# seanwood/gcc-nmf

Measured on AMD Instinct MI355X. Metric: stereo frames/sec (1024-FFT, K=1024, 100 NMF iters), higher is better.
Workload: dtype f32; 1 GPU; HBM-resident (float32 samples in HBM -> separated float32 waveforms in HBM; the host-to-host rates are the host_to_host_* fields of a --full run): 64 x 10 s stereo @16 kHz synthetic mixtures per GPU (SURVEY 8d recipe), 1024-pt FFT hop 256 (F=513, T=622/file), K=1024, 100 KL-NMF iters, 128 TDOAs, 3 targets, independent dictionary per file; dictionary_size=1024, parallelism=file-sharded x1, no data-path collective

## Files before the change

gcc_nmf_amd/_hip.py:

```python
import ctypes
import math
import numbers
import os
import warnings

import torch

_HERE = os.path.dirname(os.path.abspath(__file__))
LIB_PATH = os.environ.get('GCCNMF_HIP_LIB') or os.path.join(_HERE, 'libgccnmf_hip.so')

c_int, c_long, c_float, c_void_p = ctypes.c_int, ctypes.c_long, ctypes.c_float, ctypes.c_void_p
P_INT = ctypes.POINTER(ctypes.c_int)


class SharedShard(ctypes.Structure):
    _fields_ = [('V', c_void_p), ('H', c_void_p), ('workspace', c_void_p), ('N', c_int), ('batch', c_int), ('ld', c_int)]


class DirectGemm(ctypes.Structure):
    _fields_ = [('A', c_void_p), ('B', c_void_p), ('sA', c_long), ('sB', c_long), ('lda', c_int), ('ldb', c_int),
                ('M', c_int), ('N', c_int), ('Kd', c_int), ('batch', c_int),
                ('bscale', c_void_p), ('s_bscale', c_long), ('tailA', c_void_p), ('s_tailA', c_long), ('tail_row', c_int),
                ('rowsumB', c_void_p), ('s_rowsumB', c_long), ('C', c_void_p), ('sC', c_long), ('ldc', c_int),
                ('Ct', c_void_p), ('sCt', c_long), ('ldct', c_int), ('E0', c_void_p), ('sE0', c_long), ('lde0', c_int),
# ... 290 lines not shown

GCCNMF_SCORES_TRACKS = 0x100


def target_scores_masks(CC, trig, idx, W, F, T, K, D, S, batch, ws, scores, argmax, tracks=False, stream=None):
    _stage('gccnmf_target_scores_masks', CC, trig, idx, W, F, T, K, D, S | GCCNMF_SCORES_TRACKS if tracks else S, batch, ws, scores,
           argmax, stream=stream)


GCCNMF_PEAKS_COUNT_BIT = 1 << 30
GCCNMF_SCORES_COUNTED = 0x800
MAX_AUTO_SOURCES = 8
ENGINE_MAX_AUTO_TARGETS = 8


def check_auto_sources(numSources, maxSources=MAX_AUTO_SOURCES):
    if isinstance(numSources, str):
        if numSources != 'auto':
            raise ValueError("numSources must be a number of sources or 'auto', got %r" % (numSources,))
        m = maxSources
        if isinstance(m, bool) or not isinstance(m, numbers.Integral) or not 1 <= m <= 255:
            raise ValueError('maxSources must be a whole number from 1 to 255, got %r' % (m,))
        return True
    return False


def check_auto_targets(numTargets, maxTargets, tdoaTracking=False):
    if check_auto_sources(numTargets, 1):
        if tdoaTracking:
            raise ValueError("numTargets='auto' cannot be combined with tdoaTracking (every frame's peak set takes one count per launch)")
        m = 4 if maxTargets is None else maxTargets
        if isinstance(m, bool) or not isinstance(m, numbers.Integral) or not 1 <= m <= ENGINE_MAX_AUTO_TARGETS:
            raise ValueError('maxTargets must be a whole number from 1 to %d, got %r' % (ENGINE_MAX_AUTO_TARGETS, m))
        return True, int(m)
    if maxTargets is not None:
        raise ValueError("maxTargets needs numTargets='auto'")
    return False, numTargets


def peaks_count_word(maxSources):
    check_auto_sources('auto', maxSources)
    return int(maxSources) | GCCNMF_PEAKS_COUNT_BIT


def count_tdoa_peaks(mean_ang, D, Dp, maxSources, batch, idx, status, stream=None):
    _stage('gccnmf_pick_tdoa_peaks', mean_ang, D, Dp, peaks_count_word(maxSources), batch, idx, status, stream=stream,
           what='gccnmf_pick_tdoa_peaks (count)')


def target_scores_masks_counted(CC, trig, idx, W, F, T, K, D, S, batch, ws, scores, argmax, counted=False, stream=None):
    if not 1 <= int(S) <= 255:
        raise ValueError('the score stage takes 1 to 255 targets, got %r' % (S,))
    _stage('gccnmf_target_scores_masks', CC, trig, idx, W, F, T, K, D, int(S) | GCCNMF_SCORES_COUNTED if counted else int(S), batch, ws,
           scores, argmax, stream=stream, what='gccnmf_target_scores_masks (counted)' if counted else None)


GCCNMF_SCORES_ATOM_TDOA = 0x200
GCCNMF_SCORES_ENHANCEMENT_MASKS = 0x400
ATOM_TDOA_MAX_D = 1024
TARGET_MODE_BOXCAR, TARGET_MODE_MULTIPLE, TARGET_MODE_WINDOW_FUNCTION = 0, 1, 2


def atom_tdoa_indexes(CC, trig, W, F, T, K, D, batch, atom_tdoa, atom_score=None, stream=None):
    _stage('gccnmf_target_scores_masks', CC, trig, None, W, F, T, K, D, GCCNMF_SCORES_ATOM_TDOA, batch, None, atom_score, atom_tdoa,
           stream=stream, what='gccnmf_target_scores_masks (atom TDOA)')


def check_enhancement_target(targetMode, targetTDOAEpsilon, targetTDOABeta, targetTDOANoiseFloor):
    modes = {'boxcar': 0, 'window': 1, TARGET_MODE_BOXCAR: 0, TARGET_MODE_WINDOW_FUNCTION: 1}
    if isinstance(targetMode, bool) or targetMode not in modes:
        raise ValueError("targetMode must be TARGET_MODE_BOXCAR / 'boxcar' or TARGET_MODE_WINDOW_FUNCTION / 'window', got %r" % (targetMode,))
    out = []
    for name, v, low_ok in (('targetTDOAEpsilon', targetTDOAEpsilon, False), ('targetTDOABeta', targetTDOABeta, False),
                            ('targetTDOANoiseFloor', targetTDOANoiseFloor, True)):
        if isinstance(v, bool) or not isinstance(v, numbers.Real) or not math.isfinite(v) or v < 0 or (v == 0 and not low_ok):
            raise ValueError('%s must be a finite number %s 0, got %r' % (name, '>=' if low_ok else '>', v))
        v32 = ctypes.c_float(float(v)).value
        if not math.isfinite(v32) or (v32 == 0 and not low_ok):
            raise ValueError('%s=%r is not a float32 number %s 0' % (name, v, '>=' if low_ok else '>'))
        out.append(v32)
    return (modes[targetMode],) + tuple(out)


def enhancement_masks(atom_tdoa, target, T, K, batch, image, masks, window=0, eps=5.0, beta=2.0, noise_floor=0.0, per_frame=False, stream=None):
    if window not in (0, 1):
        raise ValueError('window must be 0 (boxcar) or 1 (window function), got %r' % (window,))
    params = (c_float * 3)(eps, beta, noise_floor)
    word = GCCNMF_SCORES_ENHANCEMENT_MASKS | int(window) | (GCCNMF_SCORES_TRACKS if per_frame else 0)
    _stage('gccnmf_target_scores_masks', atom_tdoa, ctypes.addressof(params), target, None, 0, T, K, 0, word, batch, None, masks, image,
           stream=stream, what='gccnmf_target_scores_masks (enhancement masks)')


def argmax_targets(scores, K, T, S, batch, argmax, stream=None):
    _stage('gccnmf_argmax_targets', scores, K, T, S, batch, argmax, stream=stream)


RECONSTRUCTIONS = ('direct', 'ratio', 'spatial')
GCCNMF_RECONSTRUCT_RATIO = 0x100
RATIO_MAX_TARGETS = 8
GCCNMF_RECONSTRUCT_SPATIAL_BIT = 1 << 16
GCCNMF_SPATIAL_LOADING = 1e-3
GCCNMF_RECONSTRUCT_SPATIAL_ITERATIONS_SHIFT = 20
MAX_SPATIAL_ITERATIONS = 255


def check_reconstruction(reconstruction, numTargets):
    if reconstruction not in RECONSTRUCTIONS:
        raise ValueError("reconstruction must be 'direct', 'ratio' or 'spatial', got %r" % (reconstruction,))
    if reconstruction != 'direct' and not 1 <= int(numTargets) <= RATIO_MAX_TARGETS:
        raise ValueError("reconstruction=%r takes 1 to %d targets, got %d" % (reconstruction, RATIO_MAX_TARGETS, int(numTargets)))
    return reconstruction


def check_spatial_iterations(spatialIterations, reconstruction):
    n = spatialIterations
    if isinstance(n, bool) or not isinstance(n, numbers.Integral) or not 0 <= int(n) <= MAX_SPATIAL_ITERATIONS:
        raise ValueError('spatialIterations must be an int from 0 to %d, got %r' % (MAX_SPATIAL_ITERATIONS, n))
    if int(n) and reconstruction != 'spatial':
        raise ValueError("spatialIterations=%d needs reconstruction='spatial', got %r" % (int(n), reconstruction))
    return int(n)


def reconstruct_word(S, mode, iterations=0):
    iterations = check_spatial_iterations(iterations, mode)
    word = int(S)
    if mode != 'direct':
        word |= GCCNMF_RECONSTRUCT_RATIO
    return word | (iterations << GCCNMF_RECONSTRUCT_SPATIAL_ITERATIONS_SHIFT)


def reconstruct_spatial_batch(batch):
    if not 1 <= int(batch) <= 65535:
        raise ValueError('the spatial reconstruction takes 1 to 65535 files per call, got %r' % (batch,))
    return int(batch) | GCCNMF_RECONSTRUCT_SPATIAL_BIT


def reconstruct_spatial_workspace_floats(batch, S, Fp):
    return 4 * int(batch) * int(S) * int(Fp)


def reconstruct_spatial_em_workspace_floats(batch, S, Fp, Tp):
    return reconstruct_spatial_workspace_floats(batch, S, Fp) + int(batch) * int(S) * int(Fp) * int(Tp)


def reconstruct_workspace_floats(mode, T, K, S, batch, Fp, iterations=0):
    iterations = check_spatial_iterations(iterations, mode)
    if mode == 'direct':
        return lib().gccnmf_reconstruct_workspace_floats(T, K, S, batch)
    if mode == 'spatial' and iterations:
        return reconstruct_spatial_em_workspace_floats(batch, S, Fp, -(-int(T) // 64) * 64)
    return reconstruct_spatial_workspace_floats(batch, S, Fp) if mode == 'spatial' else 0


def reconstruct(W, H, argmax, masks, X, V, F, T, K, S, batch, spec, mode='direct', workspace=None, iterations=0, stream=None):
    if mode not in RECONSTRUCTIONS:
        raise ValueError('unknown reconstruction mode %r' % (mode,))
    S = reconstruct_word(S, mode, iterations)
    if mode == 'spatial':
        if workspace is None:
            raise ValueError("reconstruction='spatial' needs its covariance workspace (reconstruct_workspace_floats)")
        batch = reconstruct_spatial_batch(batch)
    _stage('gccnmf_reconstruct', W, H, argmax, masks, X, V, F, T, K, S, batch, None if mode == 'ratio' else workspace, spec, stream=stream)


RT_FRAMES, RT_SKIP_LOCALIZE, RT_ONLY_LOCALIZE = 1, 2, 4
RT_BANK_LAYOUT, MAX_BANK_STREAMS = 1 << 3, 4096
RT_MULTI_LAYOUT, MAX_SOURCES = 1 << 20, 8
RT_ROW8_LAYOUT = 1 << 24
RT_LOCALIZE = {'with': 0, 'skip': RT_SKIP_LOCALIZE, 'only': RT_ONLY_LOCALIZE}
RT_SEPARATION_SPATIAL = 2
DEFAULT_SPATIAL_FILTER_FRAMES = 128.0


def rt_spatial_state_offset(D, numTDOAHistory, S=1):
    return -(-(int(S) * int(D) * int(numTDOAHistory)) // 4) * 4


def rt_spatial_state_floats(F, NC, S=1):
    return 4 * int(S) * int(NC) * int(F)


def check_spatial_filter(spatialFilterEnabled, spatialFilterFrames):
    t = spatialFilterFrames
    if isinstance(t, bool) or not isinstance(t, numbers.Real) or not math.isfinite(t) or not t >= 1:
        raise ValueError('spatialFilterFrames must be a finite number of frames >= 1, got %r' % (t,))
    t32 = ctypes.c_float(float(t)).value
    if not math.isfinite(t32):
        raise ValueError('spatialFilterFrames=%r is not a float32' % (t,))
    return bool(spatialFilterEnabled), float(t32)


def rt_mode_word(frames=False, localize='with', streams=None, targets=None, nl_row=False, target_mode=TARGET_MODE_MULTIPLE):
    if not isinstance(localize, str) or localize not in RT_LOCALIZE:
        raise ValueError("localize must be 'with', 'skip' or 'only', got %r" % (localize,))
    word = (RT_FRAMES if frames else 0) | RT_LOCALIZE[localize] | (RT_ROW8_LAYOUT if nl_row else 0)
    if nl_row and (streams is not None or targets is not None):
        raise ValueError('nl_row is the single-stream, single-target row: the bank and multi-target rows always have word 6')
    if streams is not None:
        if frames:
            raise ValueError('a bank of streams has no frames mode')
        if not 1 <= int(streams) <= MAX_BANK_STREAMS:
            raise ValueError('a bank holds 1 to %d streams, got %r' % (MAX_BANK_STREAMS, streams))
        word |= RT_BANK_LAYOUT | (int(streams) - 1) << 8
    if targets is not None:
        if int(target_mode) != TARGET_MODE_MULTIPLE:
            raise ValueError('the multi-target layout needs TARGET_MODE_MULTIPLE, got target_mode %r' % (target_mode,))
        if not 1 <= int(targets) <= MAX_SOURCES:
            raise ValueError('the multi-target layout takes 1 to %d targets, got %r' % (MAX_SOURCES, targets))
        word |= RT_MULTI_LAYOUT | (int(targets) - 1) << 21
    return word


def rt_process_block(block_in, block_out, in_ring, out_ring, X, Y, C, HMask, argmaxTDOA, tfMask, hist, hist_pos, target, gccphat, W, cosT,
                     sinT, window, synthesis_window, twiddle, colsumW, Hcoef, Rv, windowSize, hopSize, blockSize, K, Kp, D, Dp, numTDOAHistory,
                     target_mode, separation_enabled, localization_enabled, localization_window, numHUpdates=0, out_delay_blocks=2,
                     frames=False, localize='with', streams=None, targets=None, nl_row=False, spatial=False, stream=None):
    word = rt_mode_word(frames, localize, streams, targets, nl_row, target_mode)
    if spatial and not (nl_row or streams is not None or targets is not None):
        raise ValueError('spatial needs a target row with a word 7: nl_row, a bank of streams or the multi-target layout')
    separation = (1 | (RT_SEPARATION_SPATIAL if spatial else 0)) if separation_enabled else 0
    _stage('gccnmf_rt_process_block_ll', block_in, block_out, in_ring, out_ring, X, Y, C, HMask, argmaxTDOA, tfMask, hist, hist_pos, target,
           gccphat, W, cosT, sinT, window, synthesis_window, twiddle, colsumW, Hcoef, Rv, windowSize, hopSize, blockSize, K, Kp, D, Dp,
           numTDOAHistory, int(target_mode), separation, int(bool(localization_enabled)), localization_window, word,
           int(numHUpdates), int(out_delay_blocks), stream=stream)
```

gcc_nmf_amd/csrc/common.h:

```cpp
#pragma once
#include <hip/hip_runtime.h>
#include <stdint.h>

#define GCCNMF_OK 0
#define GCCNMF_ERR_ARG 1
#define GCCNMF_ERR_LAUNCH 2
#define GCCNMF_ERR_UNSUPPORTED 3

static inline int gccnmf_ceil_div(int a, int b) { return (a + b - 1) / b; }
static inline int gccnmf_round_up(int a, int b) { return gccnmf_ceil_div(a, b) * b; }

#define GCCNMF_CHECK_LAUNCH()                                   \
    do {                                                        \
        hipError_t e__ = hipGetLastError();                     \
        if (e__ != hipSuccess) return GCCNMF_ERR_LAUNCH;        \
    } while (0)

struct GccNmfPitches {
    int Fp, Kp, Np, Tp;
};

static inline GccNmfPitches gccnmf_make_pitches(int F, int T, int K) {
    GccNmfPitches p;
    p.Fp = gccnmf_round_up(F, 16);
    p.Kp = gccnmf_round_up(K, 64);
    p.Np = gccnmf_round_up(2 * T, 64);
    p.Tp = gccnmf_round_up(T, 64);
    return p;
}

#define GCCNMF_TUNE_KEYS 26
struct GccNmfTune {
    int v[GCCNMF_TUNE_KEYS];
};
extern thread_local GccNmfTune gccnmf_tune;
struct GccNmfCall {
    GccNmfCall();
    ~GccNmfCall();
};
#define GCCNMF_ENTER() GccNmfCall gccnmf_call_scope_
#define gccnmf_tune_ablate (gccnmf_tune.v[1])
#define gccnmf_tune_tile_policy (gccnmf_tune.v[2])
#define gccnmf_tune_dma (gccnmf_tune.v[3])
#define gccnmf_tune_ring (gccnmf_tune.v[4])
#define gccnmf_tune_wh_splits (gccnmf_tune.v[5])
#define gccnmf_tune_rht_splits (gccnmf_tune.v[6])
#define gccnmf_tune_exact_div (gccnmf_tune.v[7])
#define gccnmf_tune_shared_groups (gccnmf_tune.v[8])
#define gccnmf_tune_tail_split (gccnmf_tune.v[9])
#define gccnmf_tune_direct (gccnmf_tune.v[10])
#define gccnmf_tune_direct_tile (gccnmf_tune.v[11])
#define gccnmf_tune_direct_batch (gccnmf_tune.v[12])
#define gccnmf_tune_direct_depth (gccnmf_tune.v[13])
#define gccnmf_tune_short_updh (gccnmf_tune.v[14])
#define gccnmf_tune_fft_r16 (gccnmf_tune.v[15])
#define gccnmf_tune_fused_k12 (gccnmf_tune.v[16])
#define gccnmf_tune_fused_k34 (gccnmf_tune.v[17])
#define gccnmf_tune_persistent (gccnmf_tune.v[18])
#define gccnmf_tune_prefetch (gccnmf_tune.v[19])
#define gccnmf_tune_wide_update_w (gccnmf_tune.v[20])
#define gccnmf_tune_chain (gccnmf_tune.v[21])
#define gccnmf_tune_chain_solo (gccnmf_tune.v[22])
#define gccnmf_tune_chain_rag (gccnmf_tune.v[23])
#define gccnmf_tune_chain_chunk (gccnmf_tune.v[24])
#define gccnmf_tune_chain_fault (gccnmf_tune.v[25])
```

gcc_nmf_amd/csrc/gcc.hip:

```cpp
#include "gemm_ring.h"
#include "ratio.h"
#include "spatial.h"
#include "angular_nl.h"
#include "atom_tdoa.h"
#include "source_count.h"
#include "../../include/gccnmf_hip.h"


static bool gcc_small_launch(int batch, int M, int N, int Kd) {
    if (!gccnmf_tune_ring || !gccnmf_ring_supports(Kd) || gccnmf_tune_tile_policy == 1) return false;
    if (gccnmf_tune_tile_policy == 2) return true;
    return (long)batch * gccnmf_ceil_div(M, 512) * gccnmf_ceil_div(N, 64) < 256;
}

__global__ __launch_bounds__(256) void ang_mean_kernel(const float* __restrict__ ang, int T, int D, int Dp, int Tp,
                                                       double* __restrict__ mean_ang) {
    __shared__ double red[256];
    const int b = blockIdx.x / D, d = blockIdx.x - b * D;
    const float* row = ang + ((long)b * Dp + d) * Tp;
    double s = 0.0;
    for (int t = threadIdx.x; t < T; t += 256) s += (double)row[t];
    red[threadIdx.x] = s;
    __syncthreads();
    for (int w = 128; w > 0; w >>= 1) {
        if (threadIdx.x < w) red[threadIdx.x] += red[threadIdx.x + w];
        __syncthreads();
    }
    if (threadIdx.x == 0) mean_ang[(long)b * Dp + d] = red[0] / (double)T;
}

__device__ __forceinline__ bool pick_peaks_row(const double* v, unsigned char* is_peak, int* s_found, int D, int S, int* out,
                                               long out_stride) {
    __syncthreads();
    for (int i = threadIdx.x; i < D; i += 64) is_peak[i] = (i > 0 && i < D - 1 && v[i] > v[i - 1] && v[i] > v[i + 1]) ? 1 : 0;
    __syncthreads();
    if (threadIdx.x == 0) *s_found = 0;
    __syncthreads();
    for (int s = 0; s < S; ++s) {
        double bv = 0.0;
        int bi = -1;
        for (int i = 1 + threadIdx.x; i < D - 1; i += 64)
            if (is_peak[i] == 1 && (bi < 0 || v[i] >= bv)) {
                bv = v[i];
                bi = i;
            }
#pragma unroll
        for (int o = 32; o > 0; o >>= 1) {
            const double ov = __shfl_xor(bv, o);
            const int oi = __shfl_xor(bi, o);
            if (oi >= 0 && (bi < 0 || ov > bv || (ov == bv && oi > bi))) {
                bv = ov;
                bi = oi;
            }
        }
        if (bi < 0) break;
        if (threadIdx.x == 0) {
            is_peak[bi] = 2;
            ++*s_found;
        }
        __syncthreads();
    }
    __syncthreads();
    if (threadIdx.x != 0) return false;
    int n = 0;
    for (int i = 1; i < D - 1 && n < S; ++i)
        if (is_peak[i] == 2) out[(n++) * out_stride] = i;
    for (; n < S; ++n) out[n * out_stride] = -1;
    return *s_found == S;
}

__global__ __launch_bounds__(64) void pick_peaks_kernel(const double* __restrict__ mean_ang, int D, int Dp, int S,
                                                        int* __restrict__ tdoa_idx, int* __restrict__ status) {
    __shared__ double v[4096];
    __shared__ unsigned char is_peak[4096];
    __shared__ int s_found;
    const int b = blockIdx.x;
    const double* m = mean_ang + (long)b * Dp;
    for (int i = threadIdx.x; i < D; i += 64) v[i] = m[i];
    const bool all = pick_peaks_row(v, is_peak, &s_found, D, S, tdoa_idx + (long)b * S, 1);
    if (threadIdx.x == 0) status[b] = all ? 0 : 1;
}

__global__ __launch_bounds__(64) void track_peaks_kernel(const float* __restrict__ ang, int T, int Tp, int D, int Dp, int S, int L,
                                                         int* __restrict__ tracks, int* __restrict__ status) {
    extern __shared__ double track_lds[];
    double* v = track_lds;
    int* s_found = (int*)(track_lds + D);
    unsigned char* is_peak = (unsigned char*)(track_lds + D + 2);
    const int t = blockIdx.x, b = blockIdx.y;
    const int first = t - L / 2;
    const int lo = first < 0 ? 0 : first, hi = first + L < T ? first + L : T;
    const double len = (double)(hi - lo);
    for (int d = threadIdx.x; d < D; d += 64) {
        const float* row = ang + ((long)b * Dp + d) * Tp;
        double s = 0.0;
        for (int g = lo & ~3; g < hi; g += 4) {
            const float4 a = *(const float4*)(row + g);
            if (g >= lo) s += (double)a.x;
            if (g + 1 >= lo && g + 1 < hi) s += (double)a.y;
            if (g + 2 >= lo && g + 2 < hi) s += (double)a.z;
            if (g + 3 >= lo && g + 3 < hi) s += (double)a.w;
        }
        v[d] = s / len;
    }
    const bool all = pick_peaks_row(v, is_peak, s_found, D, S, tracks + (long)b * S * Tp + t, Tp);
    if (threadIdx.x == 0) status[(long)b * Tp + t] = all ? 0 : 1;
}

__global__ __launch_bounds__(256) void track_carry_kernel(int T, int Tp, int S, int* __restrict__ tracks, int* __restrict__ status) {
    __shared__ int scan[256];
    __shared__ int s_carry, s_first;
    const int tid = threadIdx.x;
    int* st = status + (long)blockIdx.x * Tp;
    int* tr = tracks + (long)blockIdx.x * S * Tp;
    if (tid == 0) {
        s_carry = -1;
        s_first = T;
    }
    __syncthreads();
    for (int c = 0; c < T; c += 256) {
        const int t = c + tid;
        const bool complete = t < T && st[t] == 0;
        if (complete) atomicMin(&s_first, t);
        scan[tid] = complete ? t : -1;
        __syncthreads();
        for (int o = 1; o < 256; o <<= 1) {
            const int left = tid >= o ? scan[tid - o] : -1;
            __syncthreads();
            if (left > scan[tid]) scan[tid] = left;
            __syncthreads();
        }
        const int src = scan[tid] > s_carry ? scan[tid] : s_carry;
        if (t < T) st[t] = src;
        __syncthreads();
        if (tid == 255) s_carry = src;
        __syncthreads();
    }
    const int first = s_first;
    for (int t = tid; t < T; t += 256) {
        int src = st[t];
        if (src == t) {
            st[t] = 0;
            continue;
        }
        if (src < 0) src = first;
        for (int i = 0; i < S; ++i) tr[(long)i * Tp + t] = first < T ? tr[(long)i * Tp + src] : -1;
        st[t] = first < T ? 1 : 3;
    }
}

__device__ __forceinline__ float4 gcc_steer4(float4 cr, float4 ci, float4 c, float4 sn) {
#pragma clang fp contract(off)
    float4 out;
    out.x = fmaf(cr.x, c.x, ci.x * sn.x);
    out.y = cr.y * c.y + ci.y * sn.y;
    out.z = fmaf(cr.z, c.z, ci.z * sn.z);
    out.w = fmaf(cr.w, c.w, ci.w * sn.w);
    return out;
}

template <bool TRACKS, bool COUNTED>
__global__ __launch_bounds__(256) void gcc_steer_kernel(const float* __restrict__ CC, const float* __restrict__ trig,
                                                        const int* __restrict__ tdoa_idx, int F, int Fp, int T, int Tp, int D,
                                                        int Dp, int S, float* __restrict__ P) {
    const int col = 4 * (blockIdx.x * 256 + threadIdx.x);
// ... 169 lines not shown
    return GCCNMF_OK;
}

int gccnmf_pick_tdoa_peaks(const double* mean_ang, int D, int Dp, int S, int batch, int* tdoa_idx, int* status,
                           void* stream) {
    GCCNMF_ENTER();
    if (S > 0 && (S & ~0xff) == GCCNMF_PEAKS_COUNT_BIT) {
        S &= 0xff;
        if (!mean_ang || !tdoa_idx || !status || D < 3 || D > SOURCE_COUNT_MAX_D || Dp < D || S < 1 || batch < 1) return GCCNMF_ERR_ARG;
        return gccnmf_launch_count_peaks(mean_ang, D, Dp, S, batch, tdoa_idx, status, (hipStream_t)stream);
    }
    if (S & ~0xff) {
        const int L = (S >> 9) & 0x3fffff, T = Dp;
        if (S < 0 || !(S & GCCNMF_PEAKS_TRACKS_BIT) || L < 1) return GCCNMF_ERR_ARG;
        S &= 0xff;
        if (!mean_ang || !tdoa_idx || !status || D < 3 || D > 4096 || T < 1 || T >= (1 << 21) || S < 1 || batch < 1 || batch > 65535)
            return GCCNMF_ERR_ARG;
        const int Tp = gccnmf_round_up(T, 64);
        hipLaunchKernelGGL(track_peaks_kernel, dim3(T, batch), dim3(64), 8 * D + 16 + gccnmf_round_up(D, 16), (hipStream_t)stream, (const float*)mean_ang, T, Tp, D,
                           gccnmf_round_up(D, 64), S, L, tdoa_idx, status);
        GCCNMF_CHECK_LAUNCH();
        hipLaunchKernelGGL(track_carry_kernel, dim3(batch), dim3(256), 0, (hipStream_t)stream, T, Tp, S, tdoa_idx, status);
        GCCNMF_CHECK_LAUNCH();
        return GCCNMF_OK;
    }
    if (!mean_ang || !tdoa_idx || !status || D < 3 || D > 4096 || Dp < D || S < 1 || batch < 1) return GCCNMF_ERR_ARG;
    hipLaunchKernelGGL(pick_peaks_kernel, dim3(batch), dim3(64), 0, (hipStream_t)stream, mean_ang, D, Dp, S, tdoa_idx, status);
    GCCNMF_CHECK_LAUNCH();
    return GCCNMF_OK;
}

long gccnmf_scores_workspace_floats(int F, int T, int S, int batch) {
    GCCNMF_ENTER();
    if (F < 2 || T < 1 || S < 1 || batch < 1) return -1;
    GccNmfPitches p = gccnmf_make_pitches(F, T, 1);
    return (long)batch * p.Fp * S * p.Tp;
}

int gccnmf_target_scores_masks(const float* CC, const float* trig, const int* tdoa_idx, const float* W, int F, int T,
                               int K, int D, int S, int batch, float* workspace, float* scores, unsigned char* argmax,
                               void* stream) {
    GCCNMF_ENTER();
    const int mode = S & ~0xff;
    if (S > 0 && mode == GCCNMF_SCORES_ATOM_TDOA) {
        if (S & 0xff) return GCCNMF_ERR_ARG;
        if (!CC || !trig || !W || !argmax || F < 2 || T < 1 || K < 1 || D < 1 || batch < 1) return GCCNMF_ERR_ARG;
        if (D > ATOM_TDOA_MAX_D || batch > 65535 || T > (1 << 19)) return GCCNMF_ERR_UNSUPPORTED;
        return gccnmf_launch_atom_tdoa(CC, trig, W, F, T, K, D, batch, (unsigned short*)argmax, scores, (hipStream_t)stream);
    }
    if (S > 0 && (mode & ~GCCNMF_SCORES_TRACKS) == GCCNMF_SCORES_ENHANCEMENT_MASKS) {
        const int window = S & 0xff;
        if (window > 1 || !CC || !trig || !tdoa_idx || (!scores && !argmax) || T < 1 || K < 1 || batch < 1) return GCCNMF_ERR_ARG;
        const float eps = trig[0], beta = trig[1], nf = trig[2];
        if (!(eps > 0.f && eps < INFINITY && beta > 0.f && beta < INFINITY && nf >= 0.f && nf < INFINITY)) return GCCNMF_ERR_ARG;
        if (batch > 65535 || K > 65535 - 63) return GCCNMF_ERR_UNSUPPORTED;
        return gccnmf_launch_enhancement_masks((const unsigned short*)CC, tdoa_idx, (mode & GCCNMF_SCORES_TRACKS) ? 1 : 0, window, eps,
                                               beta, nf, T, K, batch, argmax, scores, (hipStream_t)stream);
    }
    if (S < 0 || ((mode & ~GCCNMF_SCORES_TRACKS) && mode != GCCNMF_SCORES_COUNTED)) return GCCNMF_ERR_ARG;
    S &= 0xff;
    const bool tracks = mode == GCCNMF_SCORES_TRACKS, counted = mode == GCCNMF_SCORES_COUNTED;
    if (!CC || !trig || !tdoa_idx || !W || !workspace || !scores || F < 2 || T < 1 || K < 1 || D < 1 || S < 1 || batch < 1)
        return GCCNMF_ERR_ARG;
    hipStream_t s = (hipStream_t)stream;
    GccNmfPitches p = gccnmf_make_pitches(F, T, K);
    const int Dp = gccnmf_round_up(D, 64);
    const int ncol = S * p.Tp;
    float* P = workspace;
    if (counted)
        hipLaunchKernelGGL((gcc_steer_kernel<false, true>), dim3(gccnmf_ceil_div(ncol, 1024), p.Fp, batch), dim3(256), 0, s, CC, trig,
                           tdoa_idx, F, p.Fp, T, p.Tp, D, Dp, S, P);
    else if (tracks)
        hipLaunchKernelGGL((gcc_steer_kernel<true, false>), dim3(gccnmf_ceil_div(ncol, 1024), p.Fp, batch), dim3(256), 0, s, CC, trig, tdoa_idx,
                           F, p.Fp, T, p.Tp, D, Dp, S, P);
    else
        hipLaunchKernelGGL((gcc_steer_kernel<false, false>), dim3(gccnmf_ceil_div(ncol, 1024), p.Fp, batch), dim3(256), 0, s, CC, trig, tdoa_idx,
                           F, p.Fp, T, p.Tp, D, Dp, S, P);
    GCCNMF_CHECK_LAUNCH();
    GemmArgs a = {};
    a.A = W; a.sA = (long)p.Fp * p.Kp; a.lda = p.Kp; a.a_clamp = p.Kp - 4;
    a.B = P; a.sB = (long)p.Fp * ncol; a.ldb = ncol; a.b_clamp = ncol - 4;
    a.M = K; a.N = ncol; a.Kd = F;
    if ((F % 16) == 1) {
        a.Kd = F - 1;
        a.ktailA = W + (long)(F - 1) * p.Kp; a.s_ktailA = a.sA;
        a.ktailB = P + (long)(F - 1) * ncol; a.s_ktailB = a.sB;
    }
    a.batch = batch; a.xcd_affine = 1;
    a.C = scores; a.sC = (long)p.Kp * ncol; a.ldc = ncol;
    int rc;
    if (gcc_small_launch(batch, a.M, a.N, a.Kd)) rc = gccnmf_launch_gemm_ring<false, false, EPI_STORE, false>(a, s);
    else if (K > 128 && gccnmf_tune_dma && gccnmf_tune_ablate != 128) rc = gccnmf_launch_gemm_dma<false, false, EPI_STORE, false>(a, s);
    else rc = (K > 128) ? gccnmf_launch_gemm<4, 1, false, false, EPI_STORE, false>(a, s)
                        : gccnmf_launch_gemm<1, 4, false, false, EPI_STORE, false>(a, s);
    if (rc) return rc;
    if (argmax) {
        hipLaunchKernelGGL(gcc_argmax_kernel, dim3(gccnmf_ceil_div(p.Tp, 1024), p.Kp, batch), dim3(256), 0, s, scores, K, p.Kp, T,
                           p.Tp, S, argmax);
        GCCNMF_CHECK_LAUNCH();
    }
    return GCCNMF_OK;
}

int gccnmf_argmax_targets(const float* scores, int K, int T, int S, int batch, unsigned char* argmax, void* stream) {
    GCCNMF_ENTER();
    if (!scores || !argmax || K < 1 || T < 1 || S < 1 || S > 255 || batch < 1) return GCCNMF_ERR_ARG;
    GccNmfPitches p = gccnmf_make_pitches(2, T, K);
    hipLaunchKernelGGL(gcc_argmax_kernel, dim3(gccnmf_ceil_div(p.Tp, 1024), p.Kp, batch), dim3(256), 0, (hipStream_t)stream, scores,
                       K, p.Kp, T, p.Tp, S, argmax);
    GCCNMF_CHECK_LAUNCH();
    return GCCNMF_OK;
}

int gccnmf_coherence(const float* X, int F, int T, int batch, float* CC, void* stream) {
    GCCNMF_ENTER();
    if (!X || !CC || F < 2 || T < 1 || batch < 1) return GCCNMF_ERR_ARG;
    GccNmfPitches p = gccnmf_make_pitches(F, T, 1);
    hipLaunchKernelGGL(gcc_coherence_kernel, dim3(gccnmf_ceil_div(T, 256), F, batch), dim3(256), 0, (hipStream_t)stream,
                       (const float2*)X, p.Fp, T, p.Tp, CC);
    GCCNMF_CHECK_LAUNCH();
    return GCCNMF_OK;
}

int gccnmf_magnitude(const float* X, int F, int T, int batch, float* V, void* stream) {
    GCCNMF_ENTER();
    if (!X || !V || F < 2 || T < 1 || batch < 1) return GCCNMF_ERR_ARG;
    GccNmfPitches p = gccnmf_make_pitches(F, T, 1);
    hipLaunchKernelGGL(gcc_magnitude_kernel, dim3(gccnmf_ceil_div(T, 256), F, batch * 2), dim3(256), 0, (hipStream_t)stream,
                       (const float2*)X, p.Fp, T, p.Tp, p.Np, V);
    GCCNMF_CHECK_LAUNCH();
    return GCCNMF_OK;
}

long gccnmf_reconstruct_workspace_floats(int T, int K, int S, int batch) {
    GCCNMF_ENTER();
    if (T < 1 || K < 1 || S < 1 || batch < 1) return -1;
    GccNmfPitches p = gccnmf_make_pitches(2, T, K);
    return (long)batch * p.Kp * 2 * S * p.Tp;
}

int gccnmf_reconstruct(const float* W, const float* H, const unsigned char* argmax, const float* masks, const float* X,
                       const float* V, int F, int T, int K, int S, int batch, float* workspace, float* spec, void* stream) {
    GCCNMF_ENTER();
    const int mode = S & ~0xff;
    S &= 0xff;
    if (mode & ~(GCCNMF_RECONSTRUCT_RATIO | GCCNMF_RECONSTRUCT_SPATIAL_ITERATIONS(0xff))) return GCCNMF_ERR_ARG;
    const bool ratio = (mode & GCCNMF_RECONSTRUCT_RATIO) != 0;
    const int iterations = (mode >> 20) & 0xff;
    if (batch < 1 || (batch & ~(0xffff | GCCNMF_RECONSTRUCT_SPATIAL_BIT))) return GCCNMF_ERR_ARG;
    const bool spatial = (batch & GCCNMF_RECONSTRUCT_SPATIAL_BIT) != 0;
    batch &= 0xffff;
    if (spatial && !ratio) return GCCNMF_ERR_ARG;
    if (iterations && !spatial) return GCCNMF_ERR_ARG;
    if (!W || !H || (!argmax && !masks) || !X || (!ratio && (!V || !workspace)) || !spec || F < 2 || T < 1 || K < 1 || S < 1 || batch < 1)
        return GCCNMF_ERR_ARG;
    if (spatial && (!workspace || ((uintptr_t)workspace & 15))) return GCCNMF_ERR_ARG;
    if (ratio && S > GCCNMF_RATIO_MAX_TARGETS) return GCCNMF_ERR_UNSUPPORTED;
    hipStream_t s = (hipStream_t)stream;
    if (ratio) {
        const int rc = gccnmf_launch_ratio(W, H, argmax, masks, X, F, T, K, S, batch, spec, s);
        if (rc != GCCNMF_OK || !spatial) return rc;
        if (!iterations) return gccnmf_launch_spatial(X, F, T, S, batch, workspace, spec, s);
        GccNmfPitches p = gccnmf_make_pitches(F, T, 1);
        float* powers = workspace + GCCNMF_RECONSTRUCT_SPATIAL_WORKSPACE_FLOATS(batch, S, p.Fp);
        return gccnmf_launch_spatial_em(X, F, T, S, batch, iterations, workspace, powers, spec, s);
    }
    GccNmfPitches p = gccnmf_make_pitches(F, T, K);
    const int ncol = 2 * S * p.Tp;
    float* Hm = workspace;
    hipLaunchKernelGGL(gcc_masked_h_kernel, dim3(gccnmf_ceil_div(ncol, 1024), p.Kp, batch), dim3(256), 0, s, H, argmax, masks, K, p.Kp,
                       T, p.Tp, p.Np, S, Hm);
    GCCNMF_CHECK_LAUNCH();
    const bool tail = (F % 128) == 1;
    GemmArgs a = {};
    a.A = W; a.sA = (long)p.Fp * p.Kp; a.lda = p.Kp; a.a_clamp = p.Fp - 1;
    a.B = Hm; a.sB = (long)p.Kp * ncol; a.ldb = ncol; a.b_clamp = ncol - 4;
    a.M = tail ? F - 1 : F; a.N = ncol; a.Kd = K;
    a.tail_row = F - 1;
    a.batch = batch; a.xcd_affine = 1;
    a.C = spec; a.sC = 2L * S * p.Fp * p.Tp;
    a.E0 = V; a.sE0 = (long)p.Fp * p.Np;
    a.X = (const float2*)X; a.sX = 2L * p.Fp * p.Tp;
    a.T = T; a.Tp = p.Tp; a.Fp = p.Fp; a.ldv = p.Np;
    if (gcc_small_launch(batch, a.M, a.N, a.Kd))
        return tail ? gccnmf_launch_gemm_ring<true, false, EPI_PHASE, true>(a, s) : gccnmf_launch_gemm_ring<true, false, EPI_PHASE, false>(a, s);
    const bool tall = a.M > 128;
    if (tall && gccnmf_tune_dma && gccnmf_tune_ablate != 128)
        return tail ? gccnmf_launch_gemm_dma<true, false, EPI_PHASE, true>(a, s) : gccnmf_launch_gemm_dma<true, false, EPI_PHASE, false>(a, s);
    if (tall) return tail ? gccnmf_launch_gemm<4, 1, true, false, EPI_PHASE, true>(a, s)
                          : gccnmf_launch_gemm<4, 1, true, false, EPI_PHASE, false>(a, s);
    return tail ? gccnmf_launch_gemm<1, 4, true, false, EPI_PHASE, true>(a, s)
                : gccnmf_launch_gemm<1, 4, true, false, EPI_PHASE, false>(a, s);
}

}
```

gcc_nmf_amd/csrc/gemm_dma.h:

```cpp
#pragma once
#include <mutex>
#include <type_traits>
#include "gemm_mfma.h"
#include "chain_sync.h"

#ifndef GEMM_DMA_ABL
#define GEMM_DMA_ABL 0
#endif

typedef __attribute__((address_space(3))) void* gemm_lds_ptr;
typedef __attribute__((address_space(1))) const void* gemm_glb_ptr;

__device__ __forceinline__ void gemm_dma16(const float* wave_uniform_base, unsigned lane_byte_offset, unsigned lds_wave_byte_addr) {
    asm volatile("s_mov_b32 m0, %2\n\tglobal_load_lds_dwordx4 %0, %1"
                 :
                 : "v"(lane_byte_offset), "s"(wave_uniform_base), "s"(lds_wave_byte_addr)
                 : "memory");
}

__device__ __forceinline__ void gemm_dma16_masked(const float* wave_uniform_base, unsigned lane_byte_offset, unsigned lds_wave_byte_addr,
                                                  unsigned long long wave_uniform_mask) {
    unsigned long long saved;
    asm volatile("s_mov_b64 %0, exec\n\ts_mov_b64 exec, %4\n\ts_mov_b32 m0, %3\n\tglobal_load_lds_dwordx4 %1, %2\n\ts_mov_b64 exec, %0"
                 : "=&s"(saved)
                 : "v"(lane_byte_offset), "s"(wave_uniform_base), "s"(lds_wave_byte_addr), "s"(wave_uniform_mask)
                 : "memory");
}

__device__ __forceinline__ int gemm_swz(int row) { return (row >> 2) & 3; }

__device__ __forceinline__ int gemm_opaque_tid() {
    int t;
    asm volatile("v_mov_b32 %0, %1" : "=v"(t) : "v"(threadIdx.x));
    return t;
}

typedef float gemm_f32x4 __attribute__((ext_vector_type(4)));
template <int OFF>
__device__ __forceinline__ gemm_f32x4 gemm_lds_read_b128(unsigned byte_addr) {
    gemm_f32x4 v;
    asm volatile("ds_read_b128 %0, %1 offset:%2" : "=v"(v) : "v"(byte_addr), "n"(OFF));
    return v;
}
typedef float gemm_f32x2 __attribute__((ext_vector_type(2)));
template <int OFF0, int OFF1>
__device__ __forceinline__ gemm_f32x2 gemm_lds_read2_b32(unsigned byte_addr) {
    gemm_f32x2 v;
    asm volatile("ds_read2_b32 %0, %1 offset0:%2 offset1:%3" : "=v"(v) : "v"(byte_addr), "n"(OFF0), "n"(OFF1));
    return v;
}

__device__ __forceinline__ void gemm_wait_lds() { asm volatile("s_waitcnt lgkmcnt(0)" ::: "memory"); }
template <typename T>
__device__ __forceinline__ void gemm_tie(T& v) { asm volatile("" : "+v"(v)); }

__device__ __forceinline__ void gemm_barrier_arrive(unsigned counter_byte_addr) {
    unsigned long long saved;
    asm volatile("s_mov_b64 %0, exec\n\ts_mov_b64 exec, 1\n\tds_add_u32 %1, %2\n\ts_mov_b64 exec, %0"
                 : "=&s"(saved)
                 : "v"(counter_byte_addr), "v"(1u)
                 : "memory");
}
__device__ __forceinline__ unsigned gemm_barrier_peek(unsigned counter_byte_addr) {
    unsigned seen;
    asm volatile("ds_read_b32 %0, %1" : "=v"(seen) : "v"(counter_byte_addr) : "memory");
    return seen;
}
__device__ __forceinline__ void gemm_barrier_wait(unsigned counter_byte_addr, unsigned target, unsigned seen) {
    unsigned seen_s;
    asm volatile("s_waitcnt lgkmcnt(0)\n1:\n\tv_readfirstlane_b32 %1, %0\n\ts_cmp_ge_u32 %1, %3\n\ts_cbranch_scc1 2f\n\t"
                 "s_sleep 1\n\tds_read_b32 %0, %2\n\ts_waitcnt lgkmcnt(0)\n\ts_branch 1b\n2:"
                 : "+v"(seen), "=&s"(seen_s)
                 : "v"(counter_byte_addr), "s"(target)
                 : "memory", "scc");
}

template <bool KC, int NT, int ROWS>
struct GemmFrag;
template <int NT, int ROWS>
struct GemmFrag<true, NT, ROWS> {
    gemm_f32x4 v[NT];
    __device__ __forceinline__ void read(unsigned base) {
        v[0] = gemm_lds_read_b128<0 * 2048>(base);
        v[1] = gemm_lds_read_b128<1 * 2048>(base);
        if constexpr (NT == 4) {
            v[2] = gemm_lds_read_b128<2 * 2048>(base);
            v[3] = gemm_lds_read_b128<3 * 2048>(base);
        }
    }
    __device__ __forceinline__ void tie() {
#pragma unroll
        for (int m = 0; m < NT; ++m) gemm_tie(v[m]);
    }
    __device__ __forceinline__ void clear() {
#pragma unroll
        for (int m = 0; m < NT; ++m) v[m] = gemm_f32x4{0.f, 0.f, 0.f, 0.f};
    }
    __device__ __forceinline__ float get(int m, int e) const { return v[m][e]; }
    __device__ __forceinline__ void scale(const gemm_f32x4& s) {
#pragma unroll
        for (int m = 0; m < NT; ++m) v[m] *= s;
    }
};
template <int NT, int ROWS>
struct GemmFrag<false, NT, ROWS> {
    gemm_f32x2 v[4][NT / 2];
    __device__ __forceinline__ void read(unsigned base) {
#pragma unroll
        for (int e = 0; e < 4; ++e) {
            v[e][0] = gemm_lds_read2_b32<0, 32>(base + 4 * e * ROWS);
            if constexpr (NT == 4) v[e][1] = gemm_lds_read2_b32<64, 96>(base + 4 * e * ROWS);
        }
    }
    __device__ __forceinline__ void tie() {
#pragma unroll
        for (int e = 0; e < 4; ++e)
#pragma unroll
            for (int h = 0; h < NT / 2; ++h) gemm_tie(v[e][h]);
    }
    __device__ __forceinline__ void clear() {
#pragma unroll
        for (int e = 0; e < 4; ++e)
#pragma unroll
            for (int h = 0; h < NT / 2; ++h) v[e][h] = gemm_f32x2{0.f, 0.f};
    }
    __device__ __forceinline__ float get(int m, int e) const { return v[e][m >> 1][m & 1]; }
    __device__ __forceinline__ void scale(const gemm_f32x4& s) {
#pragma unroll
        for (int e = 0; e < 4; ++e)
#pragma unroll
            for (int h = 0; h < NT / 2; ++h) v[e][h] *= s[e];
    }
};

__device__ __forceinline__ float gemm_div_fast(float v, float d) {
    const float r = __builtin_amdgcn_rcpf(d);
    const float q = v * r;
    return fmaf(fmaf(-d, q, v), r, q);
}

typedef int gemm_i32x4 __attribute__((ext_vector_type(4)));
__device__ float gemm_buffer_load(gemm_i32x4 rsrc, int voffset, int soffset, int aux) __asm("llvm.amdgcn.raw.buffer.load.f32");
__device__ gemm_f32x4 gemm_buffer_load4(gemm_i32x4 rsrc, int voffset, int soffset, int aux) __asm("llvm.amdgcn.raw.buffer.load.v4f32");
__device__ void gemm_buffer_store(float data, gemm_i32x4 rsrc, int voffset, int soffset, int aux) __asm("llvm.amdgcn.raw.buffer.store.f32");
__device__ __forceinline__ gemm_i32x4 gemm_buffer_rsrc(const void* wave_uniform_base, long bytes = 0x7fffffffL) {
    const unsigned long long a = (unsigned long long)wave_uniform_base;
    gemm_i32x4 r;
    r.x = __builtin_amdgcn_readfirstlane((int)(unsigned)a);
    r.y = __builtin_amdgcn_readfirstlane((int)(unsigned)(a >> 32) & 0xffff);
    r.z = __builtin_amdgcn_readfirstlane((int)(bytes < 0x7fffffffL ? bytes : 0x7fffffffL));
    r.w = 0x00020000;
    return r;
}

template <int EPI, int BM = 512>
struct GemmEpiloguePair {
    static_assert(EPI == EPI_STORE || EPI == EPI_DIV || EPI == EPI_UPDH, "");
    float xa[16], xb[16];

    __device__ __forceinline__ void load(const GemmArgs& p, int file, int row_u, int hh, int col_a, long cb) {
        if (EPI == EPI_DIV || EPI == EPI_UPDH) {
            const int lo = 4 * (4 * hh * p.ldc + col_a);
            const int ro = 4 * row_u * p.ldc, rstep = 4 * p.ldc;
            const gemm_i32x4 X = gemm_buffer_rsrc(EPI == EPI_DIV ? p.E0 + file * p.sE0 : p.C + file * p.sC, cb);
#pragma unroll
            for (int r = 0; r < 16; ++r) {
                const int so = ro + ((r & 3) + 8 * (r >> 2)) * rstep;
                xa[r] = gemm_buffer_load(X, lo, so, 0);
                xb[r] = gemm_buffer_load(X, lo + 128, so, 0);
            }
        }
    }

    __device__ __forceinline__ void finish(const GemmArgs& p, int file, int row_u, int tile_row, int hh, int col_a, float ba, float bb,
                                           const float* s_rowvec, const f32x16& acc_a, const f32x16& acc_b, bool oka, bool okb, long cb) const {
        const int lo = 4 * (4 * hh * p.ldc + col_a);
        const int ro = 4 * row_u * p.ldc, rstep = 4 * p.ldc;
        const gemm_i32x4 C = gemm_buffer_rsrc(p.C + file * p.sC, cb);
        auto column = [&](const f32x16& acc, const float (&x)[16], const float b, const int lane_off) {
            float u[16];
#pragma unroll
            for (int r = 0; r < 16; ++r) u[r] = acc[r];
            if (EPI == EPI_STORE || EPI == EPI_UPDH) {
#pragma unroll
                for (int g = 0; g < 4; ++g) {
                    const gemm_f32x4 tav = *(const gemm_f32x4*)(s_rowvec + tile_row + 8 * g + 4 * hh);
                    gemm_f32x4 gv = {1.f, 1.f, 1.f, 1.f};
                    if (EPI == EPI_UPDH) gv = *(const gemm_f32x4*)(s_rowvec + BM + tile_row + 8 * g + 4 * hh);
#pragma unroll
                    for (int i = 0; i < 4; ++i) {
                        const int r = 4 * g + i;
                        u[r] = fmaf(tav[i], b, u[r]);
                        if (EPI == EPI_UPDH) u[r] = (x[r] * u[r]) * gv[i];
                    }
                }
            }
            if (EPI == EPI_DIV) {
                if (p.exact_div) {
#pragma unroll
                    for (int r = 0; r < 16; ++r) u[r] = x[r] / u[r];
                } else {
// ... 61 lines not shown
        if (TAIL) {
            const float u = (s_tail[tid] + s_tail[64 + tid]) + (s_tail[128 + tid] + s_tail[192 + tid]);
            wt_tail = Wp[(long)p.tail_row * p.ldc + col0 + tid] * (u / s_rs[tid]);
        }
        s_red[256 + tid] = wt_tail * wt_tail;
    }
    __syncthreads();
    if (tid < 64) s_norm[tid] = sqrtf(((s_red[tid] + s_red[64 + tid]) + (s_red[128 + tid] + s_red[192 + tid])) + s_red[256 + tid]);
    __syncthreads();
    const float ina = 1.0f / s_norm[ca], inb = 1.0f / s_norm[cb];
    float csa = 0.f, csb = 0.f;
    if (wave_active) {
#pragma unroll
        for (int m = 0; m < 4; ++m) {
            const int ro = (wm * 128 + m * 32) * rstep;
#pragma unroll
            for (int r = 0; r < 16; ++r) {
                const int so = ro + ((r & 3) + 8 * (r >> 2)) * rstep;
                const float na = acc[m][0][r] * ina, nb = acc[m][1][r] * inb;
                gemm_buffer_store(na, W, lo, so, 0);
                gemm_buffer_store(nb, W, lo + 128, so, 0);
                csa += na;
                csb += nb;
            }
        }
    }
    csa += __shfl_xor(csa, 32);
    csb += __shfl_xor(csb, 32);
    if (hh == 0) {
        s_red[wm * 64 + ca] = csa;
        s_red[wm * 64 + cb] = csb;
    }
    if (tid < 64) {
        float wn_tail = 0.f;
        if (TAIL) {
            wn_tail = wt_tail / s_norm[tid];
            Wp[(long)p.tail_row * p.ldc + col0 + tid] = wn_tail;
        }
        s_red[256 + tid] = wn_tail;
    }
    __syncthreads();
    if (tid < 64) {
        p.out_colsum[file * p.s_out + col0 + tid] = ((s_red[tid] + s_red[64 + tid]) + (s_red[128 + tid] + s_red[192 + tid])) + s_red[256 + tid];
        p.out_norm[file * p.s_out + col0 + tid] = s_norm[tid];
    }
}

__host__ __device__ __forceinline__ int gemm_dma_list_file(const GemmArgs& p, int q) {
    if (p.lists != 8) return q;
    const int n_full = p.batch >> 3, rem = p.batch & 7, big = rem * (n_full + 1);
    const int cls = q < big ? q / (n_full + 1) : rem + (q - big) / n_full;
    return cls + 8 * (q < big ? q - cls * (n_full + 1) : (q - big) - (cls - rem) * n_full);
}
__host__ __device__ __forceinline__ bool gemm_dma_item(const GemmArgs& p, int list, int t, int& file, int& tm, int& col0, int& nw) {
    if (p.ragged_n) {
        const int* L = p.ragged_lists + list * (GEMM_RAGGED_LMAX + 1);
        const int cnt = L[0];
        int acc = 0;
        for (int k = 0; k < cnt; ++k) {
            const int f = L[1 + k];
            const int n = p.ragged_kd ? p.N : p.ragged_n[f];
            const int tn = (n + 63) >> 6, per = p.tiles_m * tn;
            if (t < acc + per) {
                const int w = t - acc;
                const int wide_n = tn - (gemm_dma_file_rag(p.narrow_ok, n) ? 1 : 0), wt = p.tiles_m * wide_n;
                if (w < wt) {
                    tm = w / wide_n;
                    col0 = (w - tm * wide_n) * 64;
                    nw = 2;
                } else {
                    tm = w - wt;
                    col0 = (tn - 1) * 64;
                    nw = 1;
                }
                file = f + p.file0;
                return true;
            }
            acc += per;
        }
        return false;
    }
    const int wt = p.tiles_m * p.wide_n;
    if (p.whole_files == 2) {
        const int per = p.tiles_m * p.tiles_n;
        const long idx = (long)list * p.cw + t;
        if (t >= p.cw || idx >= (long)p.batch * per) return false;
        const int q = (int)(idx / per), w = (int)(idx - (long)q * per);
        if (w < wt) {
            tm = w / p.wide_n;
            col0 = (w - tm * p.wide_n) * 64;
            nw = 2;
        } else {
            tm = w - wt;
            col0 = (p.tiles_n - 1) * 64;
            nw = 1;
        }
        file = gemm_dma_list_file(p, q) + p.file0;
        return true;
    }
    if (p.whole_files) {
        const int per = p.tiles_m * p.tiles_n;
        const int ql = t / per, w = t - ql * per;
        const int fi = list + 8 * ql;
        if (fi >= p.batch) return false;
        if (w < wt) {
            tm = w / p.wide_n;
            col0 = (w - tm * p.wide_n) * 64;
            nw = 2;
        } else {
            tm = w - wt;
            col0 = (p.tiles_n - 1) * 64;
            nw = 1;
        }
        file = fi + p.file0;
        return true;
    }
    const int base_w = list * p.cw;
    const int len = min(max(p.batch * wt - base_w, 0), p.cw), s = min(p.split, len);
    int q;
    if (t < len + s) {
        int idx, half = 0;
        if (t < len - s) {
            idx = base_w + t;
            nw = 2;
        } else {
            const int j = t - (len - s);
            idx = base_w + (len - s) + (j >> 1);
            half = j & 1;
            nw = 1;
        }
        q = idx / wt;
        const int w = idx - q * wt;
        tm = w / p.wide_n;
        col0 = (w - tm * p.wide_n) * 64 + 32 * half;
    } else {
        const int r = t - (len + s), base_r = list * p.cr;
        const int lenr = min(max(p.batch * p.rag * p.tiles_m - base_r, 0), p.cr);
        if (r >= lenr) return false;
        const int idx = base_r + r;
        q = idx / p.tiles_m;
        tm = idx - q * p.tiles_m;
        col0 = (p.tiles_n - 1) * 64;
        nw = 1;
    }
    file = gemm_dma_list_file(p, q) + p.file0;
    return true;
}

template <int TM>
struct GemmDmaLds {
    static constexpr int SBUF = 128 * TM * 16 + 64 * 16 + 16 + 16;
};

template <bool A_KC, bool B_KC, int EPI, bool TAIL, int TM, bool NARROW>
__device__ __forceinline__ void gemm_dma_workgroup(const GemmArgs& p, float* const smem, float* const s_rowvec, unsigned* const s_arrivals_p,
                                                   int* const s_ticket, const int list, int t, const GemmSync& sync, const int sync_it = 0,
                                                   const bool trace_on = true) {
    static_assert(TM == 4 || TM == 2, "");
    static_assert(TM == 4 || EPI != EPI_UPDW, "the fused W update owns all rows of its atoms: full-height tiles only");
    static_assert(!NARROW || (EPI != EPI_UPDW && TM == 4), "narrow items: full-height tiles with an element-wise epilogue");
    constexpr int BK = 16, BM = 128 * TM, BN = 64, RW = 32 * TM;
    constexpr int NA = 2 * TM;
    constexpr int SA = BM * BK, SB = BN * BK;
    constexpr int SBUF = SA + SB + BK + BK;
    static_assert(SBUF == GemmDmaLds<TM>::SBUF, "");
    constexpr bool SCALE = !B_KC && (EPI == EPI_DIV || EPI == EPI_STORE);
    unsigned& s_arrivals = *s_arrivals_p;

    int tid = threadIdx.x, lane = tid & 63;
    const int wave = __builtin_amdgcn_readfirstlane(tid >> 6);
    const int wm = wave, wn = 0;
    int l31 = lane & 31, hh = lane >> 5;
#ifdef GCCNMF_EXPERIMENTS
    const bool persistent = p.tickets != nullptr;
#else
    constexpr bool persistent = false;
#endif

    int nkt = (p.Kd + BK - 1) / BK;
    int n_item = p.N;
    int n_sync = p.N;
    int file = 0, tm = 0, col0 = 0, nw = 2, row0 = 0;
    const float* __restrict__ A = nullptr;
    const float* __restrict__ B = nullptr;
    const float* __restrict__ bscale = nullptr;
    const float* __restrict__ tail_src = nullptr;
    const float* __restrict__ scale_src = nullptr;
    unsigned long long tail_mask = 0, scale_mask = 0;
    bool wave_active = false, do_tail = false, do_rowsum = false;
    unsigned offA[NA], offB = 0;
    auto take_item = [&](const int ticket) -> bool {
        int f_, tm_, c_, nw_;
        if (!gemm_dma_item(p, list, ticket, f_, tm_, c_, nw_)) return false;
        file = __builtin_amdgcn_readfirstlane(f_);
        tm = __builtin_amdgcn_readfirstlane(tm_);
        col0 = __builtin_amdgcn_readfirstlane(c_);
        nw = NARROW ? __builtin_amdgcn_readfirstlane(nw_) : 2;
        if (p.ragged_n) {
            const int nf = __builtin_amdgcn_readfirstlane(p.ragged_n[file]);
            n_sync = nf;
            if (p.ragged_kd) nkt = (nf + BK - 1) / BK;
            else n_item = nf;
        }
        row0 = tm * BM;
        A = p.A + file * p.sA;
        B = p.B + file * p.sB;
        bscale = (SCALE && p.bscale) ? p.bscale + file * p.s_bscale : nullptr;
        wave_active = (row0 + wm * RW) < p.M;
        do_tail = TAIL && (tm == 0);
        do_rowsum = B_KC && (p.rowsumB != nullptr || EPI == EPI_UPDW) && (tm == 0);
        tail_src = A + (long)p.tail_row * p.lda;
        tail_mask = (wave == 0 && do_tail) ? 0x0full : 0ull;
        scale_mask = (wave == 0 && bscale != nullptr) ? 0xf0ull : 0ull;
        scale_src = bscale != nullptr ? bscale : A;
        return true;
    };
    auto set_offsets = [&](const int lane) {
#pragma unroll
        for (int i = 0; i < NA; ++i) {
            const int piece = wave * NA + i;
            if (A_KC) {
                const int row = piece * 16 + (lane >> 2), c = (lane & 3) ^ gemm_swz(piece * 16 + (lane >> 2));
                offA[i] = 4u * (unsigned)(min(row0 + row, p.a_clamp) * p.lda + 4 * c);
            } else {
                constexpr int PPR = BM / 256;
                const int kk = piece / PPR, col = (piece % PPR) * 256 + lane * 4;
                offA[i] = 4u * (unsigned)(kk * p.lda + min(row0 + col, p.a_clamp));
            }
        }
        if (B_KC) {
            const int row = wave * 16 + (lane >> 2), c = (lane & 3) ^ gemm_swz(row);
            offB = 4u * (unsigned)(min(col0 + row, p.b_clamp) * p.ldb + 4 * c);
        } else {
            const int kk = wave * 4 + (lane >> 4), col = (lane & 15) * 4;
            offB = 4u * (unsigned)(kk * p.ldb + min(col0 + col, p.b_clamp));
        }
    };

    f32x16 acc[TM][2];
    float tail_acc = 0.f, rowsum_acc = 0.f;

    const unsigned lds0 = __builtin_amdgcn_readfirstlane((unsigned)(size_t)(gemm_lds_ptr)smem);
    unsigned side_off = 0;

    auto dma_piece = [&](const int piece, const int kt, const int buf) {
#ifdef GEMM_DMA_SKIP_FROM
        if (piece >= GEMM_DMA_SKIP_FROM) return;
#endif
        if (piece < NA) {
            gemm_dma16(A + (A_KC ? (long)kt * BK : (long)kt * BK * p.lda), offA[piece], lds0 + 4 * (buf * SBUF + (wave * NA + piece) * 256));
        } else if (piece == NA) {
            gemm_dma16(B + (B_KC ? (long)kt * BK : (long)kt * BK * p.ldb), offB, lds0 + 4 * (buf * SBUF + SA + wave * 256));
        } else {
            if (TAIL || SCALE) {
                const unsigned dst = lds0 + 4 * (buf * SBUF + SA + SB);
                if (TAIL) gemm_dma16_masked(tail_src + kt * BK, side_off, dst, tail_mask);
                if (SCALE) gemm_dma16_masked(scale_src + kt * BK, side_off, dst, scale_mask);
            }
        }
    };
    constexpr int NPIECES = NA + 2;
#ifdef GEMM_DMA_SPREAD
    constexpr int SPREAD = GEMM_DMA_SPREAD;
#else
    constexpr int SPREAD = (A_KC && !B_KC) ? 1 : 2;
#endif

    const gemm_f32x4 zero4 = {0.f, 0.f, 0.f, 0.f};
    GemmFrag<A_KC, TM, BM> a0, a1;
    GemmFrag<B_KC, 2, BN> b0, b1;
    gemm_f32x4 sc0 = zero4, sc1 = zero4, t4 = zero4, tb4 = zero4, ts4 = zero4, rs4 = zero4;
    gemm_f32x2 tbxy = {0.f, 0.f}, tbzw = {0.f, 0.f};

    const unsigned arrivals_addr = (unsigned)(size_t)(gemm_lds_ptr)s_arrivals_p;
    unsigned oA0 = 0, oA1 = 0, oB0 = 0, oB1 = 0, oTB = 0, oRS = 0;
    const int tg = wave;
    auto set_lane_constants = [&](const int tid_) {
        tid = tid_;
        lane = tid_ & 63;
        l31 = lane & 31;
        hh = lane >> 5;
        const int arow = wm * RW + l31, bcol = wn * 64 + l31, tj = lane;
        side_off = 16u * (unsigned)(lane & 3);
        oA0 = A_KC ? 4 * (arow * 16 + 4 * ((0 + hh) ^ gemm_swz(arow))) : 4 * (4 * (0 + hh) * BM + arow);
        oA1 = A_KC ? 4 * (arow * 16 + 4 * ((2 + hh) ^ gemm_swz(arow))) : 4 * (4 * (2 + hh) * BM + arow);
        oB0 = 4 * SA + (B_KC ? 4 * (bcol * 16 + 4 * ((0 + hh) ^ gemm_swz(bcol))) : 4 * (4 * (0 + hh) * BN + bcol));
        oB1 = 4 * SA + (B_KC ? 4 * (bcol * 16 + 4 * ((2 + hh) ^ gemm_swz(bcol))) : 4 * (4 * (2 + hh) * BN + bcol));
        oTB = 4 * SA + (B_KC ? 4 * (tj * 16 + 4 * (tg ^ gemm_swz(tj))) : 4 * (4 * tg * BN + tj));
        oRS = 4 * SA + 4 * ((tid_ >> 2) * 16 + 4 * (tid_ & 3));
    };

    auto read_group0 = [&](const unsigned lds) {
        if (wave_active) {
            a0.read(lds + oA0);
            b0.read(lds + oB0);
        }
        if (SCALE) sc0 = gemm_lds_read_b128<4 * (SA + SB + BK)>(lds + 16 * hh);
    };
    auto read_group1 = [&](const unsigned lds) {
        if (wave_active) {
            a1.read(lds + oA1);
            b1.read(lds + oB1);
        }
        if (SCALE) sc1 = gemm_lds_read_b128<4 * (SA + SB + BK) + 32>(lds + 16 * hh);
        if (TAIL) {
            t4 = gemm_lds_read_b128<4 * (SA + SB)>(lds + 16 * tg);
            if (B_KC) {
                tb4 = gemm_lds_read_b128<0>(lds + oTB);
            } else {
                tbxy = gemm_lds_read2_b32<0 * BN, 1 * BN>(lds + oTB);
                tbzw = gemm_lds_read2_b32<2 * BN, 3 * BN>(lds + oTB);
                if (SCALE) ts4 = gemm_lds_read_b128<4 * (SA + SB + BK)>(lds + 16 * tg);
            }
        }
        if (B_KC) rs4 = gemm_lds_read_b128<0>(lds + oRS);
    };
    auto wait_group0 = [&]() {
        gemm_wait_lds();
        a0.tie();
        b0.tie();
        if (SCALE) {
            gemm_tie(sc0);
            b0.scale(sc0);
        }
    };
    auto wait_group1 = [&]() {
        gemm_wait_lds();
        a1.tie();
        b1.tie();
        if (SCALE) {
            gemm_tie(sc1);
            b1.scale(sc1);
        }
        if (TAIL) {
            gemm_tie(t4);
            if (B_KC) {
                gemm_tie(tb4);
            } else {
                gemm_tie(tbxy);
                gemm_tie(tbzw);
                tb4 = gemm_f32x4{tbxy.x, tbxy.y, tbzw.x, tbzw.y};
                if (SCALE) {
                    gemm_tie(ts4);
                    tb4 *= ts4;
                }
            }
        }
        if (B_KC) gemm_tie(rs4);
    };
    auto mma = [&](auto nw_c, const GemmFrag<A_KC, TM, BM>& a, const GemmFrag<B_KC, 2, BN>& b, const int e, const int m) {
        constexpr int NW = decltype(nw_c)::value;
        acc[m][0] = __builtin_amdgcn_mfma_f32_32x32x2f32(a.get(m, e), b.get(0, e), acc[m][0], 0, 0, 0);
        if constexpr (NW == 2) acc[m][1] = __builtin_amdgcn_mfma_f32_32x32x2f32(a.get(m, e), b.get(1, e), acc[m][1], 0, 0, 0);
    };

#ifdef GEMM_DMA_PROBE
    unsigned long long probe[7] = {0, 0, 0, 0, 0, 0, 0};
#define GEMM_PROBE(i_) const unsigned long long pt##i_ = __builtin_amdgcn_s_memtime()
#define GEMM_PROBE_DECL(i_) unsigned long long pt##i_ = 0
#define GEMM_PROBE_SET(i_) pt##i_ = __builtin_amdgcn_s_memtime()
#else
#define GEMM_PROBE(i_)
#define GEMM_PROBE_DECL(i_)
#define GEMM_PROBE_SET(i_)
#endif
    auto step = [&](auto cur_c, auto nw_c, const int kt) {
        constexpr int CUR = decltype(cur_c)::value;
        const unsigned ldsC = lds0 + 4 * CUR * SBUF, ldsN = lds0 + 4 * (CUR ^ 1) * SBUF;
        const int ktn = min(kt + 1, nkt - 1);
        GEMM_PROBE(0);
#if !(GEMM_DMA_ABL & 1)
        read_group1(ldsC);
#endif
        __builtin_amdgcn_sched_barrier(0);
        if (wave_active) {
            if (SPREAD == 0) {
#pragma unroll
                for (int i = 0; i < NPIECES; ++i) dma_piece(i, ktn, CUR ^ 1);
                __builtin_amdgcn_sched_barrier(0);
            }
#pragma unroll
            for (int e = 0; e < 4; ++e)
#pragma unroll
                for (int m = 0; m < TM; ++m) {
                    mma(nw_c, a0, b0, e, m);
                    const int slot = e * TM + m;
                    if (SPREAD == 1 && slot < NPIECES) {
                        dma_piece(slot, ktn, CUR ^ 1);
                        __builtin_amdgcn_sched_barrier(0);
                    }
                    if (SPREAD == 2 && slot % 3 != 2 && (slot / 3) * 2 + slot % 3 < NPIECES) {
                        dma_piece((slot / 3) * 2 + slot % 3, ktn, CUR ^ 1);
                        __builtin_amdgcn_sched_barrier(0);
                    }
                }
        } else {
#pragma unroll
            for (int i = 0; i < NPIECES; ++i) dma_piece(i, ktn, CUR ^ 1);
        }
        __builtin_amdgcn_sched_barrier(0);
        GEMM_PROBE(1);
        wait_group1();
        GEMM_PROBE(2);
        GEMM_PROBE_DECL(3);
        GEMM_PROBE_DECL(4);
        GEMM_PROBE_DECL(5);
        unsigned seen = 0;
#ifndef GEMM_DMA_ARRIVE_E
#define GEMM_DMA_ARRIVE_E 1
#define GEMM_DMA_WAIT_E 3
#endif
#pragma unroll
        for (int e = 0; e < 4; ++e) {
            if (e == GEMM_DMA_ARRIVE_E) {
                __builtin_amdgcn_sched_barrier(0);
                GEMM_PROBE_SET(3);
                asm volatile("s_waitcnt vmcnt(0)" ::: "memory");
#if !(GEMM_DMA_ABL & 2)
                gemm_barrier_arrive(arrivals_addr);
#endif
                __builtin_amdgcn_sched_barrier(0);
            }
            if (e == GEMM_DMA_WAIT_E - 1) {
                __builtin_amdgcn_sched_barrier(0);
#if !(GEMM_DMA_ABL & 2)
                seen = gemm_barrier_peek(arrivals_addr);
#endif
                __builtin_amdgcn_sched_barrier(0);
            }
            if (e == GEMM_DMA_WAIT_E) {
                __builtin_amdgcn_sched_barrier(0);
                GEMM_PROBE_SET(4);
#if !(GEMM_DMA_ABL & 2)
                gemm_barrier_wait(arrivals_addr, 4u * (unsigned)(kt + 1), seen);
#endif
                GEMM_PROBE_SET(5);
#if !(GEMM_DMA_ABL & 1)
                read_group0(ldsN);
#endif
                __builtin_amdgcn_sched_barrier(0);
            }
            if (wave_active) {
#pragma unroll
                for (int m = 0; m < TM; ++m) mma(nw_c, a1, b1, e, m);
            }
        }
        if (TAIL) {
            tail_acc = fmaf(t4.x, tb4.x, tail_acc);
            tail_acc = fmaf(t4.y, tb4.y, tail_acc);
            tail_acc = fmaf(t4.z, tb4.z, tail_acc);
            tail_acc = fmaf(t4.w, tb4.w, tail_acc);
        }
        if (B_KC) rowsum_acc += (rs4.x + rs4.y) + (rs4.z + rs4.w);
        __builtin_amdgcn_sched_barrier(0);
        GEMM_PROBE(6);
        wait_group0();
#ifdef GEMM_DMA_PROBE
        __builtin_amdgcn_sched_barrier(0);
        const unsigned long long pt7 = __builtin_amdgcn_s_memtime();
        probe[0] += pt1 - pt0;
        probe[1] += pt2 - pt1;
        probe[2] += pt3 - pt2;
        probe[3] += pt4 - pt3;
        probe[4] += pt5 - pt4;
        probe[5] += pt6 - pt5;
        probe[6] += pt7 - pt6;
        __builtin_amdgcn_sched_barrier(0);
#endif
    };
    auto main_loop = [&](auto nw_c) {
        for (int kt = 0; kt < nkt; kt += 2) {
            step(std::integral_constant<int, 0>{}, nw_c, kt);
            if (kt + 1 < nkt) step(std::integral_constant<int, 1>{}, nw_c, kt + 1);
        }
    };

    if (SCALE) {
        if (!p.bscale && tid < 2 * BK) smem[(tid >> 4) * SBUF + SA + SB + BK + (tid & 15)] = 1.f;
    }
    bool have = take_item(t);
    if (have) set_offsets(lane);
    bool prefetched = false;
    int it = 0;
    long long* trace_row = nullptr;
    while (have) {
        const int vb = p.lists == 8 ? 8 * t + list : t;
        trace_row = (trace_on && p.trace && vb < p.trace_rows) ? p.trace + 8 * (long)vb : nullptr;
        if (trace_row && tid == 0) {
            trace_row[0] = trace_row[1] = __builtin_amdgcn_s_memrealtime();
            trace_row[4] = (long long)((__builtin_amdgcn_s_getreg((3 << 11) | 20) & 15u) << 16 | (__builtin_amdgcn_s_getreg((31 << 11) | 4) & 0xffffu));
            trace_row[7] = (long long)blockIdx.x << 16 | (long long)it;
        }
#ifdef GCCNMF_EXPERIMENTS
        set_lane_constants(gemm_opaque_tid());
        if (it > 0) set_offsets(lane);
        a0.clear(); a1.clear(); b0.clear(); b1.clear();
        sc0 = sc1 = t4 = tb4 = ts4 = rs4 = zero4;
        tbxy = tbzw = gemm_f32x2{0.f, 0.f};
#else
        set_lane_constants(tid);
#endif
        gemm_sync_wait(sync, file, col0, tid, sync_it, list, n_sync);
        if (trace_row && tid == 0) trace_row[1] = __builtin_amdgcn_s_memrealtime();
        if (!prefetched) {
#pragma unroll
            for (int i = 0; i < NPIECES; ++i) dma_piece(i, 0, 0);
        }
#pragma unroll
        for (int m = 0; m < TM; ++m)
#pragma unroll
            for (int n = 0; n < 2; ++n)
#pragma unroll
                for (int r = 0; r < 16; ++r) acc[m][n][r] = 0.f;
        tail_acc = 0.f;
        rowsum_acc = 0.f;
        if constexpr (EPI == EPI_STORE || EPI == EPI_UPDH) {
#pragma unroll
            for (int i = 0; i < BM / 256; ++i) {
                const int lr = tid + 256 * i, row = min(row0 + lr, p.M - 1);
                s_rowvec[lr] = p.ktailA ? p.ktailA[file * p.s_ktailA + row] : 0.f;
                if (EPI == EPI_UPDH) {
                    const float rd = 1.0f / (p.E2[file * p.sE2 + row] + p.alpha + p.eps);
                    s_rowvec[BM + lr] = p.E1 ? p.E1[file * p.sE1 + row] * rd : rd;
                }
            }
        }
        if (tid == 0) {
            s_arrivals = 0;
            if (persistent) s_ticket[it & 1] = p.wpl + (int)__hip_atomic_fetch_add(p.tickets + list, 1u, __ATOMIC_RELAXED, __HIP_MEMORY_SCOPE_AGENT);
        }
        asm volatile("s_waitcnt vmcnt(0)" ::: "memory");
        __syncthreads();
        read_group0(lds0);
        wait_group0();

        if constexpr (NARROW) {
            if (nw == 1) main_loop(std::integral_constant<int, 1>{});
            else main_loop(std::integral_constant<int, 2>{});
        } else {
            main_loop(std::integral_constant<int, 2>{});
        }
        __syncthreads();
        if (trace_row && tid == 0) trace_row[2] = __builtin_amdgcn_s_memrealtime();

        const int e_file = file, e_row0 = row0, e_col0 = col0, e_nw = nw, e_n = n_item;
        const bool e_active = wave_active, e_tail = do_tail, e_rowsum = do_rowsum;
        have = false;
        prefetched = false;
        if (persistent) {
            t = __builtin_amdgcn_readfirstlane(s_ticket[it & 1]);
            have = take_item(t);
            if (have && p.prefetch) {
                set_offsets(gemm_opaque_tid() & 63);
#pragma unroll
                for (int i = 0; i < NPIECES; ++i) dma_piece(i, 0, 0);
                prefetched = true;
            }
        }
        float* const scratch = smem + SBUF;

        if constexpr (EPI == EPI_UPDW) {
            if constexpr (TM == 4) gemm_epilogue_update_w_full<TAIL>(p, e_file, e_col0, tid, wm, l31, hh, e_active, acc, tail_acc, rowsum_acc, scratch);
        } else {
            if (e_active) {
                const int row_w = e_row0 + wm * RW;
                bool lean = false;
                if constexpr (EPI == EPI_STORE || EPI == EPI_DIV || EPI == EPI_UPDH) {
                    lean = row_w + RW <= p.M;
                    if (lean) {
                        GemmEpiloguePair<EPI, BM> e0, e1;
                        const int ca = e_col0 + l31, tr = wm * RW;
                        const bool oka = ca < e_n, okb = (!NARROW || e_nw == 2) && ca + 32 < e_n;
                        const long cb = 4L * p.ldc * (p.M + (TAIL ? 1 : 0));
                        float ba = 0.f, bb = 0.f;
                        e0.load(p, e_file, row_w, hh, ca, cb);
                        e1.load(p, e_file, row_w + 32, hh, ca, cb);
                        if (EPI != EPI_DIV && p.ktailA) {
                            ba = p.ktailB[e_file * p.s_ktailB + min(ca, e_n - 1)];
                            bb = p.ktailB[e_file * p.s_ktailB + min(ca + 32, e_n - 1)];
                        }
                        e0.finish(p, e_file, row_w, tr, hh, ca, ba, bb, s_rowvec, acc[0][0], acc[0][1], oka, okb, cb);
                        if (trace_row && tid == 0) trace_row[5] = __builtin_amdgcn_s_memrealtime();
                        if constexpr (TM == 4) e0.load(p, e_file, row_w + 64, hh, ca, cb);
                        e1.finish(p, e_file, row_w + 32, tr + 32, hh, ca, ba, bb, s_rowvec, acc[1][0], acc[1][1], oka, okb, cb);
                        if constexpr (TM == 4) {
                            e1.load(p, e_file, row_w + 96, hh, ca, cb);
                            e0.finish(p, e_file, row_w + 64, tr + 64, hh, ca, ba, bb, s_rowvec, acc[2][0], acc[2][1], oka, okb, cb);
                            e1.finish(p, e_file, row_w + 96, tr + 96, hh, ca, ba, bb, s_rowvec, acc[3][0], acc[3][1], oka, okb, cb);
                        }
                        if (trace_row && tid == 0) trace_row[6] = __builtin_amdgcn_s_memrealtime();
                    }
                }
                if (!lean) {
                    GemmArgs pq = p;
                    pq.N = e_n;
#pragma unroll
                    for (int m = 0; m < TM; ++m)
                        gemm_epilogue_pair<EPI>(pq, e_file, row_w + m * 32 + 4 * hh, e_col0 + wn * 64 + l31, acc[m][0], acc[m][1], !NARROW || e_nw == 2);
                }
            }
            if (TAIL) {
                if (e_tail) {
                    scratch[tid] = tail_acc;
                    __syncthreads();
                    if (tid < (NARROW && e_nw == 1 ? 32 : BN)) {
                        const float s = (scratch[tid] + scratch[BN + tid]) + (scratch[2 * BN + tid] + scratch[3 * BN + tid]);
                        const int col = e_col0 + tid;
                        if (EPI == EPI_PHASE ? gemm_col_valid<EPI>(p, col) : col < e_n) gemm_epilogue<EPI>(p, e_file, p.tail_row, col, s);
                    }
                }
            }
            if (B_KC) {
                if (e_rowsum) {
                    float s = rowsum_acc;
                    s += __shfl_xor(s, 1);
                    s += __shfl_xor(s, 2);
                    const int j = tid >> 2;
                    if ((tid & 3) == 0 && (e_col0 + j) < e_n && (!NARROW || e_nw == 2 || j < 32)) p.rowsumB[e_file * p.s_rowsumB + e_col0 + j] = s;
                }
            }
        }
        if (trace_row) {
            asm volatile("s_waitcnt vmcnt(0)" ::: "memory");
            __syncthreads();
            if (tid == 0) trace_row[3] = __builtin_amdgcn_s_memrealtime();
        }
        gemm_sync_signal(sync, e_file, e_col0, e_nw, tid);
        ++it;
        if (have) __syncthreads();
    }
#ifdef GEMM_DMA_PROBE
    if (p.trace && lane == 0 && (long)p.trace_grid + 4L * blockIdx.x + 4 <= p.trace_rows) {
#pragma unroll
        for (int i = 0; i < 7; ++i) p.trace[8 * ((long)p.trace_grid + blockIdx.x * 4 + wave) + i] = (long long)probe[i];
        p.trace[8 * ((long)p.trace_grid + blockIdx.x * 4 + wave) + 7] = it;
    }
#endif
    if (persistent && tid == 0) {
        const unsigned gone = __hip_atomic_fetch_add(p.tickets + 8, 1u, __ATOMIC_ACQ_REL, __HIP_MEMORY_SCOPE_AGENT);
        if (gone == gridDim.x - 1) {
#pragma unroll
            for (int i = 0; i < 9; ++i) __hip_atomic_store(p.tickets + i, 0u, __ATOMIC_RELAXED, __HIP_MEMORY_SCOPE_AGENT);
        }
    }
}

template <bool A_KC, bool B_KC, int EPI, bool TAIL, int TM, bool NARROW>
__global__ __launch_bounds__(256, 2) void gccnmf_gemm_dma_kernel(GemmArgs p) {
    __shared__ __attribute__((aligned(16))) float smem[2 * GemmDmaLds<TM>::SBUF];
    __shared__ __attribute__((aligned(16))) float s_rowvec[(EPI == EPI_STORE || EPI == EPI_UPDH) ? 2 * 128 * TM : 4];
    __shared__ unsigned s_arrivals;
    __shared__ int s_ticket[2];
    const int list = p.lists == 8 ? (int)(blockIdx.x & 7) : 0;
    const int t = p.lists == 8 ? (int)(blockIdx.x >> 3) : (int)blockIdx.x;
    GemmSync none = {};
    gemm_dma_workgroup<A_KC, B_KC, EPI, TAIL, TM, NARROW>(p, smem, s_rowvec, &s_arrivals, s_ticket, list, t, none);
}

struct GemmChain {
    int first[5];
    int it0, iterations;
    int trace_it;
    GemmSync sync[4];
};
template <bool TAIL, int STAGES, int TM1>
__global__ __launch_bounds__(256, 2) void gccnmf_gemm_chain_kernel(GemmArgs p0, GemmArgs p1, GemmArgs p2, GemmArgs p3, GemmChain ch) {
    static_assert(STAGES == 2 || STAGES == 4, "");
    __shared__ __attribute__((aligned(16))) float smem[2 * GemmDmaLds<4>::SBUF];
    __shared__ __attribute__((aligned(16))) float s_rowvec[2 * 512];
    __shared__ unsigned s_arrivals;
    __shared__ int s_ticket[2];
    const int list = (int)(blockIdx.x & 7);
    int pos = (int)(blockIdx.x >> 3), it = ch.it0;
    if (ch.iterations > 1) {
        const int q = pos / ch.first[4];
        it += q;
        pos -= q * ch.first[4];
    }
    const bool tr = it == ch.trace_it;
    if (pos < ch.first[1]) {
        gemm_dma_workgroup<true, false, EPI_DIV, TAIL, 4, true>(p0, smem, s_rowvec, &s_arrivals, s_ticket, list, pos, ch.sync[0], it, tr);
    } else if (pos < ch.first[2]) {
        gemm_dma_workgroup<false, false, EPI_UPDH, false, TM1, TM1 == 4>(p1, smem, s_rowvec, &s_arrivals, s_ticket, list, pos - ch.first[1], ch.sync[1], it, tr);
    } else if constexpr (STAGES == 4) {
        if (pos < ch.first[3]) {
            gemm_dma_workgroup<true, false, EPI_DIV, TAIL, 4, true>(p2, smem, s_rowvec, &s_arrivals, s_ticket, list, pos - ch.first[2], ch.sync[2], it, tr);
        } else {
            gemm_dma_workgroup<true, true, EPI_UPDW, TAIL, 4, false>(p3, smem, s_rowvec, &s_arrivals, s_ticket, list, pos - ch.first[3], ch.sync[3], it, tr);
        }
    }
}

#ifdef GCCNMF_EXPERIMENTS
unsigned* gccnmf_ticket_block(hipStream_t stream);
#endif

static int gemm_dma_plan(GemmArgs& a, bool narrow_capable, int TM, int whole_files = 0) {
    a.tiles_m = gccnmf_ceil_div(a.M, 128 * TM);
    a.tiles_n = gccnmf_ceil_div(a.N, 64);
    a.lists = (a.xcd_affine && a.batch >= 8) ? 8 : 1;
    const int policy = gccnmf_tune_tail_split;
    const bool narrow_ok = narrow_capable && TM == 4 && policy != 0;
    a.narrow_ok = narrow_ok ? 1 : 0;
    const long tiles = (long)a.batch * a.tiles_m * a.tiles_n;
    if (tiles > (1L << 28)) return -1;
    a.rag = (narrow_ok && a.tiles_n >= 2 && a.N - (a.tiles_n - 1) * 64 <= 32) ? 1 : 0;
    if (a.rag && policy == 1 && !a.concurrent) {
        const long slots = a.lists == 8 ? 64 : 512;
        const long plain = (tiles + a.lists - 1) / a.lists;
        const long with_rag = ((long)a.batch * a.tiles_m * (a.tiles_n - 1) + a.lists - 1) / a.lists + ((long)a.batch * a.tiles_m + a.lists - 1) / a.lists;
        if ((with_rag + slots - 1) / slots > (plain + slots - 1) / slots) a.rag = 0;
    }
    a.wide_n = a.tiles_n - a.rag;
    a.whole_files = 0;
    if (whole_files) {
        if (a.lists != 8 || policy > 1) return -1;
        a.rag = (narrow_ok && a.tiles_n >= 2 && a.N - (a.tiles_n - 1) * 64 <= 32) ? 1 : 0;
        a.wide_n = a.tiles_n - a.rag;
        a.whole_files = whole_files;
        a.cw = whole_files == 2 ? (int)((tiles + 7) / 8) : ((a.batch + 7) / 8) * a.tiles_m * a.tiles_n;
        a.cr = a.split = 0;
        return a.lists * a.cw;
    }
    const long wide = (long)a.batch * a.tiles_m * a.wide_n, ragged = (long)a.batch * a.rag * a.tiles_m;
    a.cw = (int)((wide + a.lists - 1) / a.lists);
    a.cr = (int)((ragged + a.lists - 1) / a.lists);
    a.split = (narrow_ok && policy == 2) ? a.cw : 0;
    return a.lists * (a.cw + a.split + a.cr);
}

template <bool A_KC, bool B_KC, int EPI, bool TAIL, int TM>
static int gccnmf_launch_gemm_dma_tm(GemmArgs a, hipStream_t stream) {
#ifdef GEMM_DMA_NO_NARROW
    constexpr bool NARROW = false;
#else
    constexpr bool NARROW = TM == 4 && (EPI == EPI_DIV || EPI == EPI_UPDH || EPI == EPI_STORE);
#endif
    const int classic_grid = gemm_dma_plan(a, NARROW, TM);
    if (classic_grid < 1) return GCCNMF_ERR_ARG;
    a.trace = gccnmf_trace_buf;
    a.trace_rows = gccnmf_trace_buf ? gccnmf_trace_blocks : 0;
    a.trace_grid = classic_grid;
    a.tickets = nullptr;
    a.prefetch = 0;
    a.wpl = 0;
    int grid = classic_grid;
#ifdef GCCNMF_EXPERIMENTS
    a.prefetch = gccnmf_tune_prefetch;
    if (gccnmf_tune_persistent && TM == 4 && classic_grid > 512) {
        a.tickets = gccnmf_ticket_block(stream);
        if (a.tickets) {
            grid = 512;
            a.wpl = 512 / a.lists;
        }
    }
#endif
    hipLaunchKernelGGL((gccnmf_gemm_dma_kernel<A_KC, B_KC, EPI, TAIL, TM, NARROW>), dim3(grid), dim3(256), 0, stream, a);
    GCCNMF_CHECK_LAUNCH();
    return GCCNMF_OK;
}

template <bool A_KC, bool B_KC, int EPI, bool TAIL>
static int gccnmf_launch_gemm_dma(GemmArgs a, hipStream_t stream) {
    if (!a.A || !a.B || !a.C || a.M < 1 || a.N < 1 || a.Kd < 1 || a.batch < 1) return GCCNMF_ERR_ARG;
    if ((a.lda & 3) || (a.ldb & 3)) return GCCNMF_ERR_ARG;
    a.ablate = gccnmf_tune_ablate;
    a.exact_div = gccnmf_tune_exact_div;
    if constexpr (EPI != EPI_UPDW) {
        if ((a.M <= 256 && gccnmf_tune_tail_split != 0) || gccnmf_tune_tail_split == 3) return gccnmf_launch_gemm_dma_tm<A_KC, B_KC, EPI, TAIL, 2>(a, stream);
        const long tpf = (long)gccnmf_ceil_div(a.M, 512) * gccnmf_ceil_div(a.N, 64);
        const long total = tpf * a.batch, rounds = total / 512;
        if (gccnmf_tune_tail_split == 1 && !gccnmf_trace_buf && !a.concurrent && a.M > 256) {
            auto full_cost = [](long tiles) { const long r = tiles % 512; return (tiles / 512) * 250 + (r == 0 ? 0 : r <= 256 ? 135 : 250); };
            auto half_cost = [](long halves) {
                const long r = halves % 768;
                return (halves / 768) * 190 + (r == 0 ? 0 : r <= 256 ? 85 : r <= 512 ? 135 : 190);
            };
            const long plain = full_cost(total), all_half = half_cost(2 * total);
            long split = 1L << 40;
            const int head = (int)(rounds * 512 / tpf);
            const int rest = a.batch - head;
            if (rounds >= 1 && head >= 8 && rest >= 1 && 2 * rest * tpf <= 768) split = full_cost(head * tpf) + half_cost(2 * rest * tpf) + 10;
            if (all_half < plain && all_half <= split) return gccnmf_launch_gemm_dma_tm<A_KC, B_KC, EPI, TAIL, 2>(a, stream);
            if (split < plain) {
                GemmArgs h = a, t = a;
                h.batch = head;
                t.batch = rest;
                t.file0 = a.file0 + head;
                int rc = gccnmf_launch_gemm_dma_tm<A_KC, B_KC, EPI, TAIL, 4>(h, stream);
                if (rc) return rc;
                return gccnmf_launch_gemm_dma_tm<A_KC, B_KC, EPI, TAIL, 2>(t, stream);
            }
        }
    }
    return gccnmf_launch_gemm_dma_tm<A_KC, B_KC, EPI, TAIL, 4>(a, stream);
}
```

gcc_nmf_amd/csrc/nmf.hip:

```cpp
#include <mutex>
#include "gemm_ring.h"
#include "direct.h"
#include "update_w.h"
#include "divergence.h"
#ifdef GCCNMF_EXPERIMENTS
int gccnmf_launch_gemm_stream(GemmArgs a, hipStream_t stream);
#endif
int gccnmf_klnmf_fixed_launch(const float* V, const float* W, float* H, float* workspace, int F, int N, int K, int batch, int iterations,
                              float alpha, float eps, bool ones, hipStream_t s);
bool gccnmf_klnmf_fixed_supported(int F, int K);
long gccnmf_klnmf_fixed_workspace_floats(int F, int K);
bool gccnmf_klnmf_semi_supported(int F, int K, int nfree);
int gccnmf_klnmf_semi_rht_launch(const float* R, const float* H, float* U, float* rowsumH, int F, int N, int K, int nfree, int batch, hipStream_t s);
int gccnmf_klnmf_semi_update_w_launch(float* W, const float* U, const float* rowsumH, float* colsumW, float* hscale, int F, int K, int nfree,
                                      int batch, hipStream_t s);
#include "../../include/gccnmf_hip.h"

#include <atomic>
#include <algorithm>
#include <vector>
#define GCCNMF_SHARED_STREAMS 4
#define GCCNMF_CHAIN_MAX_ITERATIONS gccnmf_tune_chain_chunk
#define GCCNMF_RAGGED_MAX_BATCH 248
#define GCCNMF_SPLITS 4
#define GCCNMF_DIRECT_MAX_BATCH 8
struct GccNmfKnob {
    int def, lo, hi, experiment;
};
static const GccNmfKnob gccnmf_knobs[GCCNMF_TUNE_KEYS] = {
    {0, 0, 0, 1},
    {0, 0, 1 << 30, 1},
    {0, 0, 2, 0},
    {1, 0, 1, 0},
    {1, 0, 1, 1},
    {3, 1, 4, 1},
    {4, 1, 4, 1},
    {1, 0, 1, 0},
    {3, 1, GCCNMF_SHARED_STREAMS, 0},
    {1, 0, 3, 0},
    {1, 0, 1, 0},
    {0, 0, 8, 1},
    {4, 1, GCCNMF_DIRECT_MAX_BATCH, 0},
    {0, 0, 4, 1},
    {1, 0, 1, 1},
    {1, 0, 1, 1},
    {1, 0, 2, 0},
    {1, 0, 2, 0},
    {0, 0, 1, 1},
    {1, 0, 1, 1},
    {1, 0, 1, 1},
    {1, 0, 8, 0},
    {0, 0, 1, 1},
    {1, 0, 3, 0},
    {2048, 1, 65536, 0},
    {0, 0, 1, 1},
};
static std::atomic<int> gccnmf_knob_value[GCCNMF_TUNE_KEYS];
static std::atomic<int> gccnmf_knobs_ready{0};
static void gccnmf_knobs_init() {
    static std::mutex mu;
    if (gccnmf_knobs_ready.load(std::memory_order_acquire)) return;
    std::lock_guard<std::mutex> lock(mu);
    if (gccnmf_knobs_ready.load(std::memory_order_relaxed)) return;
    for (int k = 0; k < GCCNMF_TUNE_KEYS; ++k) gccnmf_knob_value[k].store(gccnmf_knobs[k].def, std::memory_order_relaxed);
    gccnmf_knobs_ready.store(1, std::memory_order_release);
}
static GccNmfTune gccnmf_tune_load() {
    gccnmf_knobs_init();
    GccNmfTune t;
    for (int k = 0; k < GCCNMF_TUNE_KEYS; ++k) t.v[k] = gccnmf_knob_value[k].load(std::memory_order_relaxed);
    return t;
}
thread_local GccNmfTune gccnmf_tune = gccnmf_tune_load();
static thread_local int gccnmf_call_depth = 0;
GccNmfCall::GccNmfCall() {
    if (gccnmf_call_depth++ == 0) gccnmf_tune = gccnmf_tune_load();
}
GccNmfCall::~GccNmfCall() { --gccnmf_call_depth; }
long long* gccnmf_trace_buf = nullptr;
int gccnmf_trace_blocks = 0;

extern "C" {
int gccnmf_version(void) { return 106; }

int gccnmf_set_tuning(int key, int value) {
    GCCNMF_ENTER();
    gccnmf_knobs_init();
    if (key < 1 || key >= GCCNMF_TUNE_KEYS) return GCCNMF_ERR_ARG;
    const GccNmfKnob& k = gccnmf_knobs[key];
#ifndef GCCNMF_EXPERIMENTS
    if (k.experiment) return GCCNMF_ERR_ARG;
#endif
    if (value < k.lo || value > k.hi || (key == 13 && value == 1) || (key == 21 && value != 0 && value != 1 && value != 2 && value != 4 && value != 8)) return GCCNMF_ERR_ARG;
    gccnmf_knob_value[key].store(value, std::memory_order_relaxed);
    return GCCNMF_OK;
}

}

#ifdef GCCNMF_EXPERIMENTS
unsigned* gccnmf_ticket_block(hipStream_t stream) {
    constexpr int MAX_DEV = 16, PER_DEV = 128;
    struct Entry { hipStream_t s; };
    static std::mutex mu;
    static unsigned* pool[MAX_DEV] = {};
    static Entry entries[MAX_DEV][PER_DEV];
    static int used[MAX_DEV] = {};
    int dev = 0;
    if (hipGetDevice(&dev) != hipSuccess || dev < 0 || dev >= MAX_DEV) return nullptr;
    std::lock_guard<std::mutex> lock(mu);
    for (int i = 0; i < used[dev]; ++i)
        if (entries[dev][i].s == stream) return pool[dev] + 16 * i;
    if (used[dev] == PER_DEV) return nullptr;
    if (!pool[dev]) {
        static const unsigned zeros[16 * PER_DEV] = {};
        unsigned* p = nullptr;
        if (hipMalloc((void**)&p, sizeof(zeros)) != hipSuccess) {
            (void)hipGetLastError();
            return nullptr;
        }
        if (hipMemcpy(p, zeros, sizeof(zeros), hipMemcpyHostToDevice) != hipSuccess) {
            (void)hipGetLastError();
            (void)hipFree(p);
            return nullptr;
        }
        pool[dev] = p;
    }
    entries[dev][used[dev]].s = stream;
    return pool[dev] + 16 * used[dev]++;
}

#endif

extern "C" {
#ifdef GCCNMF_EXPERIMENTS
int gccnmf_debug_set_trace(long long* buf, int blocks) {
    GCCNMF_ENTER();
    gccnmf_trace_buf = buf;
    gccnmf_trace_blocks = buf ? blocks : 0;
    return GCCNMF_OK;
}

#endif

int gccnmf_pitches(int F, int T, int K, int* Fp, int* Kp, int* Np, int* Tp) {
    GCCNMF_ENTER();
    if (F < 2 || T < 1 || K < 1 || !Fp || !Kp || !Np || !Tp) return GCCNMF_ERR_ARG;
    GccNmfPitches p = gccnmf_make_pitches(F, T, K);
    *Fp = p.Fp;
    *Kp = p.Kp;
    *Np = p.Np;
    *Tp = p.Tp;
    return GCCNMF_OK;
}
}

#ifdef GCCNMF_EXPERIMENTS
__global__ __launch_bounds__(256, 2) void mfma_peak_kernel(float* out, int iters) {
    f32x16 acc[8];
#pragma unroll
    for (int i = 0; i < 8; ++i)
#pragma unroll
        for (int r = 0; r < 16; ++r) acc[i][r] = 0.f;
    float a = 1.0f + threadIdx.x * 1e-3f, b = 0.5f;
    for (int it = 0; it < iters; ++it) {
#pragma unroll
        for (int i = 0; i < 8; ++i) acc[i] = __builtin_amdgcn_mfma_f32_32x32x2f32(a, b, acc[i], 0, 0, 0);
    }
    float s = 0.f;
#pragma unroll
    for (int i = 0; i < 8; ++i)
#pragma unroll
        for (int r = 0; r < 16; ++r) s += acc[i][r];
    if (s == 123.456f) out[0] = s;
}
#endif

__global__ __launch_bounds__(256) void nmf_prepare_kernel(const float* __restrict__ W, float* __restrict__ colsumW,
                                                          float* __restrict__ hscale, int F, int Fp, int Kp) {
    __shared__ float red[4][16];
    const int chunks = Kp / 16;
    const int b = blockIdx.x / chunks, ch = blockIdx.x - b * chunks;
    const int c = threadIdx.x & 15, q = threadIdx.x >> 4, wave = threadIdx.x >> 6;
    const int k = ch * 16 + c;
    const float* Wb = W + (long)b * Fp * Kp;
    float s = 0.f;
#pragma unroll 4
    for (int f = q; f < F; f += 16) s += Wb[(long)f * Kp + k];
    s += __shfl_xor(s, 16);
    s += __shfl_xor(s, 32);
    if ((threadIdx.x & 63) < 16) red[wave][c] = s;
    __syncthreads();
    if (threadIdx.x < 16) {
        colsumW[(long)b * Kp + k] = (red[0][c] + red[1][c]) + (red[2][c] + red[3][c]);
        hscale[(long)b * Kp + k] = 1.f;
    }
}

template <int AT>
__global__ __launch_bounds__(256) void nmf_update_w_kernel(float* __restrict__ W, const float* __restrict__ U,
                                                           const float* __restrict__ rowsumH, float* __restrict__ colsumW,
                                                           float* __restrict__ hscale, int F, int Fp, int K, int Kp,
                                                           long sW, long sU, long sVec, long sRowsum, int nsplit, long sSplitU,
                                                           long sSplitR) {
    constexpr int PH = 256 / AT;
    __shared__ float red[256];
    __shared__ float s_norm[AT];
    const int chunks = Kp / AT;
// ... 638 lines not shown
    else hipLaunchKernelGGL((gccnmf_gemm_chain_kernel<true, 4, 2>), dim3(grid), dim3(256), pad, s, a[0], a[1], a[2], a[3], ch);
    GCCNMF_CHECK_LAUNCH();
    return GCCNMF_OK;
}

static int short_chain_group(const NmfGeom& g, int batch, const KlnmfMode& m) {
    const int want = gccnmf_tune_chain;
    if (!want || want == 2 || want == 4 || !gccnmf_tune_fused_k12 || !gccnmf_tune_fused_k34 || gccnmf_tune_tile_policy != 0) return 0;
    if (direct_path(g, batch, m.groups) || !m.xcd_affine || m.unfused_w_update || batch < 8 || !g.tail || g.Fm < 64 || g.Fm > 512 || (g.Fm % 64) != 0 || g.K > 128) return 0;
    if ((g.Fm / 64) * 16 < 32 * gccnmf_ceil_div(g.K, 32) || g.F > 64 * 9 || !gccnmf_tune_ring || (long)batch * (g.Kp / 64) >= 256) return 0;
    if (want == 1 && !(chain_rule(batch, m) && fused_wh_updh(g, batch, m) && fused_whdiv_rht_files(g, batch, m) == batch)) return 0;
    if (gccnmf_tune_ablate == 64) return 0;
    return ((long)batch * (g.Kp / 32) >= 256 && gccnmf_tune_wide_update_w) ? 32 : 16;
}

static int launch_short_chain(const NmfGeom& g, const float* V, float* W, float* H, const KlnmfWorkspace& ws, float alpha, float eps, int batch,
                              int group, int it0, int iterations, hipStream_t s) {
    ShortChainArgs c = {};
    c.a12 = wh_updh_args(g, V, W, H, ws.hscale, ws.colsumW, alpha, eps, batch);
    c.a34 = whdiv_rht_args(g, V, W, H, ws.U, ws.rowsumH, batch);
    c.aw = update_w_args(g, W, g.sW, ws.U, g.sU, ws.rowsumH, ws.colsumW, ws.hscale, g.Kp);
    c.it0 = it0; c.iterations = iterations; c.atoms_per_group = group; c.solo = gccnmf_tune_chain_solo;
    c.counters = ws.c12;
    c.error = ws.status;
    c.xcc_seen = ws.xcc_seen;
    c.timeout = gccnmf_tune_chain_fault ? 0 : GEMM_SYNC_TIMEOUT;
    return gccnmf_short_chain_launch(c, s);
}

__global__ void nmf_chain_poison_kernel(const unsigned* __restrict__ err, float* __restrict__ W, float* __restrict__ H, long nW, long nH) {
    bool bad = err[0] != 0u;
    for (int l = 0; l < 8; ++l) bad = bad || __popc(err[GCCNMF_STATUS_XCC_SEEN + l]) > 1;
    if (!bad) return;
    const float nan = __int_as_float(0x7fc00000);
    for (long i = blockIdx.x * 256L + threadIdx.x; i < nW; i += 256L * gridDim.x) W[i] = nan;
    for (long i = blockIdx.x * 256L + threadIdx.x; i < nH; i += 256L * gridDim.x) H[i] = nan;
}

extern "C" {

long gccnmf_klnmf_workspace_floats(int F, int N, int K, int batch) {
    GCCNMF_ENTER();
    if (F < 2 || N < 1 || K < 1 || batch < 1) return -1;
    return carve(nullptr, make_geom(F, N, K), batch, false).floats;
}

static int klnmf_stage(int stage, const float* V, float* W, float* H, const KlnmfWorkspace& ws, const NmfGeom& g, int batch, float alpha, float eps,
                       const KlnmfMode& m, hipStream_t s) {
    float *R = ws.R, *U = ws.U, *colsumW = ws.colsumW, *rowsumH = ws.rowsumH, *hscale = ws.hscale;
    if (stage == 7) {
        return gccnmf_kl_divergence_launch(V, W, m.fixed_w ? 0 : g.sW, H, g.F, g.N, g.K, g.Fp, g.Kp, g.Np, batch, (double*)R, g.sV / 2, (double*)U, s);
    }
    const int nfree = m.free_atoms;
    const bool semi = nfree > 0;
    const bool fused12 = fused_wh_updh(g, batch, m);
    const int head34 = semi ? 0 : fused_whdiv_rht_files(g, batch, m), rest34 = batch - head34;
    const bool fused34 = head34 > 0;
    const int groups = m.groups;
    if (!semi && stage != 6 && direct_path(g, batch, groups)) {
        const DirectBufs d = direct_bufs(g, ws.direct_base, batch);
        switch (stage) {
            case 0: {
                if (hipMemsetAsync(R, 0, sizeof(float) * batch * g.sV, s) != hipSuccess) return GCCNMF_ERR_LAUNCH;
                if (hipMemsetAsync(d.Wt, 0, sizeof(float) * direct_floats(g, batch), s) != hipSuccess) return GCCNMF_ERR_LAUNCH;
                hipLaunchKernelGGL(nmf_prepare_kernel, dim3(batch * (g.Kp / 16)), dim3(256), 0, s, W, colsumW, hscale, g.F, g.Fp, g.Kp);
                GCCNMF_CHECK_LAUNCH();
                return gccnmf_transpose_launch(W, g.sW, g.Kp, d.Wt, d.sWt, d.ldwt, g.F, g.Kp, batch, s);
            }
            case 1: return direct_wh_div(g, d, V, W, H, hscale, R, false, batch, s);
            case 2: return direct_update_h(g, d, W, R, H, hscale, colsumW, alpha, eps, batch, s);
            case 3: return direct_wh_div(g, d, V, W, H, nullptr, R, true, batch, s);
            case 4: return direct_rht(g, d, R, U, rowsumH, batch, s);
            case 5: return launch_update_w(update_w_args(g, W, g.sW, U, g.sU, rowsumH, colsumW, hscale, g.Kp), batch, groups, s, 1, 0, 0, d.Wt, d.sWt, d.ldwt);
            default: return GCCNMF_ERR_ARG;
        }
    }
#ifdef GCCNMF_EXPERIMENTS
    const bool split_wh = !semi && single_file_split(g, batch, g.Kp, gccnmf_tune_wh_splits);
    const bool split_rht = !semi && single_file_split(g, batch, g.Np, gccnmf_tune_rht_splits);
#else
    constexpr bool split_rht = false;
#endif
    const int xa = m.xcd_affine, conc = m.groups > 1 ? m.groups : 0;
    const int vec_grid = batch * (g.Kp / 16);
    switch (stage) {
        case 0:
            if (hipMemsetAsync(R, 0, sizeof(float) * batch * g.sV, s) != hipSuccess) return GCCNMF_ERR_LAUNCH;
            hipLaunchKernelGGL(nmf_prepare_kernel, dim3(vec_grid), dim3(256), 0, s, W, colsumW, hscale, g.F, g.Fp, g.Kp);
            break;
        case 1:
            if (fused12) return gccnmf_wh_updh_launch(wh_updh_args(g, V, W, H, hscale, colsumW, alpha, eps, batch), s);
#ifdef GCCNMF_EXPERIMENTS
            if (split_wh) return launch_wh_div_split(g, V, W, H, hscale, ws.parts, R, s);
#endif
            return launch_wh_div(g, wh_div_args(g, V, W, g.sW, H, hscale, g.Kp, R, batch, xa, conc), s);
        case 2:
            if (fused12) return GCCNMF_OK;
            return launch_update_h(update_h_args(g, W, g.sW, R, H, hscale, g.Kp, colsumW, g.Kp, alpha, eps, batch, xa, conc), s);
        case 3:
            if (fused34) {
                const int rc = gccnmf_whdiv_rht_launch(whdiv_rht_args(g, V, W, H, U, rowsumH, head34), s);
                if (rc || !rest34) return rc;
                return launch_wh_div(g, wh_div_args(g, V + head34 * g.sV, W + head34 * g.sW, g.sW, H + head34 * g.sH, nullptr, 0, R + head34 * g.sV, rest34, xa, conc), s);
            }
#ifdef GCCNMF_EXPERIMENTS
            if (split_wh) return launch_wh_div_split(g, V, W, H, nullptr, ws.parts, R, s);
#endif
            return launch_wh_div(g, wh_div_args(g, V, W, g.sW, H, nullptr, 0, R, batch, xa, conc), s);
        case 4:
            if (semi) return gccnmf_klnmf_semi_rht_launch(R, H, U, rowsumH, g.F, g.N, g.K, nfree, batch, s);
            if (fused34)
                return rest34 ? launch_rht(g, rht_args(g, R + head34 * g.sV, H + head34 * g.sH, U + head34 * g.sU, rowsumH + (long)head34 * g.Kp, rest34, xa, conc), s)
                              : GCCNMF_OK;
#ifdef GCCNMF_EXPERIMENTS
            if (split_rht) return launch_rht_split(g, R, H, ws.parts, ws.rowsum_parts, s);
#endif
            if (can_fuse_w_update(g, batch, groups) && !m.unfused_w_update)
                return launch_rht_update_w(g, rht_update_w_args(g, R, H, W, colsumW, hscale, batch, xa, conc), s);
            return launch_rht(g, rht_args(g, R, H, U, rowsumH, batch, xa, conc), s);
        case 5:
            if (semi) return gccnmf_klnmf_semi_update_w_launch(W, U, rowsumH, colsumW, hscale, g.F, g.K, nfree, batch, s);
            if (split_rht)
                return launch_update_w(update_w_args(g, W, g.sW, ws.parts, g.sU, ws.rowsum_parts, colsumW, hscale, g.Kp), batch, 1, s, gccnmf_tune_rht_splits,
                                       g.sU, (long)g.Kp, nullptr, 0, 0);
            if (can_fuse_w_update(g, batch, groups) && !m.unfused_w_update && !fused34) return GCCNMF_OK;
            return launch_update_w(update_w_args(g, W, g.sW, U, g.sU, rowsumH, colsumW, hscale, g.Kp), batch, groups, s, 1, 0, 0, nullptr, 0, 0);
        case 6:
            hipLaunchKernelGGL(nmf_scale_h_kernel, dim3(batch * g.K), dim3(256), 0, s, H, hscale, (long)g.Kp, g.K, g.sH, g.ld, g.Np);
            break;
        default: return GCCNMF_ERR_ARG;
    }
    GCCNMF_CHECK_LAUNCH();
    return GCCNMF_OK;
}

static int clear_chain_status(const KlnmfWorkspace& ws, hipStream_t s) {
    return hipMemsetAsync(ws.status, 0, GCCNMF_STATUS_WORDS * sizeof(unsigned), s) == hipSuccess ? GCCNMF_OK : GCCNMF_ERR_LAUNCH;
}
static int zero_chain_counters(const KlnmfWorkspace& ws, hipStream_t s) {
    return hipMemsetAsync(ws.c12, 0, sizeof(unsigned) * ws.counter_words, s) == hipSuccess ? GCCNMF_OK : GCCNMF_ERR_LAUNCH;
}
static int finish_call(bool chained, const float* V, float* W, float* H, const KlnmfWorkspace& ws, const NmfGeom& g, int batch, float alpha, float eps,
                       const KlnmfMode& m, hipStream_t s) {
    if (chained) {
        hipLaunchKernelGGL(nmf_chain_poison_kernel, dim3(64), dim3(256), 0, s, ws.status, W, H, (long)batch * g.sW, (long)batch * g.sH);
        GCCNMF_CHECK_LAUNCH();
    }
    return klnmf_stage(6, V, W, H, ws, g, batch, alpha, eps, m, s);
}

int gccnmf_klnmf_plan(int F, int N, int K, int batch, int flags) {
    GCCNMF_ENTER();
    if (F < 2 || N < 1 || K < 1 || batch < 1) return -1;
    KlnmfMode m;
    if (decode_mode(flags, F, K, m)) return -1;
    if (m.fixed_w) return gccnmf_klnmf_fixed_supported(F, K) ? 16 : -1;
    if (m.free_atoms) return 32;
    const NmfGeom g = make_geom(F, N, K);
    return (direct_path(g, batch, m.groups) ? 1 : 0) | (fused_wh_updh(g, batch, m) ? 2 : 0) | (fused_whdiv_rht_files(g, batch, m) > 0 ? 4 : 0) |
           ((chain_stages(g, batch, m) || short_chain_group(g, batch, m)) ? 8 : 0);
}

int gccnmf_klnmf_stage(const float* V, float* W, float* H, float* workspace, int F, int N, int K, int batch,
                       float sparsity_alpha, float epsilon, int flags, int stage, void* stream) {
    GCCNMF_ENTER();
    if (!V || !W || !H || !workspace || F < 2 || N < 1 || K < 1 || batch < 1) return GCCNMF_ERR_ARG;
    if (!workspace_aligned(workspace)) return GCCNMF_ERR_ARG;
    KlnmfMode m;
    if (const int rc = decode_mode(flags, F, K, m)) return rc;
    if (m.fixed_w && (stage != 7 || m.h_ones)) return GCCNMF_ERR_ARG;
    const NmfGeom g = make_geom(F, N, K);
    return klnmf_stage(stage, V, W, H, carve(workspace, g, batch, false), g, batch, sparsity_alpha, epsilon, m, (hipStream_t)stream);
}

int gccnmf_klnmf(const float* V, float* W, float* H, float* workspace, int F, int N, int K, int batch, int iterations,
                 float sparsity_alpha, float epsilon, int flags, void* stream) {
    GCCNMF_ENTER();
    if (!V || !W || !H || !workspace || F < 2 || N < 1 || K < 1 || batch < 1 || iterations < 0) return GCCNMF_ERR_ARG;
    if (!workspace_aligned(workspace)) return GCCNMF_ERR_ARG;
    hipStream_t s = (hipStream_t)stream;
    KlnmfMode m;
    int rc;
    if ((rc = decode_mode(flags, F, K, m))) return rc;
    const NmfGeom g = make_geom(F, N, K);
    const KlnmfWorkspace ws = carve(workspace, g, batch, false);
    const float alpha = sparsity_alpha, eps = epsilon;
    if (m.free_atoms) {
        if ((rc = clear_chain_status(ws, s))) return rc;
        if ((rc = klnmf_stage(0, V, W, H, ws, g, batch, alpha, eps, m, s))) return rc;
        for (int it = 0; it < iterations; ++it)
            for (int stage = 1; stage <= 5; ++stage)
                if ((rc = klnmf_stage(stage, V, W, H, ws, g, batch, alpha, eps, m, s))) return rc;
        return finish_call(false, V, W, H, ws, g, batch, alpha, eps, m, s);
    }
    if (m.fixed_w) {
        if (!gccnmf_klnmf_fixed_supported(F, K) || gccnmf_klnmf_fixed_workspace_floats(F, K) > ws.scratch_floats) return GCCNMF_ERR_UNSUPPORTED;
        if ((rc = clear_chain_status(ws, s))) return rc;
        return gccnmf_klnmf_fixed_launch(V, W, H, workspace, F, N, K, batch, iterations, alpha, eps, m.h_ones, s);
    }
    if ((rc = klnmf_stage(0, V, W, H, ws, g, batch, alpha, eps, m, s))) return rc;
    const int chained = chain_stages(g, batch, m);
    const int short_group = chained ? 0 : short_chain_group(g, batch, m);
    const bool chains = (chained || short_group) && iterations > 0;
    if (!chained && !short_group && (rc = clear_chain_status(ws, s))) return rc;
    if (chains && (rc = zero_chain_counters(ws, s))) return rc;
    if (short_group) {
        for (int it0 = 0; it0 < iterations; it0 += GCCNMF_CHAIN_MAX_ITERATIONS)
            if ((rc = launch_short_chain(g, V, W, H, ws, alpha, eps, batch, short_group, it0, std::min(GCCNMF_CHAIN_MAX_ITERATIONS, iterations - it0), s))) return rc;
    } else if (chained == 8) {
        for (int it0 = 0; it0 < iterations; it0 += GCCNMF_CHAIN_MAX_ITERATIONS)
            if ((rc = launch_klnmf_chain(4, g, V, W, H, ws, alpha, eps, batch, m, it0, std::min(GCCNMF_CHAIN_MAX_ITERATIONS, iterations - it0), s, nullptr))) return rc;
    } else {
        for (int it = 0; it < iterations; ++it) {
            if (chained && (rc = launch_klnmf_chain(chained, g, V, W, H, ws, alpha, eps, batch, m, it, 1, s, nullptr))) return rc;
            for (int stage = chained + 1; stage <= 5; ++stage)
                if ((rc = klnmf_stage(stage, V, W, H, ws, g, batch, alpha, eps, m, s))) return rc;
        }
    }
    return finish_call(chains, V, W, H, ws, g, batch, alpha, eps, m, s);
}

int gccnmf_klnmf_chain_status(const float* workspace, int F, int N, int K, int batch, int* status) {
    GCCNMF_ENTER();
    if (!workspace || !status || F < 2 || N < 1 || K < 1 || batch < 1) return GCCNMF_ERR_ARG;
    const KlnmfWorkspace ws = carve(const_cast<float*>(workspace), make_geom(F, N, K), batch, false);
    unsigned host[GCCNMF_STATUS_WORDS];
    if (hipMemcpy(host, ws.status, sizeof(host), hipMemcpyDeviceToHost) != hipSuccess) return GCCNMF_ERR_LAUNCH;
    int st = host[0] ? 1 : 0;
    for (int l = 0; l < 8; ++l)
        if (__builtin_popcount(host[GCCNMF_STATUS_XCC_SEEN + l]) > 1) st |= 2;
    *status = st;
    return GCCNMF_OK;
}

struct RaggedTables {
    int v[GCCNMF_RAGGED_MAX_BATCH + 8 * (GEMM_RAGGED_LMAX + 1)];
};
__global__ void nmf_store_ragged_tables_kernel(RaggedTables t, int* dst, int n) {
    for (int i = threadIdx.x; i < n; i += blockDim.x) dst[i] = t.v[i];
}

long gccnmf_klnmf_ragged_workspace_floats(int F, int Nmax, int K, int batch) {
    GCCNMF_ENTER();
    if (F < 2 || Nmax < 1 || K < 1 || batch < 1 || batch > GCCNMF_RAGGED_MAX_BATCH) return -1;
    return carve(nullptr, make_geom(F, Nmax, K), batch, true).floats;
}

int gccnmf_klnmf_ragged(const float* V, float* W, float* H, float* workspace, int F, const int* N, int Nmax, int K, int batch, int iterations,
                        float sparsity_alpha, float epsilon, int flags, void* stream) {
    GCCNMF_ENTER();
    if (!V || !W || !H || !workspace || !N || F < 2 || Nmax < 1 || K < 1 || batch < 1 || iterations < 0) return GCCNMF_ERR_ARG;
    KlnmfMode m;
    if (decode_mode(flags, F, K, m) || m.fixed_w || m.free_atoms) return GCCNMF_ERR_ARG;
    m.groups = 1;
    if (!workspace_aligned(workspace)) return GCCNMF_ERR_ARG;
    if (batch > GCCNMF_RAGGED_MAX_BATCH) return GCCNMF_ERR_UNSUPPORTED;
    long tiles = 0;
    for (int f = 0; f < batch; ++f) {
        if (N[f] < 1 || N[f] > Nmax) return GCCNMF_ERR_ARG;
        tiles += gccnmf_ceil_div(N[f], 64);
    }
    hipStream_t s = (hipStream_t)stream;
    const NmfGeom g = make_geom(F, Nmax, K);
    if (!gccnmf_tune_chain || !chain_capable(g, batch, m, true) || (gccnmf_tune_tile_policy != 1 && tiles < 256)) return GCCNMF_ERR_UNSUPPORTED;
    RaggedPlan rg = {};
    rg.n = N;
    std::vector<int> order(batch);
    for (int f = 0; f < batch; ++f) order[f] = f;
    std::stable_sort(order.begin(), order.end(), [&](int x, int y) { return N[x] > N[y]; });
    long load[8] = {};
    for (int f : order) {
        int best = 0;
        for (int l = 1; l < 8; ++l)
            if (load[l] < load[best]) best = l;
        int& cnt = rg.lists[best][0];
        if (cnt >= GEMM_RAGGED_LMAX) return GCCNMF_ERR_UNSUPPORTED;
        rg.lists[best][1 + cnt++] = f;
        load[best] += gccnmf_ceil_div(N[f], 64);
    }
    for (int l = 0; l < 8; ++l) std::sort(rg.lists[l] + 1, rg.lists[l] + 1 + rg.lists[l][0]);
    const KlnmfWorkspace ws = carve(workspace, g, batch, true);
    RaggedTables t = {};
    for (int f = 0; f < batch; ++f) t.v[f] = N[f];
    for (int l = 0; l < 8; ++l)
        for (int k = 0; k <= GEMM_RAGGED_LMAX; ++k) t.v[batch + l * (GEMM_RAGGED_LMAX + 1) + k] = rg.lists[l][k];
    hipLaunchKernelGGL(nmf_store_ragged_tables_kernel, dim3(1), dim3(256), 0, s, t, ws.ragged_tables, batch + 8 * (GEMM_RAGGED_LMAX + 1));
    GCCNMF_CHECK_LAUNCH();
    rg.d_n = ws.ragged_tables;
    rg.d_lists = ws.ragged_tables + batch;
    int rc;
    if ((rc = klnmf_stage(0, V, W, H, ws, g, batch, sparsity_alpha, epsilon, m, s))) return rc;
    if (iterations > 0) {
        if ((rc = zero_chain_counters(ws, s))) return rc;
        for (int it0 = 0; it0 < iterations; it0 += GCCNMF_CHAIN_MAX_ITERATIONS)
            if ((rc = launch_klnmf_chain(4, g, V, W, H, ws, sparsity_alpha, epsilon, batch, m, it0, std::min(GCCNMF_CHAIN_MAX_ITERATIONS, iterations - it0), s, &rg)))
                return rc;
    }
    return finish_call(iterations > 0, V, W, H, ws, g, batch, sparsity_alpha, epsilon, m, s);
}

struct SharedShard {
    const float* V;
    float *H, *R, *Upart, *rowsum_part;
    float *parts, *rowsum_parts;
    bool latency;
    bool direct;
// ... 377 lines not shown
```

gcc_nmf_amd/engine.py:

```python
import ctypes
import functools
import warnings

import numpy as np
import torch

from . import _hip
from ._hip import (_ptr, _stream, klnmf_divergence, check_gcc_phat_nl, check_tdoa_tracking, check_reconstruction,
                   GCCNMF_FLAG_FIXED_W, GCCNMF_FLAG_H_ONES, GCCNMF_RECONSTRUCT_RATIO, RECONSTRUCTIONS, RATIO_MAX_TARGETS)

SPEED_OF_SOUND_IN_METRES_PER_SECOND = 340.29


def _on_device(method):
    @functools.wraps(method)
    def wrapper(self, *args, **kwargs):
        with torch.cuda.device(self.device):
            return method(self, *args, **kwargs)
    return wrapper


def num_frames(n_samples, n_fft, hop):
    return 1 + int((n_samples - n_fft) / hop)

# ... 103 lines not shown
                                           [Hd], numIterations, tolerance, checkEvery)
        H = Hd[:, :K, :N].cpu().numpy()
    checks = check_iterations(trace, checkEvery, numIterations)
    if single:
        return H[0], dict(iterations=int(iterations[0]), divergences=[(it, float(d[0])) for it, d in zip(checks, trace)])
    return H, dict(iterations=iterations, divergences=[(it, d.copy()) for it, d in zip(checks, trace)])


def fft_twiddles(n_fft):
    k = np.arange(n_fft // 2, dtype=np.float64)
    tw = np.exp(-2j * np.pi * k / n_fft).astype(np.complex64)
    return np.ascontiguousarray(tw).view(np.float32)


def steering_tables(frequenciesInHz, tdoasInSeconds, Fp, Dp):
    E = np.exp(np.outer(np.asarray(frequenciesInHz, np.float64), -(2j * np.pi) * np.asarray(tdoasInSeconds, np.float64)))
    F, D = E.shape
    trig = np.zeros((2, Fp, Dp), np.float32)
    trig[0, :F, :D] = E.real
    trig[1, :F, :D] = -E.imag
    return trig


class Geometry(object):

    def __init__(self, F, T, K, D=1, S=1):
        vals = [ctypes.c_int() for _ in range(4)]
        _hip.check(_hip.lib().gccnmf_pitches(F, T, K, *[ctypes.byref(v) for v in vals]), 'gccnmf_pitches')
        self.F, self.T, self.K, self.D, self.S = F, T, K, D, S
        self.N = 2 * T
        self.Fp, self.Kp, self.Np, self.Tp = [v.value for v in vals]
        self.Dp = -(-D // 64) * 64


def padded(host, shape, device, dtype=torch.float32):
    t = torch.zeros(shape, dtype=dtype, device=device)
    src = torch.from_numpy(np.ascontiguousarray(host))
    idx = tuple(slice(0, n) for n in host.shape)
    t[idx] = src.to(device)
    return t


class GCCNMFEngine(object):

    def __new__(cls, n_samples=None, *args, **kwargs):
        if cls is GCCNMFEngine and kwargs.get('lengths') is not None:
            kwargs = dict(kwargs)
            if kwargs.pop('numFreeAtoms', 0):
                raise ValueError('numFreeAtoms is not available with lengths= (the ragged engine has no semi-supervised form)')
            return RaggedGCCNMFEngine(kwargs.pop('lengths'), *args, **kwargs)
        return super(GCCNMFEngine, cls).__new__(cls)

    def __init__(self, n_samples, sampleRate=16000, windowSize=1024, hopSize=256, numTDOAs=128,
                 microphoneSeparationInMetres=1.0, numTargets=3, dictionarySize=None, numIterations=100,
                 sparsityAlpha=0, epsilon=1e-16, seedValue=0, batch=1, windowFunction=np.hanning,
                 device='cuda:0', klnmf_flags=0, nmf_groups=None, dictionaryW=None, initialH='random', reconstruction='direct',
                 gccPHATNLEnabled=False, gccPHATNLAlpha=2.0, tdoaTracking=False, localizationWindowSize=None, tolerance=None, checkEvery=10,
                 numFreeAtoms=0, maxTargets=None, spatialIterations=0):
        self.autoTargets, numTargets = _hip.check_auto_targets(numTargets, maxTargets, tdoaTracking)
        if initialH not in ('random', 'ones'):
            raise ValueError("initialH must be 'random' or 'ones'")
        self.initialH = initialH
        if numFreeAtoms and dictionaryW is None:
            raise ValueError('numFreeAtoms needs dictionaryW (without a dictionary every atom is free: dictionarySize)')
        if numFreeAtoms and initialH == 'ones':
            raise ValueError("numFreeAtoms cannot be combined with initialH='ones'")
        self.tolerance, self.checkEvery, numIterations = _hip.check_convergence(tolerance, checkEvery, numIterations)
        self.iterations_used = self.divergence_trace = None
        self.tdoaTracking, self.localizationWindowSize = check_tdoa_tracking(tdoaTracking, localizationWindowSize, numTargets)
        self.reconstruction = check_reconstruction(reconstruction, numTargets)
        self.spatialIterations = _hip.check_spatial_iterations(spatialIterations, self.reconstruction)
        if self.reconstruction == 'spatial':
            _hip.reconstruct_spatial_batch(batch)
        self.gccPHATNLEnabled, self.gccPHATNLAlpha = check_gcc_phat_nl(gccPHATNLEnabled, gccPHATNLAlpha)
        self.dictionaryW, self.numFreeAtoms = None, 0
        if dictionaryW is not None:
            self.dictionaryW = check_dictionary(dictionaryW, int(windowSize) // 2 + 1)
            self.numFreeAtoms = _hip.check_free_atoms(numFreeAtoms, self.dictionaryW.shape[1], int(windowSize) // 2 + 1)
            K = self.dictionaryW.shape[1] + self.numFreeAtoms
            if dictionarySize is not None and int(dictionarySize) != K:
                raise ValueError('dictionarySize %d conflicts with the %d atoms of dictionaryW%s' % (
                    dictionarySize, K, ' and the free atoms' if self.numFreeAtoms else ''))
            dictionarySize, nmf_groups = K, 1
        elif dictionarySize is None:
            dictionarySize = 128
        if not torch.cuda.is_available():
            raise _hip.HipLibraryError('no ROCm device visible: the GCC-NMF HIP path has no CPU fallback')
        self.lib = _hip.lib()
        self.device = torch.device(device)
        self.n_samples, self.sampleRate = int(n_samples), sampleRate
        self.n_fft, self.hop = int(windowSize), int(hopSize)
        self.iters, self.alpha, self.eps, self.seed = int(numIterations), float(sparsityAlpha), float(epsilon), seedValue
        self.batch = int(batch)
        self.d = microphoneSeparationInMetres
        self.klnmf_flags = klnmf_flags
        if nmf_groups is None:
            half = self.batch // 2
            tiles_wh = -(-(2 * num_frames(self.n_samples, self.n_fft, self.hop)) // 64)
            atoms = -(-int(dictionarySize) // 64)
            nmf_groups = 2 if (self.batch % 2 == 0 and half >= 16 and half * tiles_wh >= 256 and half * atoms >= 256) else 1
            Fq, Nq = int(windowSize) // 2 + 1, 2 * num_frames(self.n_samples, self.n_fft, self.hop)
            if nmf_groups > 1 and Nq > 0 and self.lib.gccnmf_klnmf_plan(Fq, Nq, int(dictionarySize), self.batch, klnmf_flags) & 8:
                nmf_groups = 1
        if nmf_groups < 1 or self.batch % nmf_groups:
            raise ValueError('nmf_groups must divide the batch')
        self.nmf_groups = int(nmf_groups)
        F = self.n_fft // 2 + 1
        T = num_frames(self.n_samples, self.n_fft, self.hop)
        if T < 2:
            raise ValueError('Buffer is too short (n=%d) for frame_length=%d' % (n_samples, self.n_fft))
        self.g = g = Geometry(F, T, int(dictionarySize), int(numTDOAs), int(numTargets))
        self.L = self.hop * (T - 1)
        dev, B = self.device, self.batch
        f32 = torch.float32

        with torch.cuda.device(dev):
            self.window = torch.from_numpy(np.asarray(windowFunction(self.n_fft), np.float64).astype(np.float32)).to(dev)
            self.twiddle = torch.from_numpy(fft_twiddles(self.n_fft)).to(dev)
            maxTDOA = self.d / SPEED_OF_SOUND_IN_METRES_PER_SECOND
            self.tdoasInSeconds = np.linspace(-maxTDOA, maxTDOA, g.D)
            self.frequenciesInHz = np.linspace(0, sampleRate / 2.0, F)
            self.trig = torch.from_numpy(steering_tables(self.frequenciesInHz, self.tdoasInSeconds, g.Fp, g.Dp)).to(dev)
            W0, H0 = klnmf_initial_factors(F, g.N, g.K, self.eps, seedValue)
            self.W0 = padded(W0, (g.Fp, g.Kp), dev)
            self.H0 = padded(H0, (g.Kp, g.Np), dev)

            z = lambda *shape: torch.zeros(shape, dtype=f32, device=dev)
            self.x = z(B, 2, self.n_samples)
            self.X = z(B, 2, g.Fp, g.Tp, 2)
            self.V = z(B, g.Fp, g.Np)
            self.CC = z(B, 2, g.Fp, g.Tp)
            self.W = z(B, g.Fp, g.Kp)
            self.H = z(B, g.Kp, g.Np)
            if self.numFreeAtoms:
                self.W0 = padded(semi_supervised_initial_factors(self.dictionaryW, self.numFreeAtoms, g.N, self.eps, seedValue)[0], (g.Fp, g.Kp), dev)
            elif self.dictionaryW is not None:
                self.W0 = padded(self.dictionaryW, (g.Fp, g.Kp), dev)
                self.W.copy_(self.W0.unsqueeze(0).expand_as(self.W))
            self.ws_nmf = z(self.nmf_groups * self.lib.gccnmf_klnmf_workspace_floats(F, g.N, g.K, B // self.nmf_groups))
            self.nmf_streams = [torch.cuda.Stream(device=dev) for _ in range(self.nmf_groups)] if self.nmf_groups > 1 else []
            self.copy_streams = [torch.cuda.Stream(device=dev) for _ in range(2)]
            self.ang = z(B, g.Dp, g.Tp)
            self.mean_ang = torch.zeros((B, g.Dp), dtype=torch.float64, device=dev)
            self.tdoa_idx = torch.zeros((B, g.S), dtype=torch.int32, device=dev)
            self.status = torch.zeros((B,), dtype=torch.int32, device=dev)
            if self.tdoaTracking:
                if T > _hip.TRACKS_MAX_FRAMES:
                    raise ValueError('tdoaTracking takes files of fewer than 2^21 frames, got %d' % T)
                self.tracks = torch.zeros((B, g.S, g.Tp), dtype=torch.int32, device=dev)
                self.track_status = torch.zeros((B, g.Tp), dtype=torch.int32, device=dev)
            self.ws_scores = z(self.lib.gccnmf_scores_workspace_floats(F, T, g.S, B))
            self.scores = z(B, g.Kp, g.S * g.Tp)
            self.argmax = torch.zeros((B, g.Kp, g.Tp), dtype=torch.uint8, device=dev)
            self.ws_rec = z(self._reconstruct_workspace_floats()) if self.reconstruction == 'direct' else None
            self.ws_cov = z(self._reconstruct_workspace_floats()) if self.reconstruction == 'spatial' else None
            self.spec = z(B, 2 * g.S, g.Fp, g.Tp, 2)
            self.frames = None
            self.fused_istft = self.n_fft + 3 * self.hop <= 2048 and self.hop <= self.n_fft and B * g.S * -(-T // 32) >= 256
            self.y = z(B, g.S, 2, self.L)
            self.pcm_in = None
            self.pcm_out = None

    @_on_device
    def stft(self):
        pcm = self.pcm_in is not None
        _hip.stft_stereo(self.pcm_in if pcm else self.x, self.n_samples, self.n_fft, self.hop, self.g.T, self.batch, self.window, self.twiddle,
                         self.X, self.V, self.CC, pcm16=pcm)

    @_on_device
    def pack_pcm16(self):
        g = self.g
        if self.pcm_out is None:
            self.pcm_out = torch.zeros((self.batch, g.S, self.L, 2), dtype=torch.int16, device=self.device)
            self.pcm_peak = torch.zeros((self.batch * g.S,), dtype=torch.int32, device=self.device)
        _hip.pack_pcm16(self.y, self.batch * g.S, self.L, self.pcm_peak, self.pcm_out)

    @_on_device
    def klnmf(self):
        if self.tolerance is None:
            self._klnmf_start()
            self._klnmf_iterate(self.iters, True)
            return
        for attempt in range(2):
            self._klnmf_start()
            if self._fixed() and self.initialH == 'ones':
                self.H[:, :self.g.K, :self.g.N] = 1
            try:
                self.iterations_used, self.divergence_trace = converge_klnmf(
                    self._klnmf_iterate, lambda: self._divergence().cpu().numpy(), [self.H] if self._fixed() else [self.W, self.H],
                    self.iters, self.tolerance, self.checkEvery, failed=self.chain_failed)
                return
            except ChainHandOverError:
                if attempt:
                    raise
                self._fall_back_to_plain_launches()

    def _fall_back_to_plain_launches(self):
        warnings.warn('gcc_nmf_amd: a chained KL-NMF launch did not hand over cleanly; this process falls back to the plain launches '
                      '(gccnmf_set_tuning(21, 0)) and repeats the batch', RuntimeWarning)
        _hip.check(self.lib.gccnmf_set_tuning(21, 0), 'gccnmf_set_tuning')

    def _fixed(self):
        return self.dictionaryW is not None and not self.numFreeAtoms

    def _klnmf_start(self):
        if self._fixed():
            if self.initialH != 'ones':
                self.H.copy_(self.H0.unsqueeze(0).expand_as(self.H))
            return
        self.W.copy_(self.W0.unsqueeze(0).expand_as(self.W))
        self.H.copy_(self.H0.unsqueeze(0).expand_as(self.H))

    def _groups(self):
        per, ws_per = self.batch // self.nmf_groups, self.ws_nmf.numel() // self.nmf_groups
        for i in range(self.nmf_groups):
            yield i * per, per, self.ws_nmf[i * ws_per:], self.nmf_streams[i] if self.nmf_streams else None

    def _divergence(self):
        g = self.g
        fixed = self._fixed()
        out = [klnmf_divergence(self.V[b0], self.W0 if fixed else self.W[b0], self.H[b0], ws, g.F, g.N, g.K, per, fixed)
               for b0, per, ws, _ in self._groups()]
        return out[0] if len(out) == 1 else torch.cat(out)

    @_on_device
    def get_divergence(self):
        return self._divergence().cpu().numpy()

    def get_iterations(self):
        if self.tolerance is None or self.iterations_used is None:
            raise ValueError('get_iterations needs tolerance= and a klnmf() run')
        return self.iterations_used.copy()

    def get_divergence_trace(self):
        if self.tolerance is None or self.divergence_trace is None:
            raise ValueError('get_divergence_trace needs tolerance= and a klnmf() run')
        return self.divergence_trace.copy()

    def _klnmf_iterate(self, iters, first):
        g = self.g
        fixed = self._fixed()
        if self.nmf_groups > 1:
            main = torch.cuda.current_stream(self.device)
            ready = torch.cuda.Event()
            ready.record(main)
        for b0, per, ws, st in self._groups():
            if st is not None:
                st.wait_event(ready)
            _hip.klnmf(self.V[b0], self.W0 if fixed else self.W[b0], self.H[b0], ws, g.F, g.N, g.K, per, iters, self.alpha, self.eps,
                       fixed_w=fixed, h_ones=fixed and first and self.initialH == 'ones', groups=self.nmf_groups,
                       flags=0 if fixed else self.klnmf_flags, free_atoms=self.numFreeAtoms, stream=None if st is None else st.cuda_stream)
            if st is not None:
                done = torch.cuda.Event()
                done.record(st)
                main.wait_event(done)

    @_on_device
    def localize(self):
        g = self.g
        _hip.angular_spectrogram(self.CC, self.trig, g.F, g.T, g.D, self.batch, self.ang, self.mean_ang,
                                 nl_alpha=self.gccPHATNLAlpha if self.gccPHATNLEnabled else None)
        if self.autoTargets:
            _hip.count_tdoa_peaks(self.mean_ang, g.D, g.Dp, g.S, self.batch, self.tdoa_idx, self.status)
            return
        _hip.pick_tdoa_peaks(self.mean_ang, g.D, g.Dp, g.S, self.batch, self.tdoa_idx, self.status)
        if self.tdoaTracking:
            _hip.pick_tdoa_tracks(self.ang, g.D, g.T, g.S, self.localizationWindowSize, self.batch, self.tracks, self.track_status)

    @_on_device
    def masks(self):
        g = self.g
        if self.autoTargets:
            _hip.target_scores_masks_counted(self.CC, self.trig, self.tdoa_idx, self.W, g.F, g.T, g.K, g.D, g.S, self.batch, self.ws_scores,
                                             self.scores, self.argmax, counted=True)
            return
        _hip.target_scores_masks(self.CC, self.trig, self.tracks if self.tdoaTracking else self.tdoa_idx, self.W, g.F, g.T, g.K, g.D, g.S,
                                 self.batch, self.ws_scores, self.scores, self.argmax, tracks=self.tdoaTracking)

    def _reconstruct_workspace_floats(self):
        g = self.g
        return _hip.reconstruct_workspace_floats(self.reconstruction, g.T, g.K, g.S, self.batch, g.Fp, self.spatialIterations)

    def _reconstruct_workspace(self):
        if self.reconstruction != 'spatial':
            _hip.check_spatial_iterations(self.spatialIterations, self.reconstruction)
            return self.ws_rec
        need = self._reconstruct_workspace_floats()
        if self.ws_cov is None or self.ws_cov.numel() < need:
            self.ws_cov = torch.zeros(need, dtype=torch.float32, device=self.device)
        return self.ws_cov

    @_on_device
    def reconstruct(self):
        g = self.g
        _hip.reconstruct(self.W, self.H, self.argmax, None, self.X, self.V, g.F, g.T, g.K, g.S, self.batch, self.spec, mode=self.reconstruction,
                         workspace=self._reconstruct_workspace(), iterations=self.spatialIterations)

    @_on_device
    def istft(self, keep_frames=False):
        g = self.g
        gain = np.float32(self.hop / float(self.n_fft) * 2)
        frames = None
        if keep_frames or not self.fused_istft:
            if self.frames is None:
                self.frames = torch.zeros((self.batch, 2 * g.S, g.T, self.n_fft), dtype=torch.float32, device=self.device)
            frames = self.frames
        _hip.istft_ola(self.spec, 2 * g.S, self.n_fft, self.hop, g.T, self.batch, self.window, self.twiddle, gain, True, frames, self.y)

    @_on_device
    def run(self, stft=True):
        if stft:
            self.stft()
        self.klnmf()
        self.localize()
        self.masks()
        self.reconstruct()
        self.istft()

    def _checked_samples(self, stereoSamples, one_file=True):
        x = np.asarray(stereoSamples, dtype=np.float32)
        if one_file and x.ndim == 2:
            x = x[None]
        if x.shape != tuple(self.x.shape):
            raise ValueError('expected samples of shape %s, got %s' % (tuple(self.x.shape), x.shape))
        if not np.isfinite(x).all():
            raise ValueError('Audio buffer is not finite everywhere')
        return x

    @_on_device
    def upload(self, stereoSamples):
        x = self._checked_samples(stereoSamples)
        self.pcm_in = None
        self.x.copy_(torch.from_numpy(np.ascontiguousarray(x)))

    @_on_device
    def upload_pcm16(self, pcm):
        pcm = np.asarray(pcm)
        if pcm.ndim == 2:
            pcm = pcm[None]
        if pcm.dtype != np.int16 or pcm.shape != (self.batch, self.n_samples, 2):
            raise ValueError('expected int16 frames of shape %s, got %s %s' % ((self.batch, self.n_samples, 2), pcm.dtype, pcm.shape))
        if self.pcm_in is None:
            self.pcm_in = torch.zeros((self.batch, self.n_samples, 2), dtype=torch.int16, device=self.device)
        self.pcm_in.copy_(torch.from_numpy(np.ascontiguousarray(pcm)))

    @_on_device
    def separate_pcm16(self, pcm):
        self.upload_pcm16(pcm)
        self.run()
        self.pack_pcm16()
        out = self.pcm_out.cpu().numpy()
        self.check_status()
        self.check_pcm_finite()
        return out

    @_on_device
    def separate(self, stereoSamples):
        x = self._checked_samples(stereoSamples)
        if getattr(self, '_pin', None) is None:
            self._pin = (torch.zeros(self.x.shape, dtype=torch.float32).pin_memory(), torch.zeros(self.y.shape, dtype=torch.float32).pin_memory())
        hx, hy = self._pin
        hx.copy_(torch.from_numpy(np.ascontiguousarray(x)))
        self.pcm_in = None
        self.x.copy_(hx, non_blocking=True)
        self.run()
        if self.chain_failed():
            self._fall_back_to_plain_launches()
            self.run(stft=False)
        hy.copy_(self.y, non_blocking=True)
        torch.cuda.current_stream(self.device).synchronize()
        self.check_status()
        return hy.numpy().copy()

    def separate_batches(self, batches):
        dev = self.device
        g = self.g
        with torch.cuda.device(dev):
            compute = torch.cuda.current_stream(dev)
            s_in, s_out = self.copy_streams
            if getattr(self, '_pipe', None) is None:
                self._pipe = dict(x=torch.zeros_like(self.x), y=torch.zeros_like(self.y),
                                  hx=[torch.zeros(self.x.shape, dtype=torch.float32).pin_memory() for _ in range(2)],
                                  hy=[torch.zeros(self.y.shape, dtype=torch.float32).pin_memory() for _ in range(2)],
                                  hs=[torch.zeros(self.status.shape, dtype=self.status.dtype).pin_memory() for _ in range(2)],
                                  ds=[torch.zeros_like(self.status) for _ in range(2)])
            xs, ys = [self.x, self._pipe['x']], [self.y, self._pipe['y']]
            hx, hy, status = self._pipe['hx'], self._pipe['hy'], self._pipe['hs']
            ev_in = [torch.cuda.Event() for _ in range(2)]
            ev_done = [torch.cuda.Event() for _ in range(2)]
            ev_out = [torch.cuda.Event() for _ in range(2)]
            ev_stft = torch.cuda.Event()
            pending = []
            download = None

            def collect(slot):
                ev_out[slot].synchronize()
                st = status[slot].numpy()
                if st.any():
                    raise ValueError(self._too_few_peaks(st))
                return hy[slot].numpy().copy()

            try:
                for i, batch in enumerate(batches):
                    slot = i & 1
                    if len(pending) == 2:
                        yield collect(pending.pop(0))
                    x = self._checked_samples(batch, one_file=False)
                    hx[slot].copy_(torch.from_numpy(np.ascontiguousarray(x)))
                    with torch.cuda.stream(s_in):
                        s_in.wait_event(ev_done[slot])
                        xs[slot].copy_(hx[slot], non_blocking=True)
                        ev_in[slot].record(s_in)
                    compute.wait_event(ev_in[slot])
                    compute.wait_event(ev_out[slot])
                    self.x, self.y, self.pcm_in = xs[slot], ys[slot], None
                    self.stft()
                    if download is not None:
                        ev_stft.record(compute)
                        download(ev_stft)
                    self.run(stft=False)
                    self._pipe['ds'][slot].copy_(self.file_status())
                    ev_done[slot].record(compute)

                    def download(after=None, slot=slot):
                        with torch.cuda.stream(s_out):
                            s_out.wait_event(ev_done[slot])
                            if after is not None:
                                s_out.wait_event(after)
                            hy[slot].copy_(ys[slot], non_blocking=True)
                            status[slot].copy_(self._pipe['ds'][slot], non_blocking=True)
                            ev_out[slot].record(s_out)
                    pending.append(slot)
                if download is not None:
                    download()
                while pending:
                    yield collect(pending.pop(0))
            finally:
                torch.cuda.synchronize(dev)
# ... 24 lines not shown
            raise ValueError(self._too_few_peaks(st))

    @_on_device
    def _chain_status(self):
        g = self.g
        torch.cuda.current_stream(self.device).synchronize()
        worst = 0
        for _, per, ws, _ in self._groups():
            worst |= _hip.klnmf_chain_status(ws, g.F, g.N, g.K, per)
        return worst

    chain_failed = _chain_status

    def check_chain_status(self):
        st = self._chain_status()
        if st:
            raise _hip.HipLibraryError('the chained KL-NMF launch did not hand over cleanly (status %d: %s): W and H of this batch are NaN.  '
                                       'GCCNMF_TUNE="21=0" runs the plain launches.'
                                       % (st, 'a consumer timed out' if st & 1 else 'a work list ran on more than one XCC'))

    def get_X(self):
        g = self.g
        return torch.view_as_complex(self.X)[:, :, :g.F, :g.T].cpu().numpy()

    def get_V(self):
        g = self.g
        return self.V[:, :g.F, :g.N].cpu().numpy()

    def get_C(self):
        g = self.g
        c = self.CC[:, :, :g.F, :g.T].cpu().numpy()
        return (c[:, 0] + 1j * c[:, 1]).astype(np.complex64)

    def get_WH(self):
        g = self.g
        return self.W[:, :g.F, :g.K].cpu().numpy(), self.H[:, :g.K, :g.N].cpu().numpy()

    def get_angular(self):
        g = self.g
        return self.ang[:, :g.D, :g.T].cpu().numpy(), self.mean_ang[:, :g.D].cpu().numpy()

    def get_tdoa_indexes(self):
        return self.tdoa_idx.cpu().numpy()

    def get_num_sources(self):
        if not self.autoTargets:
            return np.full((self.batch,), self.g.S, dtype=np.int64)
        return (self.tdoa_idx >= 0).sum(dim=1).cpu().numpy().astype(np.int64)

    def get_count_status(self):
        if not self.autoTargets:
            raise ValueError("get_count_status needs numTargets='auto'")
        return self.status.cpu().numpy()

    def get_tdoa_tracks(self):
        if not self.tdoaTracking:
            raise ValueError('get_tdoa_tracks needs tdoaTracking=True')
        return self.tracks[:, :, :self.g.T].cpu().numpy()

    def get_track_status(self):
        if not self.tdoaTracking:
            raise ValueError('get_track_status needs tdoaTracking=True')
        return self.track_status[:, :self.g.T].cpu().numpy()

    def get_scores(self):
        g = self.g
        s = self.scores.view(self.batch, g.Kp, g.S, g.Tp)[:, :g.K, :, :g.T]
        return s.permute(0, 2, 1, 3).contiguous().cpu().numpy()

    def get_argmax(self):
        g = self.g
        return self.argmax[:, :g.K, :g.T].cpu().numpy()

    def get_spec(self):
        g = self.g
        s = torch.view_as_complex(self.spec)[:, :, :g.F, :g.T].cpu().numpy()
        return s.reshape(self.batch, g.S, 2, g.F, g.T)


def check_enhancement_target_index(targetTDOAIndex, batch, numTDOAs):
    if targetTDOAIndex is None:
        return None
    tg = np.asarray(targetTDOAIndex)
    if tg.ndim not in (0, 1) or tg.dtype.kind not in 'iuf' or (tg.ndim == 1 and tg.shape[0] != int(batch)):
        raise ValueError('targetTDOAIndex must be None, one index or one index per file (%d), got shape %s' % (batch, tg.shape))
    if not np.isfinite(tg).all() or not np.array_equal(tg, np.round(tg)) or tg.min() < 0 or tg.max() >= int(numTDOAs):
        raise ValueError('targetTDOAIndex must be whole numbers in [0, %d), got %r' % (numTDOAs, targetTDOAIndex))
    return np.ascontiguousarray(np.broadcast_to(tg, (int(batch),)), dtype=np.int32)


class GCCNMFEnhancementEngine(GCCNMFEngine):

    def __init__(self, n_samples, *args, **kwargs):
        if 'numTargets' in kwargs:
            raise TypeError('GCCNMFEnhancementEngine takes no numTargets keyword: its outputs are the talker and the noise')
        if kwargs.pop('lengths', None) is not None:
            raise ValueError('GCCNMFEnhancementEngine has no ragged form: lengths= is not available')
        names = ('sampleRate', 'windowSize', 'hopSize', 'numTDOAs', 'microphoneSeparationInMetres')
        if len(args) > len(names):
            raise TypeError('GCCNMFEnhancementEngine takes at most %d positional arguments besides n_samples' % len(names))
        kwargs.update(zip(names, args))
        self.targetMode, self.targetTDOAEpsilon, self.targetTDOABeta, self.targetTDOANoiseFloor = _hip.check_enhancement_target(
            kwargs.pop('targetMode', 'boxcar'), kwargs.pop('targetTDOAEpsilon', 5.0), kwargs.pop('targetTDOABeta', 2.0),
            kwargs.pop('targetTDOANoiseFloor', 0.0))
        numTDOAs = int(kwargs.get('numTDOAs', 128))
        if not 3 <= numTDOAs <= _hip.ATOM_TDOA_MAX_D:
            raise ValueError('enhancement takes 3 to %d TDOAs, got %d' % (_hip.ATOM_TDOA_MAX_D, numTDOAs))
        fixed = check_enhancement_target_index(kwargs.pop('targetTDOAIndex', None), kwargs.get('batch', 1), numTDOAs)
        super(GCCNMFEnhancementEngine, self).__init__(n_samples, numTargets=2, **kwargs)
        g, B, dev = self.g, self.batch, self.device
        with torch.cuda.device(dev):
            self.scores = self.ws_scores = None
            self.fixedTargetTDOAIndex = fixed is not None
            self.tdoa_idx = torch.zeros((B, 1), dtype=torch.int32, device=dev)
            if fixed is not None:
                self.tdoa_idx.copy_(torch.from_numpy(fixed).view(B, 1))
            if self.tdoaTracking:
                self.tracks = torch.zeros((B, 1, g.Tp), dtype=torch.int32, device=dev)
            self.atom_tdoa = torch.zeros((B, g.Kp, g.Tp), dtype=torch.int16, device=dev)
            self.soft_masks = torch.zeros((B, 2, g.Kp, g.Tp), dtype=torch.float32, device=dev) if self.targetMode else None

    def _per_frame(self):
        return self.tdoaTracking and not self.fixedTargetTDOAIndex

    @_on_device
    def localize(self):
        g = self.g
        _hip.angular_spectrogram(self.CC, self.trig, g.F, g.T, g.D, self.batch, self.ang, self.mean_ang,
                                 nl_alpha=self.gccPHATNLAlpha if self.gccPHATNLEnabled else None)
        if self.fixedTargetTDOAIndex:
            return
        _hip.pick_tdoa_peaks(self.mean_ang, g.D, g.Dp, 1, self.batch, self.tdoa_idx, self.status)
        if self.tdoaTracking:
            _hip.pick_tdoa_tracks(self.ang, g.D, g.T, 1, self.localizationWindowSize, self.batch, self.tracks, self.track_status)

    def file_status(self):
        if self.fixedTargetTDOAIndex:
            return torch.zeros_like(self.status)
        return super(GCCNMFEnhancementEngine, self).file_status()

    @_on_device
    def masks(self):
        g = self.g
        _hip.atom_tdoa_indexes(self.CC, self.trig, self.W, g.F, g.T, g.K, g.D, self.batch, self.atom_tdoa)
        _hip.enhancement_masks(self.atom_tdoa, self.tracks if self._per_frame() else self.tdoa_idx, g.T, g.K, self.batch,
                               None if self.targetMode else self.argmax, self.soft_masks, window=self.targetMode,
                               eps=self.targetTDOAEpsilon, beta=self.targetTDOABeta, noise_floor=self.targetTDOANoiseFloor,
                               per_frame=self._per_frame())

    @_on_device
    def reconstruct(self):
        g = self.g
        _hip.reconstruct(self.W, self.H, None if self.targetMode else self.argmax, self.soft_masks, self.X, self.V, g.F, g.T, g.K, 2,
                         self.batch, self.spec, mode=self.reconstruction, workspace=self._reconstruct_workspace(),
                         iterations=self.spatialIterations)

    def get_atom_tdoa_indexes(self):
        g = self.g
        return (self.atom_tdoa[:, :g.K, :g.T].to(torch.int32) & 0xffff).cpu().numpy()

    def get_enhancement_masks(self):
        g = self.g
        if self.targetMode:
            return self.soft_masks[:, :, :g.K, :g.T].cpu().numpy()
        noise = self.argmax[:, :g.K, :g.T].to(torch.float32)
        return torch.stack([1 - noise, noise], dim=1).cpu().numpy()


class RaggedGCCNMFEngine(object):

    def __init__(self, lengths, sampleRate=16000, windowSize=1024, hopSize=256, numTDOAs=128, microphoneSeparationInMetres=1.0,
                 numTargets=3, dictionarySize=None, numIterations=100, sparsityAlpha=0, epsilon=1e-16, seedValue=0,
                 windowFunction=np.hanning, device='cuda:0', klnmf_flags=0, dictionaryW=None, initialH='random', reconstruction='direct',
                 gccPHATNLEnabled=False, gccPHATNLAlpha=2.0, tdoaTracking=False, localizationWindowSize=None, tolerance=None, checkEvery=10,
                 maxTargets=None, spatialIterations=0):
        self.tolerance, self.checkEvery, numIterations = _hip.check_convergence(tolerance, checkEvery, numIterations)
        self.autoTargets, slots = _hip.check_auto_targets(numTargets, maxTargets, tdoaTracking)
        self.reconstruction = check_reconstruction(reconstruction, slots)
        self.spatialIterations = _hip.check_spatial_iterations(spatialIterations, self.reconstruction)
        self.gccPHATNLEnabled, self.gccPHATNLAlpha = check_gcc_phat_nl(gccPHATNLEnabled, gccPHATNLAlpha)
        self.tdoaTracking, self.localizationWindowSize = check_tdoa_tracking(tdoaTracking, localizationWindowSize, slots)
        if not torch.cuda.is_available():
            raise _hip.HipLibraryError('no ROCm device visible: the GCC-NMF HIP path has no CPU fallback')
        self.lib = _hip.lib()
        self.device = torch.device(device)
        self.lengths = [int(n) for n in lengths]
        if not self.lengths:
            raise ValueError('no files')
        self.batch = len(self.lengths)
        self.iters, self.alpha, self.eps = int(numIterations), float(sparsityAlpha), float(epsilon)
        self.klnmf_flags = klnmf_flags
        kw = dict(sampleRate=sampleRate, windowSize=windowSize, hopSize=hopSize, numTDOAs=numTDOAs,
                  microphoneSeparationInMetres=microphoneSeparationInMetres, numTargets=numTargets, dictionarySize=dictionarySize,
                  numIterations=numIterations, sparsityAlpha=sparsityAlpha, epsilon=epsilon, seedValue=seedValue,
                  windowFunction=windowFunction, device=device, klnmf_flags=klnmf_flags, dictionaryW=dictionaryW, initialH=initialH,
                  reconstruction=reconstruction, gccPHATNLEnabled=gccPHATNLEnabled, gccPHATNLAlpha=gccPHATNLAlpha,
                  tdoaTracking=tdoaTracking, localizationWindowSize=localizationWindowSize,
                  tolerance=tolerance, checkEvery=checkEvery, maxTargets=maxTargets, spatialIterations=spatialIterations)
        self.files_of = {}
        for i, n in enumerate(self.lengths):
            self.files_of.setdefault(n, []).append(i)
        self.sub = dict((n, GCCNMFEngine(n, batch=len(idx), nmf_groups=1, **kw)) for n, idx in sorted(self.files_of.items()))
        longest = self.sub[max(self.sub)]
        self.g = g = longest.g
        self.N = [self.sub[n].g.N for n in self.lengths]
        self.frames = [self.sub[n].g.T for n in self.lengths]
        with torch.cuda.device(self.device):
            z = lambda *shape: torch.zeros(shape, dtype=torch.float32, device=self.device)
            self.ragged = None
            if len(self.sub) > 1 and dictionaryW is None and self.tolerance is None:
                ws = self.lib.gccnmf_klnmf_ragged_workspace_floats(g.F, g.N, g.K, self.batch)
                if ws > 0:
                    self.ragged = dict(V=z(self.batch, g.Fp, g.Np), W=z(self.batch, g.Fp, g.Kp), H=z(self.batch, g.Kp, g.Np), ws=z(ws),
                                       N=(ctypes.c_int * self.batch)(*self.N))
        self.ragged_klnmf_used = None

    def klnmf(self):
        with torch.cuda.device(self.device):
            r = self.ragged
            if r is not None:
                g = self.g
                for n, e in self.sub.items():
                    idx = torch.as_tensor(self.files_of[n], device=self.device)
                    r['V'][idx, :, :e.g.Np] = e.V
                    r['W'][idx] = e.W0
                    r['H'][idx, :, :e.g.Np] = e.H0
                rc = self.lib.gccnmf_klnmf_ragged(_ptr(r['V']), _ptr(r['W']), _ptr(r['H']), _ptr(r['ws']), g.F, r['N'], g.N, g.K, self.batch,
                                                  self.iters, self.alpha, self.eps, self.klnmf_flags, _stream())
                if rc == 0:
                    self._ragged_ran = True
                    for n, e in self.sub.items():
                        idx = torch.as_tensor(self.files_of[n], device=self.device)
                        e.W.copy_(r['W'][idx])
                        e.H.copy_(r['H'][idx, :, :e.g.Np])
                    self.ragged_klnmf_used = True
                    return
                if rc != 3:
                    _hip.check(rc, 'gccnmf_klnmf_ragged')
            self.ragged_klnmf_used = False
            for e in self.sub.values():
                e.klnmf()

    def run(self, stft=True):
        if stft:
            for e in self.sub.values():
                e.stft()
        self.klnmf()
        for e in self.sub.values():
            e.localize()
            e.masks()
            e.reconstruct()
            e.istft()

    def upload(self, mixtures):
        if len(mixtures) != self.batch:
            raise ValueError('expected %d mixtures' % self.batch)
        for n, e in self.sub.items():
            e.upload(np.stack([np.asarray(mixtures[i], dtype=np.float32) for i in self.files_of[n]]))

    def separate(self, mixtures):
        self.upload(mixtures)
        self.run()
        out = [None] * self.batch
        if self.ragged_klnmf_used:
            torch.cuda.current_stream(self.device).synchronize()
            st = _hip.klnmf_chain_status(self.ragged['ws'], self.g.F, self.g.N, self.g.K, self.batch)
            if st:
                raise _hip.HipLibraryError('the ragged chained KL-NMF launch did not hand over cleanly (status %d): W and H are NaN' % st)
        for n, e in self.sub.items():
            y = e.y.cpu().numpy()
            e.check_status()
            for k, i in enumerate(self.files_of[n]):
                out[i] = y[k]
        return out

    def _per_file(self, values):
        return [values[n][self.files_of[n].index(i)] for i, n in enumerate(self.lengths)]

    def get_divergence(self):
        return np.array(self._per_file(dict((n, e.get_divergence()) for n, e in self.sub.items())), dtype=np.float64)

    def get_iterations(self):
        return np.array(self._per_file(dict((n, e.get_iterations()) for n, e in self.sub.items())), dtype=np.int64)

    def get_divergence_trace(self):
        return self._per_file(dict((n, e.get_divergence_trace().T) for n, e in self.sub.items()))

    def get_num_sources(self):
        return np.array(self._per_file(dict((n, e.get_num_sources()) for n, e in self.sub.items())), dtype=np.int64)

    def get_tdoa_tracks(self):
        return self._per_file(dict((n, e.get_tdoa_tracks()) for n, e in self.sub.items()))

    def get_track_status(self):
        return self._per_file(dict((n, e.get_track_status()) for n, e in self.sub.items()))

    def file(self, i):
        n = self.lengths[i]
        return self.sub[n], self.files_of[n].index(i)
```

include/gccnmf_hip.h:

```cpp
#ifndef GCCNMF_HIP_H
#define GCCNMF_HIP_H

#ifdef __cplusplus
extern "C" {
#endif

#define GCCNMF_OK 0
#define GCCNMF_ERR_ARG 1
#define GCCNMF_ERR_LAUNCH 2
#define GCCNMF_ERR_UNSUPPORTED 3
#define GCCNMF_ERR_COLLECTIVE 4

#define GCCNMF_FLAG_NO_XCD_AFFINITY 1
#define GCCNMF_FLAG_UNFUSED_W_UPDATE 2
#define GCCNMF_FLAG_CONCURRENT_GROUPS 4
#define GCCNMF_FLAG_GROUPS(n) (GCCNMF_FLAG_CONCURRENT_GROUPS | ((n) << 8))
#define GCCNMF_FLAG_FIXED_W (1 << 16)
#define GCCNMF_FLAG_H_ONES (1 << 17)

#define GCCNMF_FLAG_FREE_ATOMS(n) ((n) << 18)

int gccnmf_version(void);

int gccnmf_set_tuning(int key, int value);

int gccnmf_pitches(int F, int T, int K, int* Fp, int* Kp, int* Np, int* Tp);

int gccnmf_stft_stereo(const float* x, long x_stride, int n_samples, int n_fft, int hop, int T, int batch,
                       const float* window, const float* twiddle, float* X, float* V, float* CC, void* stream);

long gccnmf_dft_workspace_floats(int n_fft, int T, int nsig);
int gccnmf_stft_dft(const float* x, long x_stride, int n_samples, int n_fft, int hop, int T, int nsig, const float* basis,
                    float* workspace, float* X, void* stream);
int gccnmf_istft_dft(const float* spec, int nsig, int n_fft, int hop, int T, const float* ibasis, float gain, int center, float* workspace,
                     float* y, void* stream);

int gccnmf_stft_stereo_pcm16(const short* pcm, long frame_stride, int n_samples, int n_fft, int hop, int T, int batch,
                             const float* window, const float* twiddle, float* X, float* V, float* CC, void* stream);

int gccnmf_pack_pcm16(const float* y, int groups, int L, unsigned int* peak_scratch, short* pcm, void* stream);

long gccnmf_klnmf_workspace_floats(int F, int N, int K, int batch);
int gccnmf_klnmf(const float* V, float* W, float* H, float* workspace, int F, int N, int K, int batch,
                 int iterations, float sparsity_alpha, float epsilon, int flags, void* stream);

long gccnmf_klnmf_ragged_workspace_floats(int F, int Nmax, int K, int batch);
int gccnmf_klnmf_ragged(const float* V, float* W, float* H, float* workspace, int F, const int* N, int Nmax, int K, int batch,
                        int iterations, float sparsity_alpha, float epsilon, int flags, void* stream);

int gccnmf_klnmf_chain_status(const float* workspace, int F, int N, int K, int batch, int* status);

int gccnmf_klnmf_plan(int F, int N, int K, int batch, int flags);

int gccnmf_klnmf_stage(const float* V, float* W, float* H, float* workspace, int F, int N, int K, int batch,
                       float sparsity_alpha, float epsilon, int flags, int stage, void* stream);

long gccnmf_klnmf_shared_workspace_floats(int F, int N, int K, int batch);
long gccnmf_klnmf_shared_partial_floats(int F, int K);
int gccnmf_klnmf_shared_begin(const float* W, float* workspace, int F, int N, int K, int batch, void* stream);
int gccnmf_klnmf_shared_step_a(const float* V, const float* W, float* H, float* workspace, float* partial, int F,
                               int N, int K, int batch, float sparsity_alpha, float epsilon, void* stream);
int gccnmf_klnmf_shared_step_b(float* W, float* workspace, const float* partial, int F, int N, int K, int batch,
                               void* stream);
int gccnmf_klnmf_shared_finish(float* H, float* workspace, int F, int N, int K, int batch, void* stream);

#define GCCNMF_MAX_SHARDS 8
typedef struct gccnmf_shared_shard {
    const float* V;
    float* H;
    float* workspace;
    int N, batch, ld;
} gccnmf_shared_shard;
typedef int (*gccnmf_allreduce_fn)(void* ctx, float* buf, long count, void* stream);
long gccnmf_klnmf_shared_shard_workspace_floats(int F, int N, int K, int batch, int ld);
int gccnmf_klnmf_shared_run(const gccnmf_shared_shard* shards, int nshards, float* W, float* partial, float* vec, int F, int K,
                            int iterations, float sparsity_alpha, float epsilon, gccnmf_allreduce_fn allreduce, void* allreduce_ctx,
                            void* stream);

#define GCCNMF_RCCL_UNIQUE_ID_BYTES 128
int gccnmf_rccl_available(void);
int gccnmf_rccl_unique_id(char* id_bytes);
int gccnmf_rccl_comm_init(const char* id_bytes, int world_size, int rank, void** comm);
int gccnmf_rccl_comm_destroy(void* comm);
int gccnmf_rccl_allreduce(void* comm, float* buf, long count, void* stream);
gccnmf_allreduce_fn gccnmf_rccl_allreduce_hook(void);

#define GCCNMF_ANGULAR_NL_D(D, alpha_bits) ((int)((unsigned)(D) | ((unsigned)(alpha_bits) & 0xffff0000u)))
#define GCCNMF_ANGULAR_NL_BATCH(batch, alpha_bits) ((int)((unsigned)(batch) | ((unsigned)(alpha_bits) << 16)))
int gccnmf_angular_spectrogram(const float* CC, const float* trig, int F, int T, int D, int batch, float* ang,
                               double* mean_ang, void* stream);

#define GCCNMF_PEAKS_TRACKS_BIT 0x100
#define GCCNMF_PEAKS_TRACKS(S, L) ((S) | GCCNMF_PEAKS_TRACKS_BIT | ((L) << 9))
#define GCCNMF_PEAKS_COUNT_BIT (1 << 30)
#define GCCNMF_PEAKS_COUNT(Smax) ((Smax) | GCCNMF_PEAKS_COUNT_BIT)
int gccnmf_pick_tdoa_peaks(const double* mean_ang, int D, int Dp, int S, int batch, int* tdoa_idx, int* status,
                           void* stream);

#define GCCNMF_SCORES_TRACKS 0x100
#define GCCNMF_SCORES_ATOM_TDOA 0x200
#define GCCNMF_SCORES_ENHANCEMENT_MASKS 0x400
#define GCCNMF_SCORES_COUNTED 0x800
#define GCCNMF_ATOM_TDOA_INDEXES(CC, trig, W, F, T, K, D, batch, atom_tdoa, atom_score, stream)                                          \
    gccnmf_target_scores_masks(CC, trig, 0, W, F, T, K, D, GCCNMF_SCORES_ATOM_TDOA, batch, 0, atom_score, (unsigned char*)(atom_tdoa), stream)
#define GCCNMF_ENHANCEMENT_MASKS(atom_tdoa, target, per_frame, window, params, T, K, batch, image, masks, stream)                        \
    gccnmf_target_scores_masks((const float*)(atom_tdoa), params, target, 0, 0, T, K, 0,                                                 \
                               GCCNMF_SCORES_ENHANCEMENT_MASKS | (window) | ((per_frame) ? GCCNMF_SCORES_TRACKS : 0), batch, 0, masks,   \
                               image, stream)
long gccnmf_scores_workspace_floats(int F, int T, int S, int batch);
int gccnmf_target_scores_masks(const float* CC, const float* trig, const int* tdoa_idx, const float* W, int F,
                               int T, int K, int D, int S, int batch, float* workspace, float* scores,
                               unsigned char* argmax, void* stream);

int gccnmf_argmax_targets(const float* scores, int K, int T, int S, int batch, unsigned char* argmax, void* stream);

int gccnmf_coherence(const float* X, int F, int T, int batch, float* CC, void* stream);

int gccnmf_magnitude(const float* X, int F, int T, int batch, float* V, void* stream);

#define GCCNMF_RECONSTRUCT_RATIO 0x100
#define GCCNMF_RECONSTRUCT_SPATIAL_BIT (1 << 16)
#define GCCNMF_RECONSTRUCT_SPATIAL_BATCH(batch) ((batch) | GCCNMF_RECONSTRUCT_SPATIAL_BIT)
#define GCCNMF_RECONSTRUCT_SPATIAL_WORKSPACE_FLOATS(batch, S, Fp) (4L * (batch) * (S) * (Fp))
#define GCCNMF_RECONSTRUCT_SPATIAL_ITERATIONS(n) ((n) << 20)
#define GCCNMF_RECONSTRUCT_SPATIAL_EM_WORKSPACE_FLOATS(batch, S, Fp, Tp) (4L * (batch) * (S) * (Fp) + (long)(batch) * (S) * (Fp) * (Tp))
#define GCCNMF_SPATIAL_LOADING 1e-3
long gccnmf_reconstruct_workspace_floats(int T, int K, int S, int batch);
int gccnmf_reconstruct(const float* W, const float* H, const unsigned char* argmax, const float* masks,
                       const float* X, const float* V, int F, int T, int K, int S, int batch, float* workspace,
                       float* spec, void* stream);

int gccnmf_istft_ola(const float* spec, int nsig, int n_fft, int hop, int T, int batch, const float* window,
                     const float* twiddle, float gain, int center, float* frames, float* y, void* stream);

int gccnmf_ola_frames_halo(const float* prev, int halo, const float* frames, int nsig, int n_fft, int hop, int T, int first_sample, int L,
                           float gain, float* y, void* stream);

int gccnmf_rt_process_block(const float* block_in, float* block_out, float* in_ring, float* out_ring, float* X, float* Y,
                            float* C, float* HMask, int* argmaxTDOA, float* tfMask, float* hist, int* hist_pos, float* target,
                            float* gccphat, const float* W, const float* cosT, const float* sinT, const float* window,
                            const float* twiddle, int windowSize, int hopSize, int blockSize, int K, int Kp, int D, int Dp,
                            int numTDOAHistory, int target_mode, int separation_enabled, int localization_enabled,
                            int localization_window, int frames_mode, void* stream);

#define GCCNMF_RT_SEPARATION_SPATIAL 2
#define GCCNMF_RT_SPATIAL_STATE_OFFSET(S, D, Lh) ((((long)(S) * (D) * (Lh) + 3) / 4) * 4)
#define GCCNMF_RT_SPATIAL_STATE_FLOATS(S, NC, F) (4L * (S) * (NC) * (F))
int gccnmf_rt_process_block_ll(const float* block_in, float* block_out, float* in_ring, float* out_ring, float* X, float* Y, float* C,
                               float* HMask, int* argmaxTDOA, float* tfMask, float* hist, int* hist_pos, float* target,
                               float* gccphat, const float* W, const float* cosT, const float* sinT, const float* window,
                               const float* synthesis_window, const float* twiddle, const float* colsumW, float* Hcoef, float* Rv,
                               int windowSize, int hopSize, int blockSize, int K, int Kp, int D, int Dp, int numTDOAHistory,
                               int target_mode, int separation_enabled, int localization_enabled, int localization_window,
                               int frames_mode, int numHUpdates, int out_delay_blocks, void* stream);

#ifdef GCCNMF_EXPERIMENTS
int gccnmf_debug_set_trace(long long* buf, int blocks);

int gccnmf_debug_mfma_peak(float* scratch, int blocks, int iters, void* stream);
#endif

typedef struct gccnmf_direct_gemm {
    const float* A;
    const float* B;
    long sA, sB;
    int lda, ldb;
    int M, N, Kd, batch;
    const float* bscale;
    long s_bscale;
    const float* tailA;
    long s_tailA;
    int tail_row;
    float* rowsumB;
    long s_rowsumB;
    float* C;
    long sC;
    int ldc;
    float* Ct;
    long sCt;
    int ldct;
    const float* E0;
    long sE0;
    int lde0;
    const float* E1;
    long sE1;
    const float* E2;
    long sE2;
    const float* ktailA;
    const float* ktailB;
    long s_ktailA, s_ktailB;
    float alpha, eps;
    int tiles_m, tiles_n, xc, sm, sn;
    long long* trace;
} gccnmf_direct_gemm;
int gccnmf_gemm_direct(const gccnmf_direct_gemm* desc, int epilogue, int tile, void* stream);

int gccnmf_debug_gemm_plan(int M, int N, int batch, int xcd_affine, int concurrent, int narrow_capable, int* plan, int* items, int max_items);

int gccnmf_debug_gemm(const float* A, const float* B, float* C, int M, int N, int Kd, int lda, int ldb, int ldc,
                      int a_clamp, int b_clamp, int layout, int batch, long sA, long sB, long sC,
                      const float* bscale, float* rowsumB, void* stream);

#ifdef __cplusplus
}
// ... 3 lines not shown
```

Measured before the change: 151,400 frames/s.

## Fuse one-hot argmax masking of H into the reconstruction GEMM's B load

Adds a masked-B variant of the DMA GEMM kernel for the direct reconstruction. It streams H directly along with the uint8 argmax mask into LDS and zeroes B fragments whose mask differs from the tile's target, in place of first materialising a masked H copy (H times mask per target) in a workspace. This drops the gcc_masked_h_kernel launch, its large workspace write and read, and the workspace allocation when the plan query allows it. In exchange it adds extra LDS byte reads, compare-multiplies per fragment and finer-grained dword DMA loads for B, which may lower GEMM efficiency.

```diff
diff --git a/gcc_nmf_amd/_hip.py b/gcc_nmf_amd/_hip.py
--- a/gcc_nmf_amd/_hip.py
+++ b/gcc_nmf_amd/_hip.py
@@ -466,6 +466,16 @@
     return reconstruct_spatial_workspace_floats(batch, S, Fp) if mode == 'spatial' else 0
 
 
+GCCNMF_PLAN_RECONSTRUCT = 1 << 30
+
+
+def reconstruct_reads_h(F, T, K, S, batch):
+    plan = lib().gccnmf_klnmf_plan(F, T, K, batch, GCCNMF_PLAN_RECONSTRUCT | S)
+    if plan < 0:
+        raise ValueError('gccnmf_klnmf_plan rejects the reconstruction query F=%d T=%d K=%d S=%d batch=%d' % (F, T, K, S, batch))
+    return plan == 1
+
+
 def reconstruct(W, H, argmax, masks, X, V, F, T, K, S, batch, spec, mode='direct', workspace=None, iterations=0, stream=None):
     if mode not in RECONSTRUCTIONS:
         raise ValueError('unknown reconstruction mode %r' % (mode,))
diff --git a/gcc_nmf_amd/csrc/common.h b/gcc_nmf_amd/csrc/common.h
--- a/gcc_nmf_amd/csrc/common.h
+++ b/gcc_nmf_amd/csrc/common.h
@@ -29,7 +29,7 @@
     return p;
 }
 
-#define GCCNMF_TUNE_KEYS 26
+#define GCCNMF_TUNE_KEYS 27
 struct GccNmfTune {
     int v[GCCNMF_TUNE_KEYS];
 };
@@ -64,3 +64,6 @@
 #define gccnmf_tune_chain_rag (gccnmf_tune.v[23])
 #define gccnmf_tune_chain_chunk (gccnmf_tune.v[24])
 #define gccnmf_tune_chain_fault (gccnmf_tune.v[25])
+#define gccnmf_tune_reconstruct_h (gccnmf_tune.v[26])
+
+bool gccnmf_reconstruct_from_h(int F, int T, int K, int S, int batch);
diff --git a/gcc_nmf_amd/csrc/gcc.hip b/gcc_nmf_amd/csrc/gcc.hip
--- a/gcc_nmf_amd/csrc/gcc.hip
+++ b/gcc_nmf_amd/csrc/gcc.hip
@@ -11,6 +11,21 @@
     if (!gccnmf_tune_ring || !gccnmf_ring_supports(Kd) || gccnmf_tune_tile_policy == 1) return false;
     if (gccnmf_tune_tile_policy == 2) return true;
     return (long)batch * gccnmf_ceil_div(M, 512) * gccnmf_ceil_div(N, 64) < 256;
+}
+
+static void gcc_reconstruct_shape(int F, int T, int S, bool& tail, int& M, int& ncol) {
+    tail = (F % 128) == 1;
+    M = tail ? F - 1 : F;
+    ncol = 2 * S * gccnmf_round_up(T, 64);
+}
+
+bool gccnmf_reconstruct_from_h(int F, int T, int K, int S, int batch) {
+    bool tail;
+    int M, ncol;
+    gcc_reconstruct_shape(F, T, S, tail, M, ncol);
+    if (!gccnmf_tune_reconstruct_h || (gccnmf_tune_reconstruct_h == 1 && gccnmf_tune_tile_policy == 1)) return false;
+    if (gcc_small_launch(batch, M, ncol, K)) return false;
+    return M > 128 && gccnmf_tune_dma && gccnmf_tune_ablate != 128;
 }
 
 __global__ __launch_bounds__(256) void ang_mean_kernel(const float* __restrict__ ang, int T, int D, int Dp, int Tp,
@@ -486,7 +501,9 @@
     batch &= 0xffff;
     if (spatial && !ratio) return GCCNMF_ERR_ARG;
     if (iterations && !spatial) return GCCNMF_ERR_ARG;
-    if (!W || !H || (!argmax && !masks) || !X || (!ratio && (!V || !workspace)) || !spec || F < 2 || T < 1 || K < 1 || S < 1 || batch < 1)
+    const bool from_h = !ratio && !masks && argmax && !((uintptr_t)argmax & 15) && F >= 2 && T >= 1 && K >= 1 && S >= 1 &&
+                        gccnmf_reconstruct_from_h(F, T, K, S, batch);
+    if (!W || !H || (!argmax && !masks) || !X || (!ratio && (!V || (!workspace && !from_h))) || !spec || F < 2 || T < 1 || K < 1 || S < 1 || batch < 1)
         return GCCNMF_ERR_ARG;
     if (spatial && (!workspace || ((uintptr_t)workspace & 15))) return GCCNMF_ERR_ARG;
     if (ratio && S > GCCNMF_RATIO_MAX_TARGETS) return GCCNMF_ERR_UNSUPPORTED;
@@ -500,22 +517,31 @@
         return gccnmf_launch_spatial_em(X, F, T, S, batch, iterations, workspace, powers, spec, s);
     }
     GccNmfPitches p = gccnmf_make_pitches(F, T, K);
-    const int ncol = 2 * S * p.Tp;
+    bool tail;
+    int M, ncol;
+    gcc_reconstruct_shape(F, T, S, tail, M, ncol);
     float* Hm = workspace;
-    hipLaunchKernelGGL(gcc_masked_h_kernel, dim3(gccnmf_ceil_div(ncol, 1024), p.Kp, batch), dim3(256), 0, s, H, argmax, masks, K, p.Kp,
-                       T, p.Tp, p.Np, S, Hm);
-    GCCNMF_CHECK_LAUNCH();
-    const bool tail = (F % 128) == 1;
+    if (!from_h) {
+        hipLaunchKernelGGL(gcc_masked_h_kernel, dim3(gccnmf_ceil_div(ncol, 1024), p.Kp, batch), dim3(256), 0, s, H, argmax, masks, K, p.Kp,
+                           T, p.Tp, p.Np, S, Hm);
+        GCCNMF_CHECK_LAUNCH();
+    }
     GemmArgs a = {};
     a.A = W; a.sA = (long)p.Fp * p.Kp; a.lda = p.Kp; a.a_clamp = p.Fp - 1;
     a.B = Hm; a.sB = (long)p.Kp * ncol; a.ldb = ncol; a.b_clamp = ncol - 4;
-    a.M = tail ? F - 1 : F; a.N = ncol; a.Kd = K;
+    a.M = M; a.N = ncol; a.Kd = K;
     a.tail_row = F - 1;
     a.batch = batch; a.xcd_affine = 1;
     a.C = spec; a.sC = 2L * S * p.Fp * p.Tp;
     a.E0 = V; a.sE0 = (long)p.Fp * p.Np;
     a.X = (const float2*)X; a.sX = 2L * p.Fp * p.Tp;
     a.T = T; a.Tp = p.Tp; a.Fp = p.Fp; a.ldv = p.Np;
+    if (from_h) {
+        a.B = H; a.sB = (long)p.Kp * p.Np; a.ldb = p.Np; a.b_clamp = 0;
+        const GemmMaskArgs mk = {argmax, (long)p.Kp * p.Tp};
+        return tail ? gccnmf_launch_gemm_dma<true, false, EPI_PHASE, true, true>(a, s, mk)
+                    : gccnmf_launch_gemm_dma<true, false, EPI_PHASE, false, true>(a, s, mk);
+    }
     if (gcc_small_launch(batch, a.M, a.N, a.Kd))
         return tail ? gccnmf_launch_gemm_ring<true, false, EPI_PHASE, true>(a, s) : gccnmf_launch_gemm_ring<true, false, EPI_PHASE, false>(a, s);
     const bool tall = a.M > 128;
diff --git a/gcc_nmf_amd/csrc/gemm_dma.h b/gcc_nmf_amd/csrc/gemm_dma.h
--- a/gcc_nmf_amd/csrc/gemm_dma.h
+++ b/gcc_nmf_amd/csrc/gemm_dma.h
@@ -27,6 +27,21 @@
                  : "memory");
 }
 
+__device__ __forceinline__ void gemm_dma4(const float* wave_uniform_base, unsigned lane_byte_offset, unsigned lds_wave_byte_addr) {
+    asm volatile("s_mov_b32 m0, %2\n\tglobal_load_lds_dword %0, %1"
+                 :
+                 : "v"(lane_byte_offset), "s"(wave_uniform_base), "s"(lds_wave_byte_addr)
+                 : "memory");
+}
+
+__device__ __forceinline__ void gemm_dma16_lanes16(const float* wave_uniform_base, unsigned lane_byte_offset, unsigned lds_wave_byte_addr) {
+    unsigned long long saved;
+    asm volatile("s_mov_b64 %0, exec\n\ts_mov_b64 exec, 0xffff\n\ts_mov_b32 m0, %3\n\tglobal_load_lds_dwordx4 %1, %2\n\ts_mov_b64 exec, %0"
+                 : "=&s"(saved)
+                 : "v"(lane_byte_offset), "s"(wave_uniform_base), "s"(lds_wave_byte_addr)
+                 : "memory");
+}
+
 __device__ __forceinline__ int gemm_swz(int row) { return (row >> 2) & 3; }
 
 __device__ __forceinline__ int gemm_opaque_tid() {
@@ -47,6 +62,13 @@
 __device__ __forceinline__ gemm_f32x2 gemm_lds_read2_b32(unsigned byte_addr) {
     gemm_f32x2 v;
     asm volatile("ds_read2_b32 %0, %1 offset0:%2 offset1:%3" : "=v"(v) : "v"(byte_addr), "n"(OFF0), "n"(OFF1));
+    return v;
+}
+
+template <int OFF>
+__device__ __forceinline__ unsigned gemm_lds_read_u8(unsigned byte_addr) {
+    unsigned v;
+    asm volatile("ds_read_u8 %0, %1 offset:%2" : "=v"(v) : "v"(byte_addr), "n"(OFF));
     return v;
 }
 
@@ -414,13 +436,20 @@
     static constexpr int SBUF = 128 * TM * 16 + 64 * 16 + 16 + 16;
 };
 
-template <bool A_KC, bool B_KC, int EPI, bool TAIL, int TM, bool NARROW>
+struct GemmMaskArgs {
+    const unsigned char* mask;
+    long s_mask;
+};
+
+template <bool A_KC, bool B_KC, int EPI, bool TAIL, int TM, bool NARROW, bool MASK = false>
 __device__ __forceinline__ void gemm_dma_workgroup(const GemmArgs& p, float* const smem, float* const s_rowvec, unsigned* const s_arrivals_p,
                                                    int* const s_ticket, const int list, int t, const GemmSync& sync, const int sync_it = 0,
-                                                   const bool trace_on = true) {
+                                                   const bool trace_on = true, const GemmMaskArgs& mk = GemmMaskArgs{},
+                                                   unsigned char* const s_mask = nullptr) {
     static_assert(TM == 4 || TM == 2, "");
     static_assert(TM == 4 || EPI != EPI_UPDW, "the fused W update owns all rows of its atoms: full-height tiles only");
     static_assert(!NARROW || (EPI != EPI_UPDW && TM == 4), "narrow items: full-height tiles with an element-wise epilogue");
+    static_assert(!MASK || (A_KC && !B_KC && EPI == EPI_PHASE && !NARROW), "the masked-B form is the reconstruction's: W . (H_c * M_i) with the phase epilogue");
     constexpr int BK = 16, BM = 128 * TM, BN = 64, RW = 32 * TM;
     constexpr int NA = 2 * TM;
     constexpr int SA = BM * BK, SB = BN * BK;
@@ -451,6 +480,9 @@
     unsigned long long tail_mask = 0, scale_mask = 0;
     bool wave_active = false, do_tail = false, do_rowsum = false;
     unsigned offA[NA], offB = 0;
+    int m_t0 = 0;
+    unsigned m_target = 0, offM = 0;
+    const unsigned char* __restrict__ mask_src = nullptr;
     auto take_item = [&](const int ticket) -> bool {
         int f_, tm_, c_, nw_;
         if (!gemm_dma_item(p, list, ticket, f_, tm_, c_, nw_)) return false;
@@ -475,6 +507,13 @@
         tail_mask = (wave == 0 && do_tail) ? 0x0full : 0ull;
         scale_mask = (wave == 0 && bscale != nullptr) ? 0xf0ull : 0ull;
         scale_src = bscale != nullptr ? bscale : A;
+        if constexpr (MASK) {
+            const int ic = __builtin_amdgcn_readfirstlane(col0 / p.Tp);
+            m_t0 = col0 - ic * p.Tp;
+            m_target = (unsigned)(ic >> 1);
+            B += (ic & 1) * p.T;
+            mask_src = mk.mask + file * mk.s_mask + m_t0;
+        }
         return true;
     };
     auto set_offsets = [&](const int lane) {
@@ -490,7 +529,10 @@
                 offA[i] = 4u * (unsigned)(kk * p.lda + min(row0 + col, p.a_clamp));
             }
         }
-        if (B_KC) {
+        if constexpr (MASK) {
+            offB = 4u * (unsigned)(wave * 4 * p.ldb + min(m_t0 + lane, p.T - 1));
+            offM = (unsigned)((wave * 4 + ((lane & 15) >> 2)) * p.Tp + 16 * (lane & 3));
+        } else if (B_KC) {
             const int row = wave * 16 + (lane >> 2), c = (lane & 3) ^ gemm_swz(row);
             offB = 4u * (unsigned)(min(col0 + row, p.b_clamp) * p.ldb + 4 * c);
         } else {
@@ -503,6 +545,8 @@
     float tail_acc = 0.f, rowsum_acc = 0.f;
 
     const unsigned lds0 = __builtin_amdgcn_readfirstlane((unsigned)(size_t)(gemm_lds_ptr)smem);
+    unsigned ldsM = 0;
+    if constexpr (MASK) ldsM = __builtin_amdgcn_readfirstlane((unsigned)(size_t)(gemm_lds_ptr)s_mask);
     unsigned side_off = 0;
 
     auto dma_piece = [&](const int piece, const int kt, const int buf) {
@@ -511,6 +555,15 @@
 #endif
         if (piece < NA) {
             gemm_dma16(A + (A_KC ? (long)kt * BK : (long)kt * BK * p.lda), offA[piece], lds0 + 4 * (buf * SBUF + (wave * NA + piece) * 256));
+        } else if constexpr (MASK) {
+            if (piece < NA + 4) {
+                const int j = piece - NA;
+                gemm_dma4(B + ((long)kt * BK + j) * p.ldb, offB, lds0 + 4 * (buf * SBUF + SA + (wave * 4 + j) * BN));
+            } else if (piece == NA + 4) {
+                if (TAIL) gemm_dma16_masked(tail_src + kt * BK, side_off, lds0 + 4 * (buf * SBUF + SA + SB), tail_mask);
+            } else {
+                gemm_dma16_lanes16((const float*)(mask_src + (long)kt * BK * p.Tp), offM, ldsM + buf * (BK * BN) + wave * (4 * BN));
+            }
         } else if (piece == NA) {
             gemm_dma16(B + (B_KC ? (long)kt * BK : (long)kt * BK * p.ldb), offB, lds0 + 4 * (buf * SBUF + SA + wave * 256));
         } else {
@@ -521,11 +574,11 @@
             }
         }
     };
-    constexpr int NPIECES = NA + 2;
+    constexpr int NPIECES = MASK ? NA + 6 : NA + 2;
 #ifdef GEMM_DMA_SPREAD
     constexpr int SPREAD = GEMM_DMA_SPREAD;
 #else
-    constexpr int SPREAD = (A_KC && !B_KC) ? 1 : 2;
+    constexpr int SPREAD = (MASK && NPIECES > 4 * TM) ? 0 : (A_KC && !B_KC) ? 1 : 2;
 #endif
 
     const gemm_f32x4 zero4 = {0.f, 0.f, 0.f, 0.f};
@@ -533,6 +586,8 @@
     GemmFrag<B_KC, 2, BN> b0, b1;
     gemm_f32x4 sc0 = zero4, sc1 = zero4, t4 = zero4, tb4 = zero4, ts4 = zero4, rs4 = zero4;
     gemm_f32x2 tbxy = {0.f, 0.f}, tbzw = {0.f, 0.f};
+    unsigned mk0[4][2] = {}, mk1[4][2] = {}, mkt[4] = {};
+    unsigned oM = 0, oMT = 0;
 
     const unsigned arrivals_addr = (unsigned)(size_t)(gemm_lds_ptr)s_arrivals_p;
     unsigned oA0 = 0, oA1 = 0, oB0 = 0, oB1 = 0, oTB = 0, oRS = 0;
@@ -550,19 +605,48 @@
         oB1 = 4 * SA + (B_KC ? 4 * (bcol * 16 + 4 * ((2 + hh) ^ gemm_swz(bcol))) : 4 * (4 * (2 + hh) * BN + bcol));
         oTB = 4 * SA + (B_KC ? 4 * (tj * 16 + 4 * (tg ^ gemm_swz(tj))) : 4 * (4 * tg * BN + tj));
         oRS = 4 * SA + 4 * ((tid_ >> 2) * 16 + 4 * (tid_ & 3));
-    };
-
-    auto read_group0 = [&](const unsigned lds) {
+        if constexpr (MASK) {
+            oM = (unsigned)(4 * hh * BN + bcol);
+            oMT = (unsigned)(4 * tg * BN + tj);
+        }
+    };
+
+    auto read_mask = [&](auto q_c, unsigned (&m)[4][2], const unsigned ldsm) {
+        constexpr int Q = decltype(q_c)::value;
+        m[0][0] = gemm_lds_read_u8<8 * Q * BN + 0 * BN>(ldsm + oM);
+        m[0][1] = gemm_lds_read_u8<8 * Q * BN + 0 * BN + 32>(ldsm + oM);
+        m[1][0] = gemm_lds_read_u8<8 * Q * BN + 1 * BN>(ldsm + oM);
+        m[1][1] = gemm_lds_read_u8<8 * Q * BN + 1 * BN + 32>(ldsm + oM);
+        m[2][0] = gemm_lds_read_u8<8 * Q * BN + 2 * BN>(ldsm + oM);
+        m[2][1] = gemm_lds_read_u8<8 * Q * BN + 2 * BN + 32>(ldsm + oM);
+        m[3][0] = gemm_lds_read_u8<8 * Q * BN + 3 * BN>(ldsm + oM);
+        m[3][1] = gemm_lds_read_u8<8 * Q * BN + 3 * BN + 32>(ldsm + oM);
+    };
+    auto apply_mask = [&](GemmFrag<B_KC, 2, BN>& b, unsigned (&m)[4][2]) {
+        if constexpr (MASK) {
+#pragma unroll
+            for (int e = 0; e < 4; ++e)
+#pragma unroll
+                for (int h = 0; h < 2; ++h) {
+                    gemm_tie(m[e][h]);
+                    b.v[e][0][h] *= (m[e][h] == m_target) ? 1.0f : 0.0f;
+                }
+        }
+    };
+
+    auto read_group0 = [&](const unsigned lds, const unsigned ldsm) {
         if (wave_active) {
             a0.read(lds + oA0);
             b0.read(lds + oB0);
+            if constexpr (MASK) read_mask(std::integral_constant<int, 0>{}, mk0, ldsm);
         }
         if (SCALE) sc0 = gemm_lds_read_b128<4 * (SA + SB + BK)>(lds + 16 * hh);
     };
-    auto read_group1 = [&](const unsigned lds) {
+    auto read_group1 = [&](const unsigned lds, const unsigned ldsm) {
         if (wave_active) {
             a1.read(lds + oA1);
             b1.read(lds + oB1);
+            if constexpr (MASK) read_mask(std::integral_constant<int, 1>{}, mk1, ldsm);
         }
         if (SCALE) sc1 = gemm_lds_read_b128<4 * (SA + SB + BK) + 32>(lds + 16 * hh);
         if (TAIL) {
@@ -573,6 +657,12 @@
                 tbxy = gemm_lds_read2_b32<0 * BN, 1 * BN>(lds + oTB);
                 tbzw = gemm_lds_read2_b32<2 * BN, 3 * BN>(lds + oTB);
                 if (SCALE) ts4 = gemm_lds_read_b128<4 * (SA + SB + BK)>(lds + 16 * tg);
+                if constexpr (MASK) {
+                    mkt[0] = gemm_lds_read_u8<0 * BN>(ldsm + oMT);
+                    mkt[1] = gemm_lds_read_u8<1 * BN>(ldsm + oMT);
+                    mkt[2] = gemm_lds_read_u8<2 * BN>(ldsm + oMT);
+                    mkt[3] = gemm_lds_read_u8<3 * BN>(ldsm + oMT);
+                }
             }
         }
         if (B_KC) rs4 = gemm_lds_read_b128<0>(lds + oRS);
@@ -585,6 +675,7 @@
             gemm_tie(sc0);
             b0.scale(sc0);
         }
+        if constexpr (MASK) apply_mask(b0, mk0);
     };
     auto wait_group1 = [&]() {
         gemm_wait_lds();
@@ -594,6 +685,7 @@
             gemm_tie(sc1);
             b1.scale(sc1);
         }
+        if constexpr (MASK) apply_mask(b1, mk1);
         if (TAIL) {
             gemm_tie(t4);
             if (B_KC) {
@@ -606,6 +698,13 @@
                     gemm_tie(ts4);
                     tb4 *= ts4;
                 }
+                if constexpr (MASK) {
+#pragma unroll
+                    for (int e = 0; e < 4; ++e) {
+                        gemm_tie(mkt[e]);
+                        tb4[e] *= (mkt[e] == m_target) ? 1.0f : 0.0f;
+                    }
+                }
             }
         }
         if (B_KC) gemm_tie(rs4);
@@ -632,7 +731,7 @@
         const int ktn = min(kt + 1, nkt - 1);
         GEMM_PROBE(0);
 #if !(GEMM_DMA_ABL & 1)
-        read_group1(ldsC);
+        read_group1(ldsC, ldsM + CUR * (BK * BN));
 #endif
         __builtin_amdgcn_sched_barrier(0);
         if (wave_active) {
@@ -698,7 +797,7 @@
 #endif
                 GEMM_PROBE_SET(5);
 #if !(GEMM_DMA_ABL & 1)
-                read_group0(ldsN);
+                read_group0(ldsN, ldsM + (CUR ^ 1) * (BK * BN));
 #endif
                 __builtin_amdgcn_sched_barrier(0);
             }
@@ -793,7 +892,7 @@
         }
         asm volatile("s_waitcnt vmcnt(0)" ::: "memory");
         __syncthreads();
-        read_group0(lds0);
+        read_group0(lds0, ldsM);
         wait_group0();
 
         if constexpr (NARROW) {
@@ -919,6 +1018,19 @@
     gemm_dma_workgroup<A_KC, B_KC, EPI, TAIL, TM, NARROW>(p, smem, s_rowvec, &s_arrivals, s_ticket, list, t, none);
 }
 
+template <bool TAIL, int TM>
+__global__ __launch_bounds__(256, 2) void gccnmf_gemm_dma_masked_b_kernel(GemmArgs p, GemmMaskArgs mk) {
+    __shared__ __attribute__((aligned(16))) float smem[2 * GemmDmaLds<TM>::SBUF];
+    __shared__ __attribute__((aligned(16))) float s_rowvec[4];
+    __shared__ __attribute__((aligned(16))) unsigned char s_mask[2 * 16 * 64];
+    __shared__ unsigned s_arrivals;
+    __shared__ int s_ticket[2];
+    const int list = p.lists == 8 ? (int)(blockIdx.x & 7) : 0;
+    const int t = p.lists == 8 ? (int)(blockIdx.x >> 3) : (int)blockIdx.x;
+    GemmSync none = {};
+    gemm_dma_workgroup<true, false, EPI_PHASE, TAIL, TM, false, true>(p, smem, s_rowvec, &s_arrivals, s_ticket, list, t, none, 0, true, mk, s_mask);
+}
+
 struct GemmChain {
     int first[5];
     int it0, iterations;
@@ -991,8 +1103,8 @@
     return a.lists * (a.cw + a.split + a.cr);
 }
 
-template <bool A_KC, bool B_KC, int EPI, bool TAIL, int TM>
-static int gccnmf_launch_gemm_dma_tm(GemmArgs a, hipStream_t stream) {
+template <bool A_KC, bool B_KC, int EPI, bool TAIL, int TM, bool MASK = false>
+static int gccnmf_launch_gemm_dma_tm(GemmArgs a, hipStream_t stream, const GemmMaskArgs& mk = GemmMaskArgs{}) {
 #ifdef GEMM_DMA_NO_NARROW
     constexpr bool NARROW = false;
 #else
@@ -1007,29 +1119,35 @@
     a.prefetch = 0;
     a.wpl = 0;
     int grid = classic_grid;
+    if constexpr (MASK) {
+        hipLaunchKernelGGL((gccnmf_gemm_dma_masked_b_kernel<TAIL, TM>), dim3(grid), dim3(256), 0, stream, a, mk);
+        GCCNMF_CHECK_LAUNCH();
+        return GCCNMF_OK;
+    } else {
 #ifdef GCCNMF_EXPERIMENTS
-    a.prefetch = gccnmf_tune_prefetch;
-    if (gccnmf_tune_persistent && TM == 4 && classic_grid > 512) {
-        a.tickets = gccnmf_ticket_block(stream);
-        if (a.tickets) {
-            grid = 512;
-            a.wpl = 512 / a.lists;
-        }
-    }
-#endif
-    hipLaunchKernelGGL((gccnmf_gemm_dma_kernel<A_KC, B_KC, EPI, TAIL, TM, NARROW>), dim3(grid), dim3(256), 0, stream, a);
-    GCCNMF_CHECK_LAUNCH();
-    return GCCNMF_OK;
-}
-
-template <bool A_KC, bool B_KC, int EPI, bool TAIL>
-static int gccnmf_launch_gemm_dma(GemmArgs a, hipStream_t stream) {
+        a.prefetch = gccnmf_tune_prefetch;
+        if (gccnmf_tune_persistent && TM == 4 && classic_grid > 512) {
+            a.tickets = gccnmf_ticket_block(stream);
+            if (a.tickets) {
+                grid = 512;
+                a.wpl = 512 / a.lists;
+            }
+        }
+#endif
+        hipLaunchKernelGGL((gccnmf_gemm_dma_kernel<A_KC, B_KC, EPI, TAIL, TM, NARROW>), dim3(grid), dim3(256), 0, stream, a);
+        GCCNMF_CHECK_LAUNCH();
+        return GCCNMF_OK;
+    }
+}
+
+template <bool A_KC, bool B_KC, int EPI, bool TAIL, bool MASK = false>
+static int gccnmf_launch_gemm_dma(GemmArgs a, hipStream_t stream, const GemmMaskArgs& mk = GemmMaskArgs{}) {
     if (!a.A || !a.B || !a.C || a.M < 1 || a.N < 1 || a.Kd < 1 || a.batch < 1) return GCCNMF_ERR_ARG;
     if ((a.lda & 3) || (a.ldb & 3)) return GCCNMF_ERR_ARG;
     a.ablate = gccnmf_tune_ablate;
     a.exact_div = gccnmf_tune_exact_div;
     if constexpr (EPI != EPI_UPDW) {
-        if ((a.M <= 256 && gccnmf_tune_tail_split != 0) || gccnmf_tune_tail_split == 3) return gccnmf_launch_gemm_dma_tm<A_KC, B_KC, EPI, TAIL, 2>(a, stream);
+        if ((a.M <= 256 && gccnmf_tune_tail_split != 0) || gccnmf_tune_tail_split == 3) return gccnmf_launch_gemm_dma_tm<A_KC, B_KC, EPI, TAIL, 2, MASK>(a, stream, mk);
         const long tpf = (long)gccnmf_ceil_div(a.M, 512) * gccnmf_ceil_div(a.N, 64);
         const long total = tpf * a.batch, rounds = total / 512;
         if (gccnmf_tune_tail_split == 1 && !gccnmf_trace_buf && !a.concurrent && a.M > 256) {
@@ -1043,17 +1161,17 @@
             const int head = (int)(rounds * 512 / tpf);
             const int rest = a.batch - head;
             if (rounds >= 1 && head >= 8 && rest >= 1 && 2 * rest * tpf <= 768) split = full_cost(head * tpf) + half_cost(2 * rest * tpf) + 10;
-            if (all_half < plain && all_half <= split) return gccnmf_launch_gemm_dma_tm<A_KC, B_KC, EPI, TAIL, 2>(a, stream);
+            if (all_half < plain && all_half <= split) return gccnmf_launch_gemm_dma_tm<A_KC, B_KC, EPI, TAIL, 2, MASK>(a, stream, mk);
             if (split < plain) {
                 GemmArgs h = a, t = a;
                 h.batch = head;
                 t.batch = rest;
                 t.file0 = a.file0 + head;
-                int rc = gccnmf_launch_gemm_dma_tm<A_KC, B_KC, EPI, TAIL, 4>(h, stream);
+                int rc = gccnmf_launch_gemm_dma_tm<A_KC, B_KC, EPI, TAIL, 4, MASK>(h, stream, mk);
                 if (rc) return rc;
-                return gccnmf_launch_gemm_dma_tm<A_KC, B_KC, EPI, TAIL, 2>(t, stream);
-            }
-        }
-    }
-    return gccnmf_launch_gemm_dma_tm<A_KC, B_KC, EPI, TAIL, 4>(a, stream);
-}
+                return gccnmf_launch_gemm_dma_tm<A_KC, B_KC, EPI, TAIL, 2, MASK>(t, stream, mk);
+            }
+        }
+    }
+    return gccnmf_launch_gemm_dma_tm<A_KC, B_KC, EPI, TAIL, 4, MASK>(a, stream, mk);
+}
diff --git a/gcc_nmf_amd/csrc/nmf.hip b/gcc_nmf_amd/csrc/nmf.hip
--- a/gcc_nmf_amd/csrc/nmf.hip
+++ b/gcc_nmf_amd/csrc/nmf.hip
@@ -54,6 +54,7 @@
     {1, 0, 3, 0},
     {2048, 1, 65536, 0},
     {0, 0, 1, 1},
+    {1, 0, 2, 0},
 };
 static std::atomic<int> gccnmf_knob_value[GCCNMF_TUNE_KEYS];
 static std::atomic<int> gccnmf_knobs_ready{0};
@@ -998,6 +999,11 @@
 int gccnmf_klnmf_plan(int F, int N, int K, int batch, int flags) {
     GCCNMF_ENTER();
     if (F < 2 || N < 1 || K < 1 || batch < 1) return -1;
+    if (flags > 0 && (flags & GCCNMF_PLAN_RECONSTRUCT(0))) {
+        const int S = flags & 0xff;
+        if ((flags & ~0xff) != GCCNMF_PLAN_RECONSTRUCT(0) || S < 1 || batch > 0xffff) return -1;
+        return gccnmf_reconstruct_from_h(F, N, K, S, batch) ? 1 : 0;
+    }
     KlnmfMode m;
     if (decode_mode(flags, F, K, m)) return -1;
     if (m.fixed_w) return gccnmf_klnmf_fixed_supported(F, K) ? 16 : -1;
diff --git a/gcc_nmf_amd/engine.py b/gcc_nmf_amd/engine.py
--- a/gcc_nmf_amd/engine.py
+++ b/gcc_nmf_amd/engine.py
@@ -279,7 +279,7 @@
             self.ws_scores = z(self.lib.gccnmf_scores_workspace_floats(F, T, g.S, B))
             self.scores = z(B, g.Kp, g.S * g.Tp)
             self.argmax = torch.zeros((B, g.Kp, g.Tp), dtype=torch.uint8, device=dev)
-            self.ws_rec = z(self._reconstruct_workspace_floats()) if self.reconstruction == 'direct' else None
+            self.ws_rec = None
             self.ws_cov = z(self._reconstruct_workspace_floats()) if self.reconstruction == 'spatial' else None
             self.spec = z(B, 2 * g.S, g.Fp, g.Tp, 2)
             self.frames = None
@@ -408,9 +408,18 @@
         g = self.g
         return _hip.reconstruct_workspace_floats(self.reconstruction, g.T, g.K, g.S, self.batch, g.Fp, self.spatialIterations)
 
-    def _reconstruct_workspace(self):
+    def _reconstruct_workspace(self, one_hot=True, S=None):
         if self.reconstruction != 'spatial':
             _hip.check_spatial_iterations(self.spatialIterations, self.reconstruction)
+            if self.reconstruction != 'direct':
+                return None
+            g = self.g
+            S = g.S if S is None else S
+            if one_hot and _hip.reconstruct_reads_h(g.F, g.T, g.K, S, self.batch):
+                return self.ws_rec
+            need = _hip.reconstruct_workspace_floats('direct', g.T, g.K, S, self.batch, g.Fp)
+            if self.ws_rec is None or self.ws_rec.numel() < need:
+                self.ws_rec = torch.zeros(need, dtype=torch.float32, device=self.device)
             return self.ws_rec
         need = self._reconstruct_workspace_floats()
         if self.ws_cov is None or self.ws_cov.numel() < need:
@@ -741,7 +750,7 @@
     def reconstruct(self):
         g = self.g
         _hip.reconstruct(self.W, self.H, None if self.targetMode else self.argmax, self.soft_masks, self.X, self.V, g.F, g.T, g.K, 2,
-                         self.batch, self.spec, mode=self.reconstruction, workspace=self._reconstruct_workspace(),
+                         self.batch, self.spec, mode=self.reconstruction, workspace=self._reconstruct_workspace(one_hot=not self.targetMode, S=2),
                          iterations=self.spatialIterations)
 
     def get_atom_tdoa_indexes(self):
diff --git a/include/gccnmf_hip.h b/include/gccnmf_hip.h
--- a/include/gccnmf_hip.h
+++ b/include/gccnmf_hip.h
@@ -50,6 +50,7 @@
 
 int gccnmf_klnmf_chain_status(const float* workspace, int F, int N, int K, int batch, int* status);
 
+#define GCCNMF_PLAN_RECONSTRUCT(S) ((1 << 30) | (S))
 int gccnmf_klnmf_plan(int F, int N, int K, int batch, int flags);
 
 int gccnmf_klnmf_stage(const float* V, float* W, float* H, float* workspace, int F, int N, int K, int batch,
```

After: 151,600 frames/s, median of 6. About the same (+0.1%).
